# Fastaxx/Penguin.jl

Measured on AMD Instinct MI355X. Metric: time-steps/sec + SpMV GB/s (% HBM roofline), 3D mono diffusion 512^3, higher is better.
Workload: dtype f64

## Files before the change

### include/penguin_hip.h

```cpp
#ifndef PENGUIN_HIP_H
#define PENGUIN_HIP_H

#include <stddef.h>
#include <stdint.h>

#ifdef __cplusplus
extern "C" {
#endif

typedef struct pg_mesh pg_mesh;
typedef struct pg_capacity pg_capacity;
typedef struct pg_diffops pg_diffops;
typedef struct pg_solver pg_solver;
typedef struct pg_streamvort pg_streamvort;

enum { PG_BODY_BALL = 1, PG_BODY_MULTIBALL = 2, PG_BODY_HALFSPACE = 3, PG_BODY_ELLIPSOID = 4, PG_BODY_PLANE = 5 };
enum { PG_BODY_PROGRAM = 6 };
enum { PG_BODY_POLYGON = 7 };
enum { PG_FLAG_COMPLEMENT = 1, PG_FLAG_NO_CENTROIDS = 2 };
enum { PG_CAP_V = 0, PG_CAP_GAMMA = 1, PG_CAP_CELL_TYPES = 2, PG_CAP_A = 3, PG_CAP_B = 4,
       PG_CAP_W = 5, PG_CAP_C_OMEGA = 6, PG_CAP_C_GAMMA = 7,
       PG_CAP_ST_V0 = 8, PG_CAP_ST_V1 = 9, PG_CAP_ST_CT_OMEGA = 10, PG_CAP_ST_CT_GAMMA = 11 };
enum { PG_OP_G = 0, PG_OP_H = 1, PG_OP_WINV = 2,
       PG_OP_C0 = 3 , PG_OP_K0 = 6  };
// ... 194 lines not shown
                                       pg_solver** out);
int32_t pg_solver_create_unsteady_diph(pg_capacity* c1, pg_diffops* o1, pg_capacity* c2, pg_diffops* o2,
                                       const pg_jump_desc* ic, const pg_border_desc* borders, int32_t nborders,
                                       const double* D1, const double* D2, const double* f1, const double* f2,
                                       double dt, const double* T0, int32_t scheme, pg_solver** out);
int32_t pg_solver_create_moving_diph(pg_capacity* c1, pg_diffops* o1, pg_capacity* c2, pg_diffops* o2, const pg_jump_desc* ic,
                                     const pg_border_desc* borders, int32_t nborders, const double* D1, const double* D2,
                                     const double* f1_n, const double* f1_np1, const double* f2_n, const double* f2_np1,
                                     const double* T_prev, pg_solver* previous, int32_t scheme, pg_solver** out);
int32_t pg_solver_create_steady_mono(pg_capacity* c, pg_diffops* o, const pg_bc_desc* bc_interface,
                                     const pg_border_desc* borders, int32_t nborders, const double* Dcoef,
                                     const double* source, pg_solver** out);
int32_t pg_solver_create_steady_diph(pg_capacity* c1, pg_diffops* o1, pg_capacity* c2, pg_diffops* o2,
                                     const pg_jump_desc* ic, const pg_border_desc* borders, int32_t nborders,
                                     const double* D1, const double* D2, const double* f1, const double* f2,
                                     pg_solver** out);
int32_t pg_solver_create_moving_mono(pg_capacity* c, pg_diffops* o, const pg_bc_desc* bc_interface,
                                     const pg_border_desc* borders, int32_t nborders, const double* Dcoef,
                                     const double* source_n, const double* source_np1, const double* T_prev,
                                     pg_solver* previous, int32_t scheme, pg_solver** out);
int32_t pg_solver_create_moving_advdiff_mono(pg_capacity* c, pg_diffops* o, const pg_bc_desc* bc_interface,
                                             const pg_border_desc* borders, int32_t nborders, const double* Dcoef,
                                             const double* source_n, const double* source_np1, const double* T_prev,
                                             pg_solver* previous, int32_t scheme, pg_solver** out);
int32_t pg_solver_create_moving_advdiff_diph(pg_capacity* c1, pg_diffops* o1, pg_capacity* c2, pg_diffops* o2,
                                             const pg_jump_desc* ic, const pg_border_desc* borders, int32_t nborders,
                                             const double* D1, const double* D2, const double* f1_n, const double* f1_np1,
                                             const double* f2_n, const double* f2_np1, const double* T_prev,
                                             pg_solver* previous, int32_t scheme, pg_solver** out);
int32_t pg_solver_create_moving_stefan_diph(pg_capacity* c1, pg_diffops* o1, pg_capacity* c2, pg_diffops* o2,
                                            const pg_jump_desc* ic, const pg_border_desc* borders, int32_t nborders,
                                            const double* D1, const double* D2, const double* f1_n, const double* f1_np1,
                                            const double* f2_n, const double* f2_np1, const double* T_prev,
                                            pg_solver* previous, int32_t scheme, pg_solver** out);
int32_t pg_solver_stefan_terms(const pg_solver* s, double* out);
int32_t pg_solver_destroy(pg_solver* s);

int32_t pg_streamvort_create(pg_capacity* c, pg_diffops* o, const double* nu, double dt, const pg_bc_desc* bc_stream,
                             const pg_bc_desc* bc_vorticity, const pg_border_desc* borders_stream, int32_t nborders_stream,
                             const pg_border_desc* borders_vorticity, int32_t nborders_vorticity, const double* psi0,
                             const double* omega0, pg_streamvort** out);
int32_t pg_streamvort_destroy(pg_streamvort* sv);
int32_t pg_streamvort_set_omega(pg_streamvort* sv, const double* omega);
int32_t pg_streamvort_set_source(pg_streamvort* sv, const double* f_n , const double* f_np1 );
int32_t pg_streamvort_set_interface_values(pg_streamvort* sv, int32_t which, const double* g_n , const double* g_np1 );
int32_t pg_streamvort_set_border_values(pg_streamvort* sv, int32_t which, const double* values );
int32_t pg_streamvort_solve_stream(pg_streamvort* sv, const pg_krylov_opts* opts, pg_step_info* info);
int32_t pg_streamvort_step(pg_streamvort* sv, int32_t scheme, const pg_krylov_opts* opts, pg_step_info* info_psi,
                           pg_step_info* info_omega);
int32_t pg_streamvort_run(pg_streamvort* sv, int64_t steps, int32_t scheme, const pg_krylov_opts* opts, int32_t save_every,
                          pg_streamvort_run_info* info);
int32_t pg_streamvort_get(const pg_streamvort* sv, int32_t field, int64_t state_index, double* out, int64_t len);
int32_t pg_streamvort_num_states(const pg_streamvort* sv, int64_t* out);
int32_t pg_streamvort_time(const pg_streamvort* sv, int64_t state_index, double* out);
int32_t pg_streamvort_solver(pg_streamvort* sv, int32_t which, pg_solver** borrowed);

int32_t pg_solver_set_source(pg_solver* s, int32_t phase, const double* f_n , const double* f_np1 );
int32_t pg_solver_set_interface_value(pg_solver* s, const double* g_n , const double* g_np1 );
int32_t pg_solver_set_border_values(pg_solver* s, const double* values );

enum { PG_TD_SOURCE = 0, PG_TD_INTERFACE = 1, PG_TD_BORDER = 2 };
enum { PG_TD_MAX_TERMS = 8 };
int32_t pg_solver_set_separable(pg_solver* s, int32_t which, int32_t phase, int32_t K, const double* modes, int64_t nrows,
                                const double* coef);
int32_t pg_solver_clear_separable(pg_solver* s, int32_t which, int32_t phase);
int32_t pg_solver_time_data_info(const pg_solver* s, int32_t* terms , int64_t* nrows, int64_t* cursor);
int32_t pg_debug_td_combine_ms(pg_solver* s, int32_t scheme, int32_t repeats, double* ms_per_combine, int32_t* modes,
                               int64_t* bytes);

enum { PG_PROG_MAX_OPS = 96, PG_PROG_MAX_CONST = 32, PG_PROG_MAX_STACK = 16 };
enum {
  PG_OP_CONST = 0, PG_OP_VAR = 1, PG_OP_ADD = 2, PG_OP_SUB = 3, PG_OP_MUL = 4, PG_OP_DIV = 5, PG_OP_NEG = 6, PG_OP_ABS = 7,
  PG_OP_SQRT = 8, PG_OP_EXP = 9, PG_OP_LOG = 10, PG_OP_SIN = 11, PG_OP_COS = 12, PG_OP_TANH = 13, PG_OP_POW = 14,
  PG_OP_ATAN2 = 15, PG_OP_ERF = 16, PG_OP_ERFC = 17, PG_OP_MIN = 18, PG_OP_MAX = 19, PG_OP_LT = 20, PG_OP_LE = 21,
  PG_OP_GT = 22, PG_OP_GE = 23, PG_OP_SELECT = 24, PG_OP_COUNT = 25
};
typedef struct pg_program {
  int32_t n_ops;
  int32_t n_const;
  uint8_t op[PG_PROG_MAX_OPS];
  uint8_t arg[PG_PROG_MAX_OPS];
  double konst[PG_PROG_MAX_CONST];
} pg_program;
int32_t pg_program_validate(const pg_program* prog);
int32_t pg_program_eval_host(const pg_program* prog, int64_t npts, const double* xyz , double t, double* out);
int32_t pg_solver_set_program(pg_solver* s, int32_t which, int32_t phase, const pg_program* prog, int64_t nrows,
                              const double* times );
int32_t pg_solver_set_border_program(pg_solver* s, int32_t key, const pg_program* prog, int64_t nrows,
                                     const double* times );
int32_t pg_solver_program_info(const pg_solver* s, int32_t* programs , int64_t* entries , int64_t* nrows,
                               int64_t* cursor);
int32_t pg_debug_program_eval(const pg_program* prog, int64_t npts, const double* xyz , double t, double* out);
int32_t pg_capacity_create_program(pg_mesh* m, const pg_program* phi, const pg_program* grad , int32_t flags,
                                   pg_capacity** out);
int32_t pg_capacity_create_program3(pg_mesh* m, const pg_program* phi, const pg_program* grad , int32_t flags,
                                    pg_capacity** out);
int32_t pg_capacity_create_polygon(pg_mesh* m, const double* xy , int64_t M, int32_t flags, pg_capacity** out);
int32_t pg_capacity_polygon_ms_parts(const pg_capacity* c, double* ms );
int32_t pg_capacity_create_spacetime_program(pg_mesh* m, const pg_program* phi, const pg_program* grad ,
                                             const pg_program* dphidt, int32_t flags, double t0, double t1, int32_t nq,
                                             const double* tau_w , pg_capacity** out);
int32_t pg_capacity_create_spacetime_polygon(pg_mesh* m, const double* xy0 , const double* xy1 , int64_t M,
                                             int32_t flags, double t0, double t1, int32_t nq, const double* tau_w ,
                                             pg_capacity** out);
int32_t pg_debug_spacetime_kernel_timing(int32_t on);
int32_t pg_debug_capacity_spacetime_ms_parts(const pg_capacity* c, double* ms , int64_t* n_listed);
int32_t pg_debug_td_eval_ms(pg_solver* s, int32_t scheme, int32_t repeats, double* ms_per_eval, int64_t* entries,
                            int64_t* instructions);

enum { PG_MON_SUM = 0, PG_MON_SUMSQ = 1 };
enum { PG_MON_MAX = 8 };
int32_t pg_solver_set_monitors(pg_solver* s, int32_t K, const int32_t* kinds, const double* weights , int64_t len);
int32_t pg_solver_clear_monitors(pg_solver* s);
int32_t pg_solver_monitor_info(const pg_solver* s, int32_t* K, int64_t* rows, int32_t* sparse , int64_t* stored );
int32_t pg_solver_get_monitor_series(const pg_solver* s, int64_t row0, int64_t nrows, double* values ,
                                     double* times );
int32_t pg_solver_drop_states(pg_solver* s);
int32_t pg_debug_monitor_ms(pg_solver* s, int32_t repeats, double* ms_per_eval, int64_t* bytes);
int32_t pg_debug_monitor_eval(pg_solver* s, double* values , int32_t* x_form);

int32_t pg_solver_initial_solve(pg_solver* s, const pg_krylov_opts* opts, pg_step_info* info);
int32_t pg_solver_step(pg_solver* s, int32_t scheme, const pg_krylov_opts* opts, pg_step_info* info);
int32_t pg_solver_run(pg_solver* s, double Tend, int32_t scheme, const pg_krylov_opts* opts, int32_t do_initial,
                      int64_t max_steps, int32_t save_every, pg_run_info* info);
int32_t pg_solver_num_states(const pg_solver* s, int64_t* out);
int32_t pg_solver_get_state(const pg_solver* s, int64_t state_index, double* x, int64_t len);
int32_t pg_solver_system_info(const pg_solver* s, int32_t which, pg_system_info* out);
int32_t pg_solver_get_system_csr(const pg_solver* s, int32_t which, int64_t* rowptr, int64_t* col, double* val,
                                 double* b, int64_t* idx);
int32_t pg_solver_get_row_scaling(const pg_solver* s, int32_t which, double* ds);
int32_t pg_solver_mg_info(const pg_solver* s, pg_mg_info* out);
int32_t pg_solver_mg_info_for(const pg_solver* s, int32_t precond, pg_mg_info* out);
int32_t pg_solver_mg_step_info(const pg_solver* s, int32_t which, pg_mg_info* out);
int32_t pg_solver_spectral_estimate(pg_solver* s, int32_t which, pg_specest_info* out);
int32_t pg_solver_time_spmv(pg_solver* s, int32_t which, int32_t reps, double* avg_ms);

int32_t pg_partition_planes(const int64_t* weight, int64_t nplanes, int32_t nranks, int64_t* bounds);
int32_t pg_slab_numbering_host(int32_t K, int64_t plane, int64_t nplanes, int64_t p0, int64_t p1, const uint8_t* active,
                               int64_t* out);

int32_t pg_debug_spmv_compare(pg_solver* s, int32_t which, int32_t variant_a, int32_t variant_b, double* max_abs_diff,
                              double* max_abs);
int32_t pg_debug_spmv_mode_compare(pg_solver* s, int32_t which, int32_t mode, double* max_abs_diff, double* max_abs,
                                   double* max_dot_rel);
int32_t pg_debug_spmv_sizes(pg_solver* s, int32_t which, int64_t* n, int64_t* n_vec, int64_t* nnz, int32_t* grid);
#define PG_DEBUG_SPMV_SENTINEL 0x7FF8C0DE5EED0BADull
int32_t pg_debug_spmv_apply(pg_solver* s, int32_t which, int32_t variant, int32_t mode, const double* x, const double* aux,
                            const double* dotx, const double* base, double pc0, double pc1, double pc2, int32_t fold,
                            int32_t done, int32_t repeat, double* y, double* partials, double* slot_sums, double* folded,
                            int64_t* ticket);
#define PG_DEBUG_SPMV_SENTINEL_F32 0x7FC5EED0u
int32_t pg_debug_spmv_apply_typed(pg_solver* s, int32_t which, int32_t kind, const void* x, const void* base, double pc0, double pc1,
                                  double pc2, double sigma, int32_t done, double* y64, float* y32, float* p32);
int32_t pg_debug_read_probe(int64_t bytes, int32_t elem_bytes, int32_t nt, int32_t blocks, int32_t reps, double* gbs);
int32_t pg_debug_run_virtual_ranks(int32_t nranks, int32_t N, const int64_t* n, const double* L, int32_t body_kind,
                                   const double* params, int32_t nparams, double interface_value, double border_value,
                                   int32_t nkeys, const int32_t* keys, double dt, int32_t scheme_ctor, int32_t scheme_run,
                                   int64_t steps, double* x_out, int64_t* n_own_out, int64_t* nnz_out,
                                   int64_t* n_ghost_out, int64_t* iters_out);
int32_t pg_debug_set_virtual_rank_method(int32_t method, int32_t restart);
int32_t pg_debug_set_virtual_rank_precond(int32_t precond);
int32_t pg_debug_set_virtual_rank_ramp(double ramp);
int32_t pg_debug_set_virtual_rank_kick(int64_t step, double factor);
int32_t pg_debug_virtual_rank_info(int32_t rank, int64_t* full_rows, int64_t* loop_rows, int64_t* loop_bytes,
                                   int64_t* loop_ghosts);
int32_t pg_debug_scale_diagonal_rows(pg_solver* s, double factor);
int32_t pg_debug_set_poly_give_up(int32_t iterations);

int32_t pg_debug_mg_aggregates(pg_solver* s, int32_t level, int64_t* n, int32_t* agg);
int32_t pg_debug_mg_level_csr(pg_solver* s, int32_t level, int64_t* n, int64_t* nnz, int64_t* rowptr, int64_t* col, double* val);
int32_t pg_debug_mg_apply(pg_solver* s, const double* r, double* z);
int32_t pg_debug_mg_aggregates_for(pg_solver* s, int32_t precond, int32_t level, int64_t* n, int32_t* agg);
int32_t pg_debug_mg_level_csr_for(pg_solver* s, int32_t precond, int32_t level, int64_t* n, int64_t* nnz, int64_t* rowptr, int64_t* col,
                                  double* val);
int32_t pg_debug_mg_apply_for(pg_solver* s, int32_t precond, const double* r, double* z);
int32_t pg_debug_mg_step_aggregates(pg_solver* s, int32_t which, int32_t level, int64_t* n, int32_t* agg);
int32_t pg_debug_mg_step_level_csr(pg_solver* s, int32_t which, int32_t level, int64_t* n, int64_t* nnz, int64_t* rowptr, int64_t* col,
                                   double* val);
int32_t pg_debug_mg_step_apply(pg_solver* s, int32_t which, const double* r, double* z);

int32_t pg_debug_specest_hessenberg(pg_solver* s, int32_t which, int32_t* steps, double* H);

int32_t pg_solver_guess_info(pg_solver* s, int32_t* kept, int32_t* nstates, int32_t* offsets , double* coef ,
                             double* rr_plain, double* rr_taken);

#ifdef __cplusplus
}
#endif
#endif
```

### penguin/jl_amd/_lib.py

```python
from __future__ import annotations

import ctypes as C
import os
import re
from pathlib import Path

import numpy as np

_HERE = Path(__file__).resolve().parent
LIB_PATH = Path(os.environ["PG_LIB_PATH"]) if os.environ.get("PG_LIB_PATH") else _HERE / "lib" / "libpenguin_hip.so"
HEADER_PATH = _HERE.parent.parent / "include" / "penguin_hip.h"


class PenguinHipError(RuntimeError):
    pass


PG_BODY_BALL, PG_BODY_MULTIBALL, PG_BODY_HALFSPACE, PG_BODY_ELLIPSOID, PG_BODY_PLANE = 1, 2, 3, 4, 5
PG_BODY_PROGRAM, PG_BODY_POLYGON = 6, 7
PG_FLAG_COMPLEMENT, PG_FLAG_NO_CENTROIDS = 1, 2
PG_CAP_V, PG_CAP_GAMMA, PG_CAP_CELL_TYPES, PG_CAP_A, PG_CAP_B, PG_CAP_W, PG_CAP_C_OMEGA, PG_CAP_C_GAMMA = range(8)
PG_CAP_ST_V0, PG_CAP_ST_V1, PG_CAP_ST_CT_OMEGA, PG_CAP_ST_CT_GAMMA = 8, 9, 10, 11
PG_OP_G, PG_OP_H, PG_OP_WINV = 0, 1, 2
PG_OP_C0, PG_OP_K0 = 3, 6
# ... 197 lines not shown
def solver_mg_info(handle, precond: int = PG_PRECOND_MG) -> dict:
    info = pg_mg_info()
    check(lib().pg_solver_mg_info_for(handle, C.c_int32(precond), C.byref(info)))
    n = info.levels
    return {"levels": n, "tail_level": info.tail_level, "rows": list(info.rows[:n]), "nnz": list(info.nnz[:n]),
            "setup_ms": info.setup_ms, "bytes": info.bytes}


def debug_mg_aggregates(handle, level: int, precond: int = PG_PRECOND_MG) -> np.ndarray:
    n = C.c_int64(0)
    check(lib().pg_debug_mg_aggregates_for(handle, C.c_int32(precond), C.c_int32(level), C.byref(n), None))
    agg = np.zeros(max(n.value, 1), dtype=np.int32)
    check(lib().pg_debug_mg_aggregates_for(handle, C.c_int32(precond), C.c_int32(level), C.byref(n), agg.ctypes.data_as(c_i32_p)))
    return agg[: n.value]


def debug_mg_level_csr(handle, level: int, precond: int = PG_PRECOND_MG):
    n, nnz = C.c_int64(0), C.c_int64(0)
    pc = C.c_int32(precond)
    check(lib().pg_debug_mg_level_csr_for(handle, pc, C.c_int32(level), C.byref(n), C.byref(nnz), None, None, None))
    rowptr, col, val = np.zeros(n.value + 1, dtype=np.int64), np.zeros(max(nnz.value, 1), dtype=np.int64), np.zeros(max(nnz.value, 1))
    check(lib().pg_debug_mg_level_csr_for(handle, pc, C.c_int32(level), C.byref(n), C.byref(nnz), iptr(rowptr), iptr(col), dptr(val)))
    return rowptr, col[: nnz.value], val[: nnz.value]


def debug_mg_apply(handle, r: np.ndarray, precond: int = PG_PRECOND_MG) -> np.ndarray:
    r = np.ascontiguousarray(r, dtype=np.float64)
    z = np.zeros_like(r)
    check(lib().pg_debug_mg_apply_for(handle, C.c_int32(precond), dptr(r), dptr(z)))
    return z


def _mg_info_dict(info) -> dict:
    n = info.levels
    return {"levels": n, "tail_level": info.tail_level, "rows": list(info.rows[:n]), "nnz": list(info.nnz[:n]),
            "setup_ms": info.setup_ms, "bytes": info.bytes}


def solver_mg_step_info(handle, which: int = 0) -> dict:
    info = pg_mg_info()
    check(lib().pg_solver_mg_step_info(handle, C.c_int32(which), C.byref(info)))
    return _mg_info_dict(info)


def debug_mg_step_aggregates(handle, which: int, level: int) -> np.ndarray:
    n = C.c_int64(0)
    check(lib().pg_debug_mg_step_aggregates(handle, C.c_int32(which), C.c_int32(level), C.byref(n), None))
    agg = np.zeros(max(n.value, 1), dtype=np.int32)
    check(lib().pg_debug_mg_step_aggregates(handle, C.c_int32(which), C.c_int32(level), C.byref(n), agg.ctypes.data_as(c_i32_p)))
    return agg[: n.value]


def debug_mg_step_level_csr(handle, which: int, level: int):
    n, nnz = C.c_int64(0), C.c_int64(0)
    w = C.c_int32(which)
    check(lib().pg_debug_mg_step_level_csr(handle, w, C.c_int32(level), C.byref(n), C.byref(nnz), None, None, None))
    rowptr, col, val = np.zeros(n.value + 1, dtype=np.int64), np.zeros(max(nnz.value, 1), dtype=np.int64), np.zeros(max(nnz.value, 1))
    check(lib().pg_debug_mg_step_level_csr(handle, w, C.c_int32(level), C.byref(n), C.byref(nnz), iptr(rowptr), iptr(col), dptr(val)))
    return rowptr, col[: nnz.value], val[: nnz.value]


def debug_mg_step_apply(handle, which: int, r: np.ndarray) -> np.ndarray:
    r = np.ascontiguousarray(r, dtype=np.float64)
    z = np.zeros_like(r)
    check(lib().pg_debug_mg_step_apply(handle, C.c_int32(which), dptr(r), dptr(z)))
    return z


def solver_spectral_estimate(handle, which: int = 0, run: bool = True) -> dict:
    info = pg_specest_info()
    check(lib().pg_solver_spectral_estimate(handle, C.c_int32(which | (0 if run else 4)), C.byref(info)))
    return {k: getattr(info, k) for k, _ in pg_specest_info._fields_ if k != "reserved"}


def debug_specest_hessenberg(handle, which: int = 0, run: bool = True) -> np.ndarray:
    w = C.c_int32(which | (0 if run else 4))
    k = C.c_int32(0)
    check(lib().pg_debug_specest_hessenberg(handle, w, C.byref(k), None))
    H = np.zeros((k.value + 1) * max(k.value, 1))
    check(lib().pg_debug_specest_hessenberg(handle, w, C.byref(k), dptr(H)))
    return H[: (k.value + 1) * k.value].reshape((k.value + 1, k.value), order="F")


DEBUG_SPMV_SENTINEL = 0x7FF8C0DE5EED0BAD
DEBUG_SPMV_GUARD = 64


def debug_spmv_sizes(handle, which: int) -> tuple[int, int, int, int]:
    n, nv, nnz, grid = C.c_int64(0), C.c_int64(0), C.c_int64(0), C.c_int32(0)
    check(lib().pg_debug_spmv_sizes(handle, C.c_int32(which), C.byref(n), C.byref(nv), C.byref(nnz), C.byref(grid)))
    return n.value, nv.value, nnz.value, grid.value


def loop_system_csr(handle, which: int):
    n, _, nnz, _ = debug_spmv_sizes(handle, which)
    rowptr, col, val = np.zeros(n + 1, dtype=np.int64), np.zeros(max(nnz, 1), dtype=np.int64), np.zeros(max(nnz, 1))
    check(lib().pg_solver_get_system_csr(handle, C.c_int32(which), iptr(rowptr), iptr(col), dptr(val), None, None))
    return rowptr, col[:nnz], val[:nnz]


def debug_spmv_apply(handle, which: int, variant: int, mode: int, x, aux=None, dotx=None, base=None, pc=(0.0, 0.0, 0.0),
                     fold: int = 0, done: int = 0, repeat: int = 1) -> dict:
    n, nv, _, grid = debug_spmv_sizes(handle, which)

    def arr(a, length, name):
        if a is None:
            return None, None
        a = np.ascontiguousarray(a, dtype=np.float64)
        if a.size != length:
            raise ValueError(f"debug_spmv_apply: {name} has {a.size} entries, the matrix needs {length}")
        return a, dptr(a)

    xs, xp = arr(x, nv, "x")
    auxs, auxp = arr(aux, n, "aux")
    dots, dotp = arr(dotx, n, "dotx")
    bases, basep = arr(base, n, "base")
    y = np.zeros(n + DEBUG_SPMV_GUARD)
    partials = np.zeros((5, grid))
    sums, folded = np.zeros(5), np.zeros(5)
    ticket = C.c_int64(-1)
    check(lib().pg_debug_spmv_apply(handle, C.c_int32(which), C.c_int32(variant), C.c_int32(mode), xp, auxp, dotp, basep,
                                    C.c_double(pc[0]), C.c_double(pc[1]), C.c_double(pc[2]), C.c_int32(fold), C.c_int32(done),
                                    C.c_int32(repeat), dptr(y), dptr(partials), dptr(sums), dptr(folded), C.byref(ticket)))
    return {"y": y, "partials": partials, "slot_sums": sums, "folded": folded, "ticket": ticket.value, "grid": grid, "n": n}


DEBUG_SPMV_SENTINEL_F32 = 0x7FC5EED0
TYPED_FIRST, TYPED_MIDDLE, TYPED_HANDOVER = 1, 2, 3


def debug_spmv_apply_typed(handle, which: int, kind: int, x, base=None, pc=(0.0, 0.0, 0.0), sigma: float = 1.0, done: int = 0) -> dict:
    n, nv, _, _ = debug_spmv_sizes(handle, which)
    want_x = np.float64 if kind == TYPED_FIRST else np.float32
    want_b = {TYPED_FIRST: None, TYPED_MIDDLE: np.float32, TYPED_HANDOVER: np.float64}[kind]
    x = np.ascontiguousarray(x)
    if x.dtype != want_x or x.size != nv:
        raise ValueError(f"debug_spmv_apply_typed: x must be {nv} x {np.dtype(want_x).name}")
    if (base is None) != (want_b is None):
        raise ValueError("debug_spmv_apply_typed: base goes with kinds 2 and 3, and only with them")
    bp = None
    if base is not None:
        base = np.ascontiguousarray(base)
        if base.dtype != want_b or base.size != n:
            raise ValueError(f"debug_spmv_apply_typed: base must be {n} x {np.dtype(want_b).name}")
        bp = base.ctypes.data_as(C.c_void_p)
    y64 = np.zeros(n + DEBUG_SPMV_GUARD) if kind == TYPED_HANDOVER else None
    y32 = np.zeros(n + DEBUG_SPMV_GUARD, dtype=np.float32) if kind != TYPED_HANDOVER else None
    p32 = np.zeros(n + DEBUG_SPMV_GUARD, dtype=np.float32) if kind == TYPED_FIRST else None
    ptr = lambda a: None if a is None else a.ctypes.data_as(C.c_void_p)
    check(lib().pg_debug_spmv_apply_typed(handle, C.c_int32(which), C.c_int32(kind), x.ctypes.data_as(C.c_void_p), bp,
                                          C.c_double(pc[0]), C.c_double(pc[1]), C.c_double(pc[2]), C.c_double(sigma), C.c_int32(done),
                                          ptr(y64), ptr(y32), ptr(p32)))
    return {"y": y64 if kind == TYPED_HANDOVER else y32, "p32": p32}
```

### penguin/jl_amd/csrc/pg_common.h

```cpp
#pragma once
#include <hip/hip_runtime.h>
#include "pg_rccl.h"

#include <chrono>
#include <cstdint>
#include <cstdio>
#include <cstring>
#include <stdexcept>
#include <string>
#include <vector>

#include "../../../include/penguin_hip.h"

namespace pg {

using i64 = int64_t;
using i32 = int32_t;

struct Error : std::runtime_error {
  using std::runtime_error::runtime_error;
};

void set_last_error(const std::string& msg);

#define PG_HIP(expr)                                                                              \
  do {                                                                                            \
    hipError_t _e = (expr);                                                                       \
    if (_e != hipSuccess)                                                                         \
      throw pg::Error(std::string("HIP error: ") + hipGetErrorString(_e) + " at " + __FILE__ + ":" + \
                      std::to_string(__LINE__) + " (" #expr ")");                                 \
  } while (0)

#define PG_NCCL(expr)                                                                             \
  do {                                                                                            \
    ncclResult_t _e = (expr);                                                                     \
    if (_e != ncclSuccess)                                                                        \
      throw pg::Error(std::string("RCCL error: ") + pg::rccl::api().GetErrorString(_e) + " at " + __FILE__ + ":" + \
                      std::to_string(__LINE__) + " (" #expr ")");                                 \
  } while (0)

#define PG_REQUIRE(cond, msg)                                   \
  do {                                                          \
    if (!(cond)) throw pg::Error(std::string(msg));             \
  } while (0)

#define PG_API_BEGIN try {
#define PG_API_END                                  \
  return 0;                                         \
  }                                                 \
  catch (const std::exception& e) {                 \
    pg::set_last_error(e.what());                   \
    return 1;                                       \
  }                                                 \
  catch (...) {                                     \
    pg::set_last_error("unknown exception");        \
    return 2;                                       \
  }

struct Config {
  bool debug = false;
  int alloc_poison = 0;
  int async_alloc = 0;
  int alloc_guard = 0;
  long long pool_limit_mb = 0;
  bool poly = true;
  int poly_degree = 6;
  bool poly_adapt = true;
  double poly_margin = 1.0;
  double poly_slack = -1.0;
  int poly_hist = 3;
  bool poly_trend = true;
  int poly_maxdeg = 0;
  int poly_mindeg = 4;
  bool poly_f32 = true;
  int poly_f32_tail = -1;
  int profile_sample = 3;
  bool gamma_elim = true;
  bool diag_elim = true;
  double diag_elim_frac = 0.0005;
  int spmv_variant = 70;
  int spmv_xcd = 1;
  int spmv_strip = 16;
  int spmv_march_k = 0;
  int spmv_minrun = 24;
  bool spmv_march = true;
  bool spmv_edges = true;
  int spmv_tile_units = 0;
  int spmv_blocks_per_cu = 0;
  bool halo_overlap = true;
  int guess_n = 4;
  int guess_depth = 7;
  bool guess_defer = true;
  bool guess_always = false;
  int guess_monitor = 256;
  double guess_pass_cost = 0.34;
  double guess_gain = 0.8;
  bool step_fuse = true;
  bool speculate_product = true;
  int mg_tail_rows = 2048;
  int unit_order = 0;
};
const Config& config();

struct LocalComm;

struct Context {
  bool inited = false;
  LocalComm* local = nullptr;
  int device = 0;
  hipStream_t stream = nullptr;
  hipStream_t comm_stream = nullptr;
  hipEvent_t ev_fork = nullptr, ev_join = nullptr;
  int rank = 0, nranks = 1;
  ncclComm_t comm = nullptr;
  ncclComm_t comm_halo = nullptr;
  bool profiling = false;
  std::string device_name;
};
Context& ctx();
void require_init();
void set_thread_context(Context* c);
Context* thread_context();
LocalComm* local_comm_create(int nranks);
void local_comm_destroy(LocalComm* c);
void comm_allreduce_sum_f64(double* dev, int count, hipStream_t st);
void comm_allreduce_max_f64(double* dev, int count, hipStream_t st);
void comm_allreduce_sum_u64(unsigned long long* dev, i64 count, hipStream_t st);

void* dev_alloc(size_t bytes);
void dev_free(void* p);
void dev_cache_release();
struct AsyncAllocScope {
  AsyncAllocScope();
  ~AsyncAllocScope();
};

template <class T>
struct DevBuf {
  T* p = nullptr;
  i64 n = 0;
  DevBuf() = default;
  explicit DevBuf(i64 n_) { alloc(n_); }
  DevBuf(const DevBuf&) = delete;
  DevBuf& operator=(const DevBuf&) = delete;
  DevBuf(DevBuf&& o) noexcept : p(o.p), n(o.n) { o.p = nullptr; o.n = 0; }
  DevBuf& operator=(DevBuf&& o) noexcept {
    if (this != &o) { release(); p = o.p; n = o.n; o.p = nullptr; o.n = 0; }
    return *this;
  }
  ~DevBuf() { release(); }
  void release() {
    if (p) dev_free(p);
    p = nullptr; n = 0;
  }
  void alloc(i64 n_) {
    release();
    n = n_;
    if (n > 0) p = static_cast<T*>(dev_alloc(sizeof(T) * static_cast<size_t>(n) + 64));
  }
  void zero() {
    if (n > 0) PG_HIP(hipMemsetAsync(p, 0, sizeof(T) * static_cast<size_t>(n), ctx().stream));
  }
  void upload(const T* h, i64 count, i64 offset = 0) {
    if (count > 0) {
      PG_HIP(hipMemcpyAsync(p + offset, h, sizeof(T) * static_cast<size_t>(count), hipMemcpyHostToDevice, ctx().stream));
      PG_HIP(hipStreamSynchronize(ctx().stream));
    }
  }
  void download(T* h, i64 count, i64 offset = 0) const {
    if (count > 0) {
      PG_HIP(hipMemcpyAsync(h, p + offset, sizeof(T) * static_cast<size_t>(count), hipMemcpyDeviceToHost, ctx().stream));
      PG_HIP(hipStreamSynchronize(ctx().stream));
    }
  }
};

inline void* pinned_scratch(int slot, size_t bytes) {
  static thread_local void* buf[2] = {nullptr, nullptr};
  static thread_local size_t cap[2] = {0, 0};
  if (bytes > cap[slot]) {
    if (buf[slot]) (void)hipHostFree(buf[slot]);
    PG_HIP(hipHostMalloc(&buf[slot], bytes + (bytes >> 2)));
    cap[slot] = bytes + (bytes >> 2);
  }
  return buf[slot];
}

struct Laps {
  bool on;
  std::chrono::steady_clock::time_point t0;
  explicit Laps() : on(config().debug), t0(std::chrono::steady_clock::now()) {}
  void lap(const char* what) {
    if (!on) return;
    (void)hipDeviceSynchronize();
    const auto t1 = std::chrono::steady_clock::now();
    fprintf(stderr, "[pg_laps] %-34s %8.2f ms\n", what, std::chrono::duration<double, std::milli>(t1 - t0).count());
    t0 = t1;
  }
};

struct EventPair {
  hipEvent_t e0 = nullptr, e1 = nullptr;
  EventPair() {
    PG_HIP(hipEventCreate(&e0));
    if (hipEventCreate(&e1) != hipSuccess) {
      (void)hipEventDestroy(e0);
      throw Error("hipEventCreate failed");
    }
  }
  ~EventPair() {
    if (e0) (void)hipEventDestroy(e0);
    if (e1) (void)hipEventDestroy(e1);
  }
  EventPair(const EventPair&) = delete;
  EventPair& operator=(const EventPair&) = delete;
};

inline int grid_for(i64 n, int block, int cap = 256 * 8) {
  i64 g = (n + block - 1) / block;
  if (g < 1) g = 1;
  if (g > cap) g = cap;
  return static_cast<int>(g);
}

constexpr int CAP_HALO = 3;

struct Slab {
  int N = 0;
  i64 n[3] = {1, 1, 1};
  i64 ext[3] = {1, 1, 1};
  i64 stride[3] = {1, 1, 1};
  i64 plane = 1;
  i64 nplanes = 1;
  i64 M = 1;
  i64 p0 = 0, p1 = 1;
  i64 s0 = 0, s1 = 1;
  i64 Mloc() const { return (s1 - s0) * plane; }
  i64 first_cell() const { return s0 * plane; }
  void set_own(i64 a, i64 b) {
    p0 = a; p1 = b;
    s0 = p0 - CAP_HALO; if (s0 < 0) s0 = 0;
// ... 38 lines not shown
```

### penguin/jl_amd/csrc/pg_context.hip

```cpp
#include "pg_common.h"

#include <cxxabi.h>
#include <execinfo.h>

#include <atomic>
#include <map>
#include <mutex>
#include <unordered_map>
#include <unordered_set>
#include "pg_host_algos.h"

#include <algorithm>
#include <array>
#include <memory>
#include <set>

namespace pg {

static thread_local std::string g_last_error;
void set_last_error(const std::string& msg) { g_last_error = msg; }

Context& ctx() {
  static Context c;
  Context* t = thread_context();
  return t ? *t : c;
}

const Config& config() {
  static const Config c = [] {
    Config k;
    auto geti = [](const char* name, long long dflt) { const char* v = getenv(name); return v ? atoll(v) : dflt; };
    auto getd = [](const char* name, double dflt) { const char* v = getenv(name); return v ? atof(v) : dflt; };
    k.debug = getenv("PG_DEBUG") != nullptr;
    k.alloc_poison = (int)geti("PG_ALLOC_POISON", 0);
    k.async_alloc = (int)geti("PG_ASYNC_ALLOC", 0);
    k.alloc_guard = (int)geti("PG_ALLOC_GUARD", 0);
    k.pool_limit_mb = geti("PG_POOL_LIMIT_MB", 0);
    k.poly = geti("PG_POLY", 1) != 0;
    k.poly_degree = (int)geti("PG_POLY_DEGREE", 6);
    k.poly_adapt = geti("PG_POLY_ADAPT", getenv("PG_POLY_DEGREE") ? 0 : 1) != 0;
    k.poly_margin = getd("PG_POLY_MARGIN", 1.0);
    k.poly_slack = getd("PG_POLY_SLACK", -1.0);
    k.poly_hist = (int)std::max<long long>(1, std::min<long long>(3, geti("PG_POLY_HIST", 3)));
    k.poly_maxdeg = (int)geti("PG_POLY_MAXDEG", 0);
    k.poly_mindeg = (int)std::max<long long>(2, std::min<long long>(8, geti("PG_POLY_MINDEG", 4)));
    k.poly_trend = geti("PG_POLY_TREND", 1) != 0;
    k.poly_f32 = geti("PG_POLY_F32", 1) != 0;
    k.poly_f32_tail = (int)std::max<long long>(-1, std::min<long long>(64, geti("PG_POLY_F32_TAIL", -1)));
    k.profile_sample = (int)std::max<long long>(1, geti("PG_PROFILE_SAMPLE", 3));
    k.gamma_elim = geti("PG_GAMMA_ELIM", 1) != 0;
    k.diag_elim = geti("PG_DIAG_ELIM", 1) != 0;
    k.diag_elim_frac = getd("PG_DIAG_ELIM_FRAC", 0.0005);
    k.spmv_variant = (int)geti("PG_SPMV_VARIANT", 70);
    k.spmv_xcd = (int)geti("PG_SPMV_XCD", 1);
    k.spmv_strip = (int)geti("PG_SPMV_STRIP", 16);
    k.spmv_march_k = (int)geti("PG_SPMV_MARCH_K", 0);
    k.spmv_minrun = (int)geti("PG_SPMV_MINRUN", 24);
    k.spmv_march = geti("PG_SPMV_MARCH", 1) != 0;
    k.spmv_edges = geti("PG_SPMV_EDGES", 1) != 0;
    k.spmv_tile_units = (int)geti("PG_SPMV_TILE_UNITS", 0);
    k.spmv_blocks_per_cu = (int)geti("PG_SPMV_BLOCKS_PER_CU", 0);
    k.halo_overlap = geti("PG_HALO_OVERLAP", 1) != 0;
    k.speculate_product = geti("PG_SPECULATE", 1) != 0;
    k.guess_n = (int)std::max<long long>(0, std::min<long long>(4, geti("PG_GUESS_STATES", 4)));
    k.guess_depth = (int)std::max<long long>(1, std::min<long long>(7, geti("PG_GUESS_DEPTH", 7)));
    k.mg_tail_rows = (int)std::max<long long>(0, geti("PG_MG_TAIL_ROWS", 2048));
    k.guess_monitor = (int)std::max<long long>(1, geti("PG_GUESS_MONITOR", 256));
    k.guess_pass_cost = getd("PG_GUESS_PASS_COST", 0.34);
    k.guess_always = geti("PG_GUESS_ALWAYS", 0) != 0;
    k.guess_defer = geti("PG_GUESS_DEFER", 1) != 0;
    k.guess_gain = getd("PG_GUESS_GAIN", 0.8);
    k.step_fuse = geti("PG_STEP_FUSE", 1) != 0;
    k.unit_order = (int)geti("PG_SPMV_UNIT_ORDER", 0);
    return k;
  }();
  return c;
}

void require_init() {
  if (!ctx().inited)
    throw Error("penguin_hip: not initialised (call pg_init / pg_init_distributed first)");
}

static void init_device(int device_id) {
  Context& c = ctx();
  int ndev = 0;
  hipError_t e = hipGetDeviceCount(&ndev);
  if (e != hipSuccess || ndev <= 0)
    throw Error("penguin_hip: no HIP device visible -- this library has no CPU fallback");
  PG_REQUIRE(device_id >= 0 && device_id < ndev, "penguin_hip: device id out of range");
  PG_HIP(hipSetDevice(device_id));
  hipDeviceProp_t prop;
  PG_HIP(hipGetDeviceProperties(&prop, device_id));
  c.device = device_id;
  c.device_name = std::string(prop.name) + " (" + prop.gcnArchName + ")";
  if (!c.stream) PG_HIP(hipStreamCreateWithFlags(&c.stream, hipStreamNonBlocking));
  if (!c.comm_stream) PG_HIP(hipStreamCreateWithFlags(&c.comm_stream, hipStreamNonBlocking));
  c.inited = true;
}

}

using namespace pg;

namespace pg {
namespace {
thread_local int t_async_scope = 0;
std::mutex g_alloc_mutex;
struct BlockCache {
  std::multimap<size_t, void*> free_blocks;
  std::unordered_map<void*, size_t> owned;
  size_t free_bytes = 0;
};
BlockCache g_cache;
constexpr size_t CACHE_TRIM_BYTES = (size_t)48 << 30;

size_t round_block(size_t bytes) {
  const size_t q = bytes >= ((size_t)2 << 20) ? ((size_t)2 << 20) : 4096;
  return (bytes + q - 1) / q * q;
}

bool cache_wanted(const Context& c, size_t bytes) {
  const int mode = config().async_alloc;
  if (mode < 0 || !c.inited || !c.stream || c.local) return false;
  if (!(t_async_scope > 0 || mode > 0)) return false;
  const long long lim = config().pool_limit_mb;
  return lim <= 0 || bytes < ((size_t)lim << 20);
}

void poison(void* p, size_t bytes) {
  if (!config().alloc_poison || !p || bytes == 0) return;
  Context& c = ctx();
  if (c.inited && c.stream) PG_HIP(hipMemsetAsync(p, 0xFF, bytes, c.stream));
  else PG_HIP(hipMemset(p, 0xFF, bytes));
}

void cache_trim_locked() {
  if (g_cache.free_blocks.empty()) return;
  (void)hipDeviceSynchronize();
  for (auto& kv : g_cache.free_blocks) {
    g_cache.owned.erase(kv.second);
    (void)hipFree(kv.second);
  }
  g_cache.free_blocks.clear();
  g_cache.free_bytes = 0;
}

void* dev_alloc_raw(size_t bytes) {
  void* p = nullptr;
  Context& c = ctx();
  if (cache_wanted(c, bytes)) {
    const size_t want = round_block(bytes);
    {
      std::lock_guard<std::mutex> lk(g_alloc_mutex);
      auto it = g_cache.free_blocks.lower_bound(want);
      if (it != g_cache.free_blocks.end() && it->first <= want + want / 8) {
        p = it->second;
        g_cache.free_bytes -= it->first;
        g_cache.free_blocks.erase(it);
      }
    }
    if (!p) {
      if (hipMalloc(&p, want) != hipSuccess || !p) {
        (void)hipGetLastError();
        { std::lock_guard<std::mutex> lk(g_alloc_mutex); cache_trim_locked(); }
        PG_HIP(hipMalloc(&p, want));
      }
      std::lock_guard<std::mutex> lk(g_alloc_mutex);
      g_cache.owned[p] = want;
    }
    poison(p, bytes);
    return p;
  }
  PG_HIP(hipMalloc(&p, bytes));
  poison(p, bytes);
  return p;
}

void dev_free_raw(void* p) {
  if (!p) return;
  {
    std::lock_guard<std::mutex> lk(g_alloc_mutex);
    auto it = g_cache.owned.find(p);
    if (it != g_cache.owned.end()) {
      g_cache.free_blocks.emplace(it->second, p);
      g_cache.free_bytes += it->second;
      if (g_cache.free_bytes > CACHE_TRIM_BYTES) cache_trim_locked();
      return;
    }
  }
  (void)hipFree(p);
}

constexpr size_t GUARD = 4096;
struct GuardInfo { char* raw; size_t bytes; unsigned long long seq; std::string where; };
std::unordered_map<void*, GuardInfo> g_guarded;
unsigned long long g_alloc_seq = 0;
std::string call_stack() {
  void* frames[24];
  const int nf = backtrace(frames, 24);
  char** sym = backtrace_symbols(frames, nf);
  std::string s;
  for (int i = 2; sym && i < nf && i < 12; ++i) {
    std::string f = sym[i];
    const size_t a = f.find('('), b = f.find('+', a == std::string::npos ? 0 : a);
    if (a != std::string::npos && b != std::string::npos && b > a + 1) {
      std::string mangled = f.substr(a + 1, b - a - 1);
      int st = 0;
      char* dem = abi::__cxa_demangle(mangled.c_str(), nullptr, nullptr, &st);
      f = st == 0 && dem ? dem : mangled;
      free(dem);
      const size_t par = f.find('(');
      if (par != std::string::npos) f = f.substr(0, par);
    }
// ... 2 lines not shown
  free(sym);
  return s;
}
}

AsyncAllocScope::AsyncAllocScope() { ++t_async_scope; }
AsyncAllocScope::~AsyncAllocScope() { --t_async_scope; }

void dev_cache_release() {
  std::lock_guard<std::mutex> lk(g_alloc_mutex);
  cache_trim_locked();
}

void* dev_alloc(size_t bytes) {
  if (!config().alloc_guard) return dev_alloc_raw(bytes);
  char* raw = static_cast<char*>(dev_alloc_raw(bytes + 2 * GUARD));
  Context& c = ctx();
  hipStream_t st = (c.inited && c.stream) ? c.stream : nullptr;
  PG_HIP(hipMemsetAsync(raw, 0xA5, GUARD, st));
  PG_HIP(hipMemsetAsync(raw + GUARD + bytes, 0xA5, GUARD, st));
  void* user = raw + GUARD;
  std::lock_guard<std::mutex> lk(g_alloc_mutex);
  g_guarded[user] = GuardInfo{raw, bytes, ++g_alloc_seq, call_stack()};
  return user;
}

void dev_free(void* p) {
  if (!config().alloc_guard) { dev_free_raw(p); return; }
  GuardInfo gi;
  {
    std::lock_guard<std::mutex> lk(g_alloc_mutex);
    auto it = g_guarded.find(p);
    if (it == g_guarded.end()) { gi.raw = nullptr; }
    else { gi = it->second; g_guarded.erase(it); }
  }
  if (!gi.raw) { dev_free_raw(p); return; }
  (void)hipDeviceSynchronize();
  std::vector<unsigned char> lo(GUARD), hi(GUARD);
  (void)hipMemcpy(lo.data(), gi.raw, GUARD, hipMemcpyDeviceToHost);
  (void)hipMemcpy(hi.data(), gi.raw + GUARD + gi.bytes, GUARD, hipMemcpyDeviceToHost);
  auto first_bad = [](const std::vector<unsigned char>& g, bool from_end) -> long {
    if (from_end) { for (long i = (long)g.size() - 1; i >= 0; --i) if (g[i] != 0xA5) return i; }
    else { for (size_t i = 0; i < g.size(); ++i) if (g[i] != 0xA5) return (long)i; }
    return -1;
  };
  const long bl = first_bad(lo, true), bh = first_bad(hi, false);
  if (bl >= 0 || bh >= 0) {
    long nl = 0, nh = 0;
    for (unsigned char v : lo) nl += v != 0xA5;
    for (unsigned char v : hi) nh += v != 0xA5;
    fprintf(stderr, "[pg_alloc] GUARD DAMAGED: block #%llu of %zu bytes (incl. 64 of slack): %ld bytes written BELOW it (nearest %ld bytes "
            "before the start), %ld bytes written ABOVE it (first %ld bytes past the end); allocated by: %s\n", gi.seq, gi.bytes, nl,
            bl >= 0 ? (long)GUARD - bl : 0, nh, bh >= 0 ? bh : 0, gi.where.c_str());
  }
  dev_free_raw(gi.raw);
}
}

extern "C" {

int32_t pg_last_error(char* buf, size_t n) {
  if (buf && n > 0) {
    std::strncpy(buf, g_last_error.c_str(), n - 1);
    buf[n - 1] = 0;
  }
  return 0;
}

int32_t pg_init(int32_t device_id) {
  PG_API_BEGIN
  Context& c = ctx();
  init_device(device_id);
  c.rank = 0;
  c.nranks = 1;
  PG_API_END
}

int32_t pg_get_unique_id(void* out128) {
  PG_API_BEGIN
  static_assert(sizeof(ncclUniqueId) == 128, "ncclUniqueId is expected to be 128 bytes");
  ncclUniqueId id;
  PG_NCCL(rccl::api().GetUniqueId(&id));
  std::memcpy(out128, &id, sizeof(id));
  PG_API_END
}

int32_t pg_init_distributed(int32_t device_id, int32_t rank, int32_t nranks, const void* unique_id128) {
  PG_API_BEGIN
  Context& c = ctx();
  PG_REQUIRE(nranks >= 1 && rank >= 0 && rank < nranks, "pg_init_distributed: bad rank / nranks");
  init_device(device_id);
  c.rank = rank;
  c.nranks = nranks;
  if (nranks > 1 || unique_id128 != nullptr) {
    PG_REQUIRE(unique_id128 != nullptr, "pg_init_distributed: unique id required when nranks > 1");
    ncclUniqueId id;
    std::memcpy(&id, unique_id128, sizeof(id));
    const rccl::Api& R = rccl::api();
    PG_NCCL(R.CommInitRank(&c.comm, nranks, id, rank));
    bool split_ok = false;
    if (R.CommSplit) {
      split_ok = R.CommSplit(c.comm, 0, rank, &c.comm_halo, nullptr) == ncclSuccess && c.comm_halo != nullptr;
      if (!split_ok) c.comm_halo = nullptr;
    }
    if (!split_ok) {
      ncclUniqueId id2;
      if (rank == 0) PG_NCCL(R.GetUniqueId(&id2));
      DevBuf<char> buf((i64)sizeof(id2));
      if (rank == 0) buf.upload(reinterpret_cast<const char*>(&id2), (i64)sizeof(id2));
      PG_NCCL(R.Broadcast(buf.p, buf.p, sizeof(id2), ncclChar, 0, c.comm, c.stream));
      buf.download(reinterpret_cast<char*>(&id2), (i64)sizeof(id2));
      PG_NCCL(R.CommInitRank(&c.comm_halo, nranks, id2, rank));
    }
  }
  PG_API_END
}

int32_t pg_finalize(void) {
  PG_API_BEGIN
  Context& c = ctx();
  if (c.inited) {
    (void)hipDeviceSynchronize();
    if (c.comm_halo) { (void)rccl::api().CommDestroy(c.comm_halo); c.comm_halo = nullptr; }
    if (c.comm) { (void)rccl::api().CommDestroy(c.comm); c.comm = nullptr; }
    dev_cache_release();
    if (c.stream) { (void)hipStreamDestroy(c.stream); c.stream = nullptr; }
    if (c.comm_stream) { (void)hipStreamDestroy(c.comm_stream); c.comm_stream = nullptr; }
    if (c.ev_fork) { (void)hipEventDestroy(c.ev_fork); c.ev_fork = nullptr; }
    if (c.ev_join) { (void)hipEventDestroy(c.ev_join); c.ev_join = nullptr; }
    c.inited = false;
  }
  PG_API_END
}

int32_t pg_device_synchronize(void) {
  PG_API_BEGIN
  require_init();
  PG_HIP(hipDeviceSynchronize());
  PG_API_END
}

int32_t pg_set_profiling(int32_t on) {
  PG_API_BEGIN
  ctx().profiling = on != 0;
  PG_API_END
}

int32_t pg_config_string(char* buf, size_t n) {
  PG_API_BEGIN
  const Config& k = config();
  char tmp[1024];
  snprintf(tmp, sizeof(tmp),
           "spmv_variant=%d spmv_xcd=%d spmv_strip=%d spmv_unit_order=%d spmv_march=%d spmv_edges=%d spmv_march_k=%d spmv_minrun=%d spmv_tile_units=%d "
           "spmv_blocks_per_cu=%d halo_overlap=%d speculate=%d poly=%d poly_degree=%d poly_adapt=%d "
           "poly_margin=%g poly_slack=%g poly_hist=%d poly_trend=%d poly_maxdeg=%d poly_f32=%d poly_f32_tail=%d gamma_elim=%d diag_elim=%d "
           "guess_states=%d guess_depth=%d guess_defer=%d step_fuse=%d async_alloc=%d cache_limit_mb=%lld alloc_poison=%d alloc_guard=%d profile_sample=%d debug=%d",
           k.spmv_variant, k.spmv_xcd, k.spmv_strip, k.unit_order, (int)k.spmv_march, (int)k.spmv_edges, k.spmv_march_k, k.spmv_minrun, k.spmv_tile_units,
           k.spmv_blocks_per_cu, (int)k.halo_overlap, (int)k.speculate_product, (int)k.poly, k.poly_degree, (int)k.poly_adapt,
           k.poly_margin, k.poly_slack, k.poly_hist, (int)k.poly_trend, k.poly_maxdeg, (int)k.poly_f32, k.poly_f32_tail,
           (int)k.gamma_elim, (int)k.diag_elim, k.guess_n, k.guess_depth, (int)k.guess_defer, (int)k.step_fuse, k.async_alloc, k.pool_limit_mb, k.alloc_poison, k.alloc_guard, k.profile_sample, (int)k.debug);
  if (buf && n > 0) {
    std::strncpy(buf, tmp, n - 1);
    buf[n - 1] = 0;
  }
  PG_API_END
}

int32_t pg_device_name(char* buf, size_t n) {
  PG_API_BEGIN
  require_init();
  if (buf && n > 0) {
    std::strncpy(buf, ctx().device_name.c_str(), n - 1);
    buf[n - 1] = 0;
  }
  PG_API_END
}

int32_t pg_mesh_create(int32_t N, const int64_t* n, const double* L, const double* x0, pg_mesh** out) {
  PG_API_BEGIN
  PG_REQUIRE(N >= 1 && N <= 3, "pg_mesh_create: N must be 1, 2 or 3");
  PG_REQUIRE(out != nullptr, "pg_mesh_create: out is NULL");
  PG_REQUIRE(n != nullptr && L != nullptr, "pg_mesh_create: n / L is NULL");
  std::unique_ptr<pg_mesh> guard(new pg_mesh());
  pg_mesh* m = guard.get();
  m->N = N;
  for (int d = 0; d < N; ++d) {
    PG_REQUIRE(n[d] >= 1, "pg_mesh_create: n_d must be >= 1");
    m->n[d] = n[d];
    m->L[d] = L[d];
    m->x0[d] = x0 ? x0[d] : 0.0;
    const double h = L[d] / static_cast<double>(n[d]);
    m->centers[d].resize(n[d]);
    m->nodes[d].resize(n[d] + 1);
    for (i64 j = 0; j < n[d]; ++j) m->centers[d][j] = m->x0[d] + static_cast<double>(j) * h;
    for (i64 j = 0; j <= n[d]; ++j) m->nodes[d][j] = m->x0[d] + (static_cast<double>(j) + 0.5) * h;
  }
  if (ctx().inited) {
    for (int d = 0; d < N; ++d) {
      m->d_nodes[d].alloc(n[d] + 1);
      m->d_nodes[d].upload(m->nodes[d].data(), n[d] + 1);
    }
  }
  *out = guard.release();
  PG_API_END
}

int32_t pg_mesh_destroy(pg_mesh* m) {
  PG_API_BEGIN
  delete m;
  PG_API_END
}

int32_t pg_mesh_get_centers(const pg_mesh* m, int32_t d, double* out, int64_t len) {
  PG_API_BEGIN
  PG_REQUIRE(m && d >= 0 && d < m->N && len == m->n[d], "pg_mesh_get_centers: bad arguments");
  std::memcpy(out, m->centers[d].data(), sizeof(double) * len);
  PG_API_END
}

int32_t pg_mesh_get_nodes(const pg_mesh* m, int32_t d, double* out, int64_t len) {
  PG_API_BEGIN
  PG_REQUIRE(m && d >= 0 && d < m->N && len == m->n[d] + 1, "pg_mesh_get_nodes: bad arguments");
  std::memcpy(out, m->nodes[d].data(), sizeof(double) * len);
  PG_API_END
}

int32_t pg_mesh_num_border_cells(const pg_mesh* m, int64_t* out) {
  PG_API_BEGIN
  PG_REQUIRE(m && out, "pg_mesh_num_border_cells: bad arguments");
  i64 all = 1, inner = 1;
  for (int d = 0; d < m->N; ++d) {
    all *= m->n[d];
    inner *= std::max<i64>(m->n[d] - 2, 0);
  }
  *out = all - inner;
  PG_API_END
}

int32_t pg_mesh_get_border_cells(const pg_mesh* mc, int64_t* idx, double* pos, int32_t* key) {
  PG_API_BEGIN
  PG_REQUIRE(mc, "pg_mesh_get_border_cells: mesh is NULL");
  pg_mesh* m = const_cast<pg_mesh*>(mc);
  mesh_build_border(m);
  const size_t nb = m->border_key.size();
  if (idx) std::memcpy(idx, m->border_idx.data(), sizeof(i64) * nb * m->N);
  if (pos) std::memcpy(pos, m->border_pos.data(), sizeof(double) * nb * m->N);
  if (key) std::memcpy(key, m->border_key.data(), sizeof(i32) * nb);
  PG_API_END
}

int32_t pg_partition_planes(const int64_t* weight, int64_t nplanes, int32_t nranks, int64_t* bounds) {
  PG_API_BEGIN
  PG_REQUIRE(weight && bounds && nplanes >= 1 && nranks >= 1, "pg_partition_planes: bad arguments");
  PG_REQUIRE(nplanes >= nranks, "pg_partition_planes: fewer planes than ranks");
  pghost::partition_planes(weight, nplanes, nranks, bounds);
  PG_API_END
}

int32_t pg_slab_numbering_host(int32_t K, int64_t plane, int64_t nplanes, int64_t p0, int64_t p1, const uint8_t* active,
                               int64_t* out) {
  PG_API_BEGIN
  PG_REQUIRE(K >= 1 && K <= pghost::SLAB_MAX_KINDS && plane >= 1 && nplanes >= 1 && p0 >= 0 && p1 > p0 && p1 <= nplanes && active && out,
             "pg_slab_numbering_host: bad arguments");
  const pghost::SlabPlanes g = pghost::slab_planes(p0, p1, nplanes, CAP_HALO);
  const i64 Mloc = (g.s1 - g.s0) * plane;
  const i64 lcA0 = (g.a0 - g.s0) * plane, lcA1 = (g.a1 - g.s0) * plane;
  const i64 lcO = (p0 - g.s0) * plane, lcU = (p1 - g.s0) * plane, lcFE = (p0 + 1 - g.s0) * plane, lcLB = (p1 - 1 - g.s0) * plane;
  i64 posO[pghost::SLAB_MAX_KINDS], posU[pghost::SLAB_MAX_KINDS], posFE[pghost::SLAB_MAX_KINDS], posLB[pghost::SLAB_MAX_KINDS],
      tot[pghost::SLAB_MAX_KINDS];
  for (int k = 0; k < K; ++k) {
    i64 c = 0;
    posO[k] = posU[k] = posFE[k] = posLB[k] = -1;
    for (i64 lc = 0; lc <= Mloc; ++lc) {
      if (lc == lcO) posO[k] = c;
      if (lc == lcU) posU[k] = c;
      if (lc == lcFE) posFE[k] = c;
      if (lc == lcLB) posLB[k] = c;
      if (lc < Mloc && lc >= lcA0 && lc < lcA1 && active[(i64)k * Mloc + lc]) ++c;
    }
    tot[k] = c;
  }
  pghost::SlabNumbering sn;
  pghost::slab_numbering(K, posO, posU, posFE, posLB, tot, p0 > 0, p1 < nplanes, sn);
  i64 q = 0;
  out[q++] = sn.n_own;
  out[q++] = sn.n_ghost;
  const i64* arrays[10] = {sn.cnt_own, sn.off_own, sn.cntL, sn.offL, sn.cntU, sn.offU, sn.sendL_off, sn.sendL_cnt, sn.sendU_off, sn.sendU_cnt};
  for (const i64* a : arrays)
    for (int k = 0; k < K; ++k) out[q++] = a[k];
  PG_API_END
}

}

namespace pg {

void mesh_build_border(pg_mesh* m) {
  if (m->border_built) return;
  const int N = m->N;
  std::vector<i64>& bi = m->border_idx;
  std::set<std::array<i64, 3>> seen;
  auto emit = [&](i64 i0, i64 i1, i64 i2) {
    std::array<i64, 3> key{i0, i1, i2};
    if (!seen.insert(key).second) return;
    const i64 id[3] = {i0, i1, i2};
    for (int d = 0; d < N; ++d) {
      bi.push_back(id[d] + 1);
      m->border_pos.push_back(m->centers[d][id[d]]);
    }
    m->border_key.push_back(border_key_of(N, m->n, i0, i1, i2));
  };
// ... 34 lines not shown
```

### penguin/jl_amd/csrc/pg_solver.hip

```cpp
#include <algorithm>
#include <cmath>
#include <memory>

#include "pg_krylov.h"
#include "pg_reduce.h"
#include "pg_multigrid.h"
#include "pg_program.h"
#include "pg_scan.h"
#include "pg_solver_internal.h"
#include "pg_spmv.h"
#include "pg_specest.h"

using namespace pg;

namespace pg { extern double g_host_wait_us; }

struct pg_solver {
  int nphase = 1;
  pg_capacity* cap[2] = {nullptr, nullptr};
  pg_diffops* ops[2] = {nullptr, nullptr};
  Slab slab;
  int K = 2;
  i64 Mloc = 0, M = 0;
  double dt = 0.0, t = 0.0;
// ... 3485 lines not shown
  spmv_mode_compare(A, std::max(nv, A.n), mode, max_abs_diff, max_abs, max_dot_rel);
  PG_API_END
}

int32_t pg_debug_spmv_sizes(pg_solver* s, int32_t which, int64_t* n, int64_t* n_vec, int64_t* nnz, int32_t* grid) {
  PG_API_BEGIN
  require_init();
  PG_REQUIRE(s, "pg_debug_spmv_sizes: NULL argument");
  i64 nv = 0;
  const CsrMatrix& A = debug_matrix(s, which, &nv);
  if (n) *n = A.n;
  if (n_vec) *n_vec = std::max(nv, A.n);
  if (nnz) *nnz = A.nnz;
  if (grid) *grid = spmv_default_grid(A.n);
  PG_API_END
}

int32_t pg_debug_spmv_apply(pg_solver* s, int32_t which, int32_t variant, int32_t mode, const double* x, const double* aux,
                            const double* dotx, const double* base, double pc0, double pc1, double pc2, int32_t fold,
                            int32_t done, int32_t repeat, double* y, double* partials, double* slot_sums, double* folded,
                            int64_t* ticket) {
  PG_API_BEGIN
  require_init();
  PG_REQUIRE(s && x && y && slot_sums && folded && ticket, "pg_debug_spmv_apply: NULL argument");
  PG_REQUIRE(ctx().nranks == 1 && !ctx().comm, "pg_debug_spmv_apply: one rank (the split launch of a slab is not covered)");
  PG_REQUIRE(variant == 70 || variant == 38 || variant == 2 || variant == 1, "pg_debug_spmv_apply: variants 70, 38, 2 and 1");
  PG_REQUIRE(mode == 0 || mode == 1 || mode == 2 || mode == 3 || mode == 8, "pg_debug_spmv_apply: launch modes 0, 1, 2, 3 and 8");
  PG_REQUIRE(repeat == 1 || repeat == 2, "pg_debug_spmv_apply: repeat is 1 or 2");
  PG_REQUIRE(fold == 0 || fold == 1, "pg_debug_spmv_apply: fold is 0 or 1");
  const bool slices = (variant & 64) != 0;
  PG_REQUIRE(slices || (mode != 8 && !dotx && !fold),
             "pg_debug_spmv_apply: mode 8, a separate dot operand and the folded scalar phase exist in the slice kernel (variant 70) only");
  PG_REQUIRE(!fold || (mode >= 1 && mode <= 3), "pg_debug_spmv_apply: only the modes with dots (1, 2, 3) fold a scalar phase");
  PG_REQUIRE((mode == 1 || mode == 3) == (aux != nullptr), "pg_debug_spmv_apply: aux goes with modes 1 and 3, and only with them");
  PG_REQUIRE(!dotx || mode == 2 || mode == 3, "pg_debug_spmv_apply: dotx goes with modes 2 and 3");
  PG_REQUIRE(!base || mode == 8, "pg_debug_spmv_apply: base goes with mode 8");
  i64 nv = 0;
  const CsrMatrix& A = debug_matrix(s, which, &nv);
  const i64 n = A.n;
  PG_REQUIRE(n > 0, "pg_debug_spmv_apply: the matrix has no rows");
  PG_REQUIRE(!slices || A.srec.p, "pg_debug_spmv_apply: the matrix has no slice image");
  nv = std::max(nv, n);
  hipStream_t st = ctx().stream;
  const int grid = spmv_default_grid(n);
  constexpr i64 GUARD = 64;
  double sentinel;
  const unsigned long long sbits = PG_DEBUG_SPMV_SENTINEL;
  std::memcpy(&sentinel, &sbits, sizeof(double));
  DevBuf<double> dx(nv), daux(nv), ddot(nv), dbase(nv), dy(n + GUARD), dpart(5 * (i64)grid), dsc(S_COUNT);
  DevBuf<unsigned> dticket(1);
  daux.zero(); ddot.zero(); dbase.zero(); dsc.zero(); dticket.zero();
  dx.upload(x, nv);
  if (aux) daux.upload(aux, n);
  if (dotx) ddot.upload(dotx, n);
  if (base) dbase.upload(base, n);
  {
    std::vector<double> fill((size_t)std::max<i64>(n + GUARD, 5 * (i64)grid), sentinel);
    dy.upload(fill.data(), n + GUARD);
    if (fold && mode == 3) std::fill(fill.begin() + 2 * (size_t)grid, fill.begin() + 4 * (size_t)grid, 0.0);
    dpart.upload(fill.data(), 5 * (i64)grid);
    std::vector<double> hsc(S_COUNT, 0.0);
    for (int k = 0; k < 5; ++k) hsc[S_RED0 + k] = sentinel;
    hsc[S_DONE] = (double)done;
    dsc.upload(hsc.data(), S_COUNT);
  }
  FinArgs f{fold ? dticket.p : nullptr, fold ? dsc.p : nullptr, PH_NONE, fold ? (mode == 1 ? 1 : (mode == 2 ? 2 : 5)) : 0, 0,
            dotx ? ddot.p : nullptr};
  if (mode == 8) { f.pc0 = pc0; f.pc1 = pc1; f.pc2 = pc2; f.base = base ? dbase.p : dx.p; }
  const bool with_fin = mode == 8 || fold || dotx;
  for (int r = 0; r < repeat; ++r) {
    const bool folded_here = launch_spmv_as(variant, mode, A, dx.p, dy.p, aux ? daux.p : nullptr, mode >= 1 && mode <= 3 ? dpart.p : nullptr,
                                            dsc.p, grid, st, with_fin ? &f : nullptr);
    PG_REQUIRE(folded_here == (fold != 0), "pg_debug_spmv_apply: the launch did not report the scalar phase as asked");
  }
  PG_HIP(hipGetLastError());
  dy.download(y, n + GUARD);
  std::vector<double> hp(5 * (size_t)grid), hsc(S_COUNT);
  dpart.download(hp.data(), 5 * (i64)grid);
  dsc.download(hsc.data(), S_COUNT);
  if (partials) std::memcpy(partials, hp.data(), sizeof(double) * hp.size());
  for (int k = 0; k < 5; ++k) {
    double a = 0.0;
    for (int i = 0; i < grid; ++i) a += hp[(size_t)k * grid + i];
    slot_sums[k] = a;
    folded[k] = hsc[S_RED0 + k];
  }
  unsigned ht = 0;
  dticket.download(&ht, 1);
  *ticket = (int64_t)ht;
  PG_API_END
}

int32_t pg_debug_spmv_apply_typed(pg_solver* s, int32_t which, int32_t kind, const void* x, const void* base, double pc0, double pc1,
                                  double pc2, double sigma, int32_t done, double* y64, float* y32, float* p32) {
  PG_API_BEGIN
  require_init();
  PG_REQUIRE(s && x, "pg_debug_spmv_apply_typed: NULL argument");
  PG_REQUIRE(ctx().nranks == 1 && !ctx().comm, "pg_debug_spmv_apply_typed: one rank");
  PG_REQUIRE(kind == TYPED_FIRST || kind == TYPED_MIDDLE || kind == TYPED_HANDOVER, "pg_debug_spmv_apply_typed: kinds 1 (first), 2 (middle), 3 (hand-over)");
  PG_REQUIRE((kind == TYPED_FIRST) == (base == nullptr), "pg_debug_spmv_apply_typed: the first launch's base is its x; the others take one");
  PG_REQUIRE((kind == TYPED_FIRST) == (p32 != nullptr), "pg_debug_spmv_apply_typed: p32 is the first launch's output, and only its");
  PG_REQUIRE(kind == TYPED_HANDOVER ? (y64 && !y32) : (y32 && !y64), "pg_debug_spmv_apply_typed: y32 for kinds 1 and 2, y64 for kind 3");
  PG_REQUIRE(spmv_supports_typed_chain(), "pg_debug_spmv_apply_typed: the typed launches exist in the slice kernel with the stream hint only");
  i64 nv = 0;
  const CsrMatrix& A = debug_matrix(s, which, &nv);
  const i64 n = A.n;
  PG_REQUIRE(n > 0 && A.srec.p, "pg_debug_spmv_apply_typed: the matrix has no rows or no slice image");
  nv = std::max(nv, n);
  hipStream_t st = ctx().stream;
  const int grid = spmv_default_grid(n);
  constexpr i64 GUARD = 64;
  double sentinel;
  const unsigned long long sbits = PG_DEBUG_SPMV_SENTINEL;
  std::memcpy(&sentinel, &sbits, sizeof(double));
  float sentinel32;
  const unsigned sbits32 = PG_DEBUG_SPMV_SENTINEL_F32;
  std::memcpy(&sentinel32, &sbits32, sizeof(float));
  DevBuf<double> dx64(nv), db64(nv), dy64(n + GUARD), dsc(S_COUNT);
  DevBuf<float> dx32(nv), db32(nv), dy32(n + GUARD), dp32(n + GUARD);
  db64.zero(); db32.zero();
  if (kind == TYPED_FIRST) dx64.upload(static_cast<const double*>(x), nv);
  else dx32.upload(static_cast<const float*>(x), nv);
  if (kind == TYPED_MIDDLE) db32.upload(static_cast<const float*>(base), n);
  if (kind == TYPED_HANDOVER) db64.upload(static_cast<const double*>(base), n);
  {
    std::vector<double> f64((size_t)(n + GUARD), sentinel);
    std::vector<float> f32((size_t)(n + GUARD), sentinel32);
    dy64.upload(f64.data(), n + GUARD);
    dy32.upload(f32.data(), n + GUARD);
    dp32.upload(f32.data(), n + GUARD);
    std::vector<double> hsc(S_COUNT, 0.0);
    hsc[S_DONE] = (double)done;
    dsc.upload(hsc.data(), S_COUNT);
  }
  FinArgs f{nullptr, nullptr, PH_NONE, 0, 0, nullptr};
  f.pc0 = pc0; f.pc1 = pc1; f.pc2 = pc2;
  if (kind == TYPED_FIRST) {
    f.base = dx64.p; f.p32 = dp32.p; f.psig = sigma;
    launch_spmv_typed(kind, A, dx64.p, dy32.p, dsc.p, grid, st, f);
  } else if (kind == TYPED_MIDDLE) {
    f.base = reinterpret_cast<const double*>(db32.p);
    launch_spmv_typed(kind, A, dx32.p, dy32.p, dsc.p, grid, st, f);
  } else {
    f.base = db64.p;
    launch_spmv_typed(kind, A, dx32.p, dy64.p, dsc.p, grid, st, f);
  }
  PG_HIP(hipGetLastError());
  if (y64) dy64.download(y64, n + GUARD);
  if (y32) dy32.download(y32, n + GUARD);
  if (p32) dp32.download(p32, n + GUARD);
  PG_API_END
}

__global__ void k_scale_rows(i64 n_e, const int* __restrict__ elist, double factor, double* __restrict__ z) {
  for (i64 q = blockIdx.x * (i64)blockDim.x + threadIdx.x; q < n_e; q += (i64)gridDim.x * blockDim.x) z[elist[q]] *= factor;
}

int32_t pg_debug_scale_diagonal_rows(pg_solver* s, double factor) {
  PG_API_BEGIN
  require_init();
  PG_REQUIRE(s && s->have_run, "pg_debug_scale_diagonal_rows: no run matrix yet");
  const CsrMatrix& A = run_matrix(s);
  DiagElim& DE = (&A == &s->A_ctor) ? s->diag_ctor : s->diag_run;
  PG_REQUIRE(DE.active && DE.n_e > 0, "pg_debug_scale_diagonal_rows: the loop of this solver is not the compact one");
  hipLaunchKernelGGL(k_scale_rows, dim3(grid_for(DE.n_e, BLOCK)), dim3(BLOCK), 0, ctx().stream, DE.n_e, (const int*)DE.elist.p, factor,
                     s->z.p);
  PG_HIP(hipGetLastError());
  PG_HIP(hipStreamSynchronize(ctx().stream));
  s->x_valid = false;
  s->spec_y_valid = false;
  PG_API_END
}

int32_t pg_solver_guess_info(pg_solver* s, int32_t* kept, int32_t* nstates, int32_t* offsets, double* coef, double* rr_plain,
                             double* rr_taken) {
  PG_API_BEGIN
  require_init();
  PG_REQUIRE(s && kept && nstates && offsets && coef && rr_plain && rr_taken, "pg_solver_guess_info: NULL argument");
  *kept = s->hist_cnt;
  *nstates = 0;
  *rr_plain = *rr_taken = 0.0;
  for (int j = 0; j < 4; ++j) { offsets[j] = 0; coef[j] = 0.0; }
  if (s->guess_coef.n >= 16 && s->hist_cnt > 0) {
    double hc[16];
    s->guess_coef.download(hc, 16, s->guess_buf ? GUESS_USED : 0);
    *nstates = (int32_t)hc[4];
    for (int j = 0; j < *nstates && j < 4; ++j) { offsets[j] = (int32_t)hc[5 + j] + 1; coef[j] = hc[j]; }
    *rr_plain = hc[9];
    *rr_taken = hc[10];
  }
  PG_API_END
}

int32_t pg_solver_time_spmv(pg_solver* s, int32_t which, int32_t reps, double* avg_ms) {
  PG_API_BEGIN
  require_init();
  PG_REQUIRE(s && avg_ms && reps > 0, "pg_solver_time_spmv: bad arguments");
  const int sel = which & 1, mode = (which & 2048) ? 8 : ((which >> 4) & 7);
  PG_REQUIRE(mode <= 3 || mode == 8, "pg_solver_time_spmv: unknown launch mode");
  if (sel == 1) PG_REQUIRE(s->have_run, "run matrix not assembled yet");
  const CsrMatrix& Afull = sel == 0 ? s->A_ctor : run_matrix(s);
  GammaElim& E = (&Afull == &s->A_ctor) ? s->elim_ctor : s->elim_run;
  if ((which & 512) && !E.tried) build_gamma_elim(Afull, s->nb, E);
  DiagElim& DE = (&Afull == &s->A_ctor) ? s->diag_ctor : s->diag_run;
  if ((which & 4096) && !DE.tried) build_diag_elim(Afull, s->nb, s->slab, DE);
  const CsrMatrix& A = ((which & 4096) && DE.active) ? DE.A : (((which & 512) && E.active) ? E.A : Afull);
  const bool chained = (which & 1024) != 0;
  hipStream_t st = ctx().stream;
  EventPair ev;
  KrylovWork& w = s->work;
  const bool cold = (which & 256) != 0;
  constexpr int RING = 7;
  std::vector<DevBuf<double>> ring;
  const i64 nv = s->nb.n_vec();
  if (cold) {
    ring.resize(RING);
    for (auto& b : ring) {
      b.alloc(nv > 0 ? nv : 1);
      if (nv > 0) PG_HIP(hipMemcpyAsync(b.p, s->z.p, sizeof(double) * (size_t)nv, hipMemcpyDeviceToDevice, st));
    }
  }
  int it = 0;
  auto one = [&]() {
    const double* xin = cold ? ring[it % RING].p : (chained && (it & 1) ? s->y.p : s->z.p);
    double* yout = cold ? ring[(it + 3) % RING].p : (chained && (it & 1) ? s->z.p : s->y.p);
    const double* ax = cold ? ring[(it + 5) % RING].p : w.rhat.p;
    ++it;
    if (mode == 0) spmv(A, xin, yout, st);
    else if (mode == 8) {
      FinArgs f{nullptr, nullptr, PH_NONE, 0, 0, nullptr};
      f.pc0 = 1.0; f.pc1 = -0.5; f.pc2 = 0.5; f.base = s->b.p;
      launch_spmv(8, A, xin, yout, nullptr, nullptr, nullptr, w.grid, st, &f);
    }
    else launch_spmv(mode, A, xin, yout, ax, w.partials.p, nullptr, w.grid, st);
  };
  for (int i = 0; i < 3; ++i) one();
  PG_HIP(hipEventRecord(ev.e0, st));
  for (int i = 0; i < reps; ++i) one();
  PG_HIP(hipEventRecord(ev.e1, st));
  PG_HIP(hipEventSynchronize(ev.e1));
  PG_HIP(hipGetLastError());
  float ms = 0.f;
  PG_HIP(hipEventElapsedTime(&ms, ev.e0, ev.e1));
  *avg_ms = ms / reps;
  PG_API_END
}

}

namespace pg {

int32_t solver_create_unsteady_mono_dev(pg_capacity* c, pg_diffops* o, const pg_bc_desc* bc_interface, const pg_border_desc* borders,
                                        int32_t nborders, const SolverDeviceData& dev, double dt, const double* T0,
                                        pg_solver* previous, int32_t scheme, pg_solver** out) {
  SolverSpec d = spec_mono("pg_streamvort_step", c, o, bc_interface, borders, nborders, nullptr, nullptr, nullptr, out);
  d.dt = dt; d.T0 = T0; d.previous = previous; d.scheme = scheme;
  d.dev = &dev;
  d.solved_once = true;
  return create_solver(d);
}

i64 solver_mloc(const pg_solver* s) { return s->Mloc; }

double* solver_source_dev(pg_solver* s) {
  if (s->f_np1[0].n != s->Mloc) { s->f_np1[0].alloc(s->Mloc); s->f_np1[0].zero(); }
  return s->f_np1[0].p;
}

void solver_data_changed(pg_solver* s) { s->bconst_dirty = true; }

void solver_solve_again(pg_solver* s, const pg_krylov_opts* opts, SolveStats& st) {
  PG_REQUIRE(s->scheme_ctor == PG_SCHEME_STEADY && !s->moving, "solve again: a steady solver is expected");
  if (!s->initial_done) {
    build_first_rhs(s);
    do_initial(s, opts, st);
    return;
  }
  const pg_krylov_opts o = opts ? *opts : default_opts();
  MgHierarchy* const mg = mg_prepare(s, o);
  if (mg_is_step(o.precond)) mg_step_conditions(s, o.method);
  specest_prepare(s, s->A_ctor, o);
  const i64 n = s->nb.n_own;
  ensure_bconst(s, PG_SCHEME_STEADY);
  if (n > 0) apply_left(s->A_ctor, s->bconst.p, s->b.p, ctx().stream);
  const bool from_state = o.warm_start != 0 && (o.method == PG_METHOD_BICGSTAB || o.method == PG_METHOD_IDRS) && n > 0;
  solve_ctor_system(s, o, st, from_state, false, mg);
}

constexpr double REFINE_RELTOL = 1e-6;

__global__ void k_refine_residual(i64 n, i64 nvec, const double* __restrict__ b, const double* __restrict__ y, double* __restrict__ r) {
  for (i64 i = blockIdx.x * (i64)blockDim.x + threadIdx.x; i < nvec; i += (i64)gridDim.x * blockDim.x) r[i] = i < n ? b[i] - y[i] : 0.0;
}

__global__ void k_refine_add(i64 n, const double* __restrict__ d, double* __restrict__ z) {
  for (i64 i = blockIdx.x * (i64)blockDim.x + threadIdx.x; i < n; i += (i64)gridDim.x * blockDim.x) z[i] += d[i];
}

static void refine_once(pg_solver* s, const pg_krylov_opts& o, SolveStats& st) {
  const i64 n = s->nb.n_own, nv = s->nb.n_vec();
  if (n <= 0) return;
  hipStream_t stream = ctx().stream;
  const CsrMatrix& A = s->A_ctor;
  spmv_halo(A, s->nb, s->slab, s->z.p, s->y.p, stream);
  DevBuf<double> r(nv);
  hipLaunchKernelGGL(k_refine_residual, dim3(grid_for(nv, BLOCK)), dim3(BLOCK), 0, stream, n, nv, (const double*)s->b.p,
// ... 48 lines not shown
```

### penguin/jl_amd/csrc/pg_spmv.h

```cpp
#pragma once
#include "pg_system.h"

namespace pg {

enum { S_RHO = 0, S_RHO_OLD, S_ALPHA, S_OMEGA, S_BETA, S_RR, S_BB, S_TOL2, S_DONE, S_ITERS, S_RELTOL2, S_ABSTOL2,
       S_RESTART, S_RHAT2, S_FORCE, S_PENDING3, S_RRW, S_HALF, S_RR0 ,
       S_MOVED ,
       S_HELD ,
       S_RED0, S_RED1, S_RED2, S_RED3, S_RED4, S_COUNT };

constexpr int BLOCK = 256;

__device__ inline double wave_sum(double v) {
#pragma unroll
  for (int off = 32; off > 0; off >>= 1) v += __shfl_down(v, off, 64);
  return v;
}

__device__ inline double block_sum(double v, double* sh ) {
  v = wave_sum(v);
  const int lane = threadIdx.x & 63, wave = threadIdx.x >> 6;
  __syncthreads();
  if (lane == 0) sh[wave] = v;
  __syncthreads();
// ... 2 lines not shown
#pragma unroll
    for (int w = 0; w < BLOCK / 64; ++w) s += sh[w];
  }
  return s;
}

enum { PH_NONE = -1, PH_INIT = 0, PH_BICG_1, PH_BICG_2, PH_BICG_3, PH_CG_INIT, PH_CG_1, PH_CG_2, PH_BICG_S };

__device__ inline void end_of_iteration(double* sc) {
  const double rrw = sc[S_RED1], rr = sc[S_RED2];
  sc[S_PENDING3] = 0.0;
  sc[S_RR] = rrw;
  sc[S_ITERS] += 1.0;
  if (rrw <= sc[S_TOL2]) sc[S_DONE] = 1.0;
  else if (sc[S_RESTART] != 0.0) { sc[S_RHO] = rr; sc[S_RHAT2] = rr; }
}

__device__ inline void derive(int phase, double* sc) {
  const double r0 = sc[S_RED0], r1 = sc[S_RED1];
  switch (phase) {
    case PH_INIT: {
      const double bbw = r1, rrw = sc[S_RED2];
      sc[S_BB] = bbw; sc[S_RR] = rrw; sc[S_RHO] = r0; sc[S_RHO_OLD] = 1.0;
      sc[S_ALPHA] = 1.0; sc[S_OMEGA] = 1.0; sc[S_BETA] = 0.0; sc[S_ITERS] = 0.0;
      sc[S_RESTART] = 0.0; sc[S_RHAT2] = r0; sc[S_FORCE] = 0.0; sc[S_PENDING3] = 0.0;
      const double t2 = sc[S_RELTOL2] * bbw;
      sc[S_TOL2] = t2 > sc[S_ABSTOL2] ? t2 : sc[S_ABSTOL2];
      sc[S_DONE] = (rrw <= sc[S_TOL2]) ? 1.0 : 0.0;
      sc[S_RR0] = rrw;
      break;
    }
    case PH_CG_INIT: {
      sc[S_BB] = r1; sc[S_RR] = r0; sc[S_RHO] = r0; sc[S_RHO_OLD] = 1.0;
      sc[S_ALPHA] = 1.0; sc[S_OMEGA] = 1.0; sc[S_BETA] = 0.0; sc[S_ITERS] = 0.0;
      sc[S_RESTART] = 0.0; sc[S_RHAT2] = r0; sc[S_FORCE] = 0.0; sc[S_PENDING3] = 0.0;
      const double t2 = sc[S_RELTOL2] * r1;
      sc[S_TOL2] = t2 > sc[S_ABSTOL2] ? t2 : sc[S_ABSTOL2];
      sc[S_DONE] = (r1 <= sc[S_TOL2]) ? 1.0 : 0.0;
      sc[S_RRW] = r1;
      break;
    }
    case PH_BICG_1:
      if (sc[S_PENDING3] != 0.0) end_of_iteration(sc);
      if (sc[S_DONE] != 0.0) break;
      if (r0 == 0.0) { sc[S_ALPHA] = 0.0; sc[S_FORCE] = 1.0; } else sc[S_ALPHA] = sc[S_RHO] / r0;
      break;
    case PH_BICG_2: {
      const double ts = r0, tt = r1, rs = sc[S_RED2], ss = sc[S_RED3], rt = sc[S_RED4];
      const double omega = tt != 0.0 ? ts / tt : 0.0;
      const double rho_old = sc[S_RHO], rho_new = rs - omega * rt;
      double rr_pred = ss - 2.0 * omega * ts + omega * omega * tt;
      rr_pred = rr_pred > 0.0 ? rr_pred : 0.0;
      sc[S_OMEGA] = omega;
      sc[S_RHO_OLD] = rho_old;
      sc[S_RHO] = rho_new;
      if (omega == 0.0 || sc[S_FORCE] != 0.0 || rho_new * rho_new < 1e-20 * sc[S_RHAT2] * rr_pred) {
        sc[S_FORCE] = 0.0;
        sc[S_RESTART] = 1.0;
        sc[S_BETA] = 0.0;
      } else {
        sc[S_RESTART] = 0.0;
        sc[S_BETA] = (rho_new / rho_old) * (sc[S_ALPHA] / omega);
      }
      break;
    }
    case PH_BICG_3:
      if (sc[S_PENDING3] != 0.0) end_of_iteration(sc);
      break;
    case PH_BICG_S:
      if (sc[S_DONE] == 0.0 && sc[S_RED4] <= sc[S_TOL2]) {
        sc[S_RR] = sc[S_RED4];
        sc[S_ITERS] += 1.0;
        sc[S_PENDING3] = 0.0;
        sc[S_DONE] = 1.0;
        sc[S_HALF] = sc[S_ITERS];
      }
      break;
    case PH_CG_1:
      if (r0 == 0.0) sc[S_DONE] = 2.0; else sc[S_ALPHA] = sc[S_RR] / r0;
      break;
    case PH_CG_2: {
      const double rr_old = sc[S_RR];
      sc[S_RR] = r0;
      sc[S_RRW] = r1;
      sc[S_ITERS] += 1.0;
      if (r1 <= sc[S_TOL2]) sc[S_DONE] = 1.0;
      else sc[S_BETA] = r0 / rr_old;
      break;
    }
  }
}


__device__ inline void store_partial(double* p, double v) {
  __hip_atomic_store(reinterpret_cast<unsigned long long*>(p), (unsigned long long)__double_as_longlong(v), __ATOMIC_RELAXED,
                     __HIP_MEMORY_SCOPE_AGENT);
}
__device__ inline double load_partial(const double* p) {
  return __longlong_as_double((long long)__hip_atomic_load(reinterpret_cast<const unsigned long long*>(p), __ATOMIC_RELAXED,
                                                            __HIP_MEMORY_SCOPE_AGENT));
}

__device__ inline void put_partial(double* p, double v, int accum) { store_partial(p, accum ? v + load_partial(p) : v); }

__device__ inline bool last_block_arrives(unsigned* ticket, unsigned nblocks, double* sh ) {
  asm volatile("s_waitcnt vmcnt(0)" ::: "memory");
  __syncthreads();
  if (threadIdx.x == 0) {
    const unsigned t = __hip_atomic_fetch_add(ticket, 1u, __ATOMIC_RELAXED, __HIP_MEMORY_SCOPE_AGENT);
    const bool last = t == nblocks - 1;
    if (last) __hip_atomic_store(ticket, 0u, __ATOMIC_RELAXED, __HIP_MEMORY_SCOPE_AGENT);
    sh[0] = last ? 1.0 : 0.0;
  }
  __syncthreads();
  const bool last = sh[0] != 0.0;
  __syncthreads();
  return last;
}

struct FinArgs {
  unsigned* ticket;
  double* sc;
  int phase;
  int nslots;
  int do_derive;
  const double* dotx;
  double pc0 = 0.0, pc1 = 0.0;
  const double* base = nullptr;
  double pc2 = 0.0;
  float* p32 = nullptr;
  double psig = 0.0;
};

__device__ inline void fold_scalar_phase(const FinArgs& fin, const double* __restrict__ partials, double* s_red, int nparts) {
  if (!fin.ticket) return;
  if (!last_block_arrives(fin.ticket, gridDim.x, s_red)) return;
  for (int sl = 0; sl < fin.nslots; ++sl) {
    double a = 0.0;
    for (int i = threadIdx.x; i < nparts; i += BLOCK) a += load_partial(partials + (size_t)sl * nparts + i);
    const double t = block_sum(a, s_red);
    if (threadIdx.x == 0) fin.sc[S_RED0 + sl] = t;
  }
  if (threadIdx.x == 0 && fin.do_derive) derive(fin.phase, fin.sc);
}

bool launch_spmv(int mode, const CsrMatrix& A, const double* x, double* y, const double* aux, double* partials,
                 const double* sc, int grid, hipStream_t st, const FinArgs* fin = nullptr);
bool launch_spmv_as(int variant, int mode, const CsrMatrix& A, const double* x, double* y, const double* aux, double* partials,
                    const double* sc, int grid, hipStream_t st, const FinArgs* fin = nullptr);
enum { TYPED_FIRST = 1, TYPED_MIDDLE = 2, TYPED_HANDOVER = 3 };
void launch_spmv_typed(int kind, const CsrMatrix& A, const void* x, void* y, const double* sc, int grid, hipStream_t st,
                       const FinArgs& fin);
bool spmv_supports_typed_chain();
bool spmv_with_halo(int mode, const CsrMatrix& A, const Numbering& nb, const Slab& slab, double* x, double* y, const double* aux,
                    double* partials, const double* sc, int grid, hipStream_t st, const FinArgs* fin = nullptr);
void launch_spmv_variant(int variant, const CsrMatrix& A, const double* x, double* y, hipStream_t st);
void spmv_mode_compare(const CsrMatrix& A, i64 nv, int mode, double* max_abs_diff, double* max_abs, double* max_dot_rel);
int spmv_default_grid(i64 n);
bool spmv_supports_preconditioner_product();

}
```

### penguin/jl_amd/csrc/pg_spmv.hip

```cpp
#include <algorithm>
#include <cstdlib>
#include <thread>
#include <type_traits>
#include <vector>

#include "pg_host_algos.h"
#include "pg_krylov.h"
#include "pg_spmv.h"

namespace pg {
namespace {

constexpr int SPMV_ROWS = 256;
constexpr int SPMV_LDS_ENTRIES = 3584;

template <int MODE>
__global__ __launch_bounds__(BLOCK) void k_spmv(i64 n, const int* __restrict__ rowptr, const int* __restrict__ col,
                                                const double* __restrict__ val, const double* __restrict__ x,
                                                double* __restrict__ y, const double* __restrict__ aux,
                                                double* __restrict__ partials, const double* __restrict__ sc) {
  __shared__ double s_val[SPMV_LDS_ENTRIES];
  __shared__ int s_col[SPMV_LDS_ENTRIES];
  __shared__ double s_red[BLOCK / 64];
  if (sc && sc[S_DONE] != 0.0) return;
// ... 432 lines not shown
    a1[j] = xp.y;  a2[j] = xp_n;  ++j;
    a1[j] = xm.y;  a2[j] = xm_n;  ++j;
    a1[j] = xc.y;  a2[j] = xc_nx;
  }
  double s1 = 0.0, s2 = 0.0;
  int lo = rng & 255, hi = rng >> 8;
  if (EDGE) {
    const int nlo = einfo & 255, nhi = (einfo >> 8) & 255, e0 = (einfo >> 16) - e_first;
    const int elo = lo - nlo, ehi = hi + nhi, p1 = l2 + 1, p2 = l2 + 2;
    const bool g1 = p1 >= elo && p1 < ehi && !(p1 >= lo && p1 < hi), g2 = p2 >= elo && p2 < ehi && !(p2 >= lo && p2 < hi);
    const d2_t* q1 = g1 ? el + (e0 + (p1 - elo) - (p1 >= hi ? hi - lo : 0)) : cl;
    const d2_t* q2 = g2 ? el + (e0 + (p2 - elo) - (p2 >= hi ? hi - lo : 0)) : cl;
#pragma unroll
    for (int jp = 0; jp < (CNT + 1) / 2; ++jp) {
      const d2_t w1 = q1[64 * jp], w2 = q2[64 * jp];
      s1 += w1.x * a1[2 * jp];
      s2 += w2.x * a2[2 * jp];
      if (2 * jp + 1 < CNT) {
        s1 += w1.y * a1[2 * jp + 1];
        s2 += w2.y * a2[2 * jp + 1];
      }
    }
    lo = elo;
    hi = ehi;
  } else {
#pragma unroll
    for (int j = 0; j < CNT; ++j) { s1 += c[j] * a1[j]; s2 += c[j] * a2[j]; }
  }
  const double b1 = VT::P32 ? xc.y : sd.ax2.x, b2 = VT::P32 ? xc_nx : sd.ax2.y;
  s1 = mode_out<MODE>(s1, xc.y, b1, pc0, pc1, pc2);
  s2 = mode_out<MODE>(s2, xc_nx, b2, pc0, pc1, pc2);
  const bool nost = (dbg & 32) && s1 != 1.2345e-300;
  const bool allst = (dbg & 512) != 0;
  const bool v1 = ((l2 + 1 >= lo && l2 + 1 < hi) || allst) && !nost, v2 = ((l2 + 2 >= lo && l2 + 2 < hi) || allst) && !nost;
  if (VT::P32) {
    if (v1 && v2) store_pair_t(prow, psig * b1, psig * b2, false);
    else if (v1) store_one_t(prow, psig * b1);
    else if (v2) store_one_t(prow + 1, psig * b2);
  }
  if (v1 && v2) {
    store_pair_t(yrow, s1, s2, (dbg & 2048) != 0);
  } else if (v1) {
    store_one_t(yrow, s1);
  } else if (v2) {
    store_one_t(yrow + 1, s2);
  }
  if (MI::DOT0) {
    const double w1 = v1 ? s1 : 0.0, w2 = v2 ? s2 : 0.0;
    acc0 += (v1 ? sd.ax.x : 0.0) * w1 + (v2 ? sd.ax.y : 0.0) * w2;
    if (MI::DOT1) acc1 += w1 * w1 + w2 * w2;
    if (MI::DOT2) acc2 += (v1 ? sd.ax2.x : 0.0) * w1 + (v2 ? sd.ax2.y : 0.0) * w2;
  }
  return xc_nx;
}

template <int CNT, int MODE, bool EDGE, class VT, int KK, int Q0 = 0, int KTOT = KK>
__device__ __forceinline__ void march_unit(int rec, int lane, const typename VT::TX* __restrict__ x, typename VT::TY* __restrict__ y,
                                  const double* __restrict__ pa, const typename VT::TB* __restrict__ pb, double pc0, double pc1,
                                  double pc2, double& acc0, double& acc1, double& acc2, int dbg,
                                  const double* __restrict__ e_val, double* sv, double* sx, float* __restrict__ p32, double psig) {
  using MI = ModeInfo<MODE>;
  constexpr bool Y = CNT == 7;
  const int amask = (dbg & 128) ? ~1 : ~0;
  const int one = (dbg & 128) ? 0 : 1;
  const bool nolat = (dbg & 64) != 0;
  double c[CNT];
#pragma unroll
  for (int j = 0; j < CNT; ++j) c[j] = __hiloint2double(rlane(rec, 3 + 2 * j), rlane(rec, 2 + 2 * j));
  const int l2 = 2 * lane;
  int rb[KK];
  typedef typename PairOf<typename VT::TX>::type xpair_t;
  typedef typename PairOf<typename VT::TB>::type bpair_t;
  xpair_t ln[KK + 2];
  MarchSide<typename VT::TX, typename VT::TB> sd[KK];
  const bool act = lane < (rlane(rec, 0) >> 16);
  d2_t zero;
  zero.x = zero.y = 0.0;
  xpair_t xzero;
  xzero.x = xzero.y = 0;
  bpair_t bzero;
  bzero.x = bzero.y = 0;
#pragma unroll
  for (int q = 0; q < KK + 2; ++q) ln[q] = xzero;
#pragma unroll
  for (int q = 0; q < KK; ++q) {
    rb[q] = rlane(rec, 18 + 4 * (Q0 + q)) & amask;
    sd[q].ym = sd[q].yp = xzero;
    sd[q].ax = zero;
    sd[q].ax2 = bzero;
  }
  if (act) {
    ln[0] = load_raw<false>(x + (rlane(rec, Q0 == 0 ? 16 : 18 + 4 * (Q0 - 1)) & amask) + l2);
#pragma unroll
    for (int q = 0; q < KK; ++q) ln[q + 1] = load_raw<false>(x + rb[q] + l2);
    ln[KK + 1] = load_raw<false>(x + (rlane(rec, Q0 + KK == KTOT ? 17 : 18 + 4 * (Q0 + KK)) & amask) + l2);
#pragma unroll
    for (int q = 0; q < KK; ++q) {
      if (Y && !nolat) {
        sd[q].ym = load_raw<false>(x + rb[q] + (rlane(rec, 19 + 4 * (Q0 + q)) & amask) + l2 + one);
        sd[q].yp = load_raw<false>(x + rb[q] + (rlane(rec, 20 + 4 * (Q0 + q)) & amask) + l2 + one);
      }
      if (MI::HAS_A) sd[q].ax = load_pair<false>(pa + rb[q] + l2 + one);
      if (MI::HAS_B && !VT::P32) sd[q].ax2 = load_raw<false>(pb + rb[q] + l2 + one);
    }
  }
  const int e_first = rlane(rec, MARCH_EDGE + 2 + Q0) >> 16;
  const int e_cnt = (Q0 + KK == KTOT ? rlane(rec, MARCH_EDGE + 1) : rlane(rec, MARCH_EDGE + 2 + Q0 + KK) >> 16) - e_first;
  int elane = lane;
  if (EDGE) asm volatile("" : "+v"(elane));
  if (EDGE && e_cnt > 0) {
    const int e_all = rlane(rec, MARCH_EDGE + 1);
    const double* ep = e_val + (i64)MARCH_ESLOTS * rlane(rec, MARCH_EDGE) + 2 * (e_first + elane);
    asm volatile("s_waitcnt lgkmcnt(0)" ::: "memory");
    if (elane < e_cnt) {
#pragma unroll
      for (int jp = 0; jp < (CNT + 1) / 2; ++jp)
        __builtin_amdgcn_global_load_lds((const __attribute__((address_space(1))) void*)(ep + 2 * jp * e_all),
                                         (__attribute__((address_space(3))) void*)(sv + 128 * jp), 16, 0, 0);
    }
    asm volatile("s_waitcnt vmcnt(0)" ::: "memory");
  }
  if (EDGE) {
    const int k = elane - 2;
    if (k >= 0 && k < 2 * CNT) reinterpret_cast<int*>(sx)[256 * (k >> 2) + (k & 3)] = rec;
  }
  const d2_t* el = reinterpret_cast<const d2_t*>(sv);
  const d2_t* cl = reinterpret_cast<const d2_t*>(sx);
  double xm_n = lane_up((double)ln[0].x);
#pragma unroll
  for (int q = 0; q < KK; ++q)
    xm_n = march_plane<CNT, MODE, EDGE, VT>(c, rlane(rec, 21 + 4 * (Q0 + q)), l2, y + rb[q] + l2 + one, ln[q], xm_n, ln[q + 1], ln[q + 2], sd[q], pc0,
                                  pc1, pc2, acc0, acc1, acc2, dbg, rlane(rec, MARCH_EDGE + 2 + Q0 + q), e_first, el, cl,
                                  VT::P32 ? p32 + rb[q] + l2 + one : nullptr, psig);
}

template <int CNT, int MODE, bool EDGE, class VT>
__device__ __forceinline__ void march_dispatch(int rec, int lane, const typename VT::TX* __restrict__ x, typename VT::TY* __restrict__ y,
                                      const double* __restrict__ pa, const typename VT::TB* __restrict__ pb, double pc0, double pc1,
                                      double pc2, double& acc0, double& acc1, double& acc2, int dbg,
                                      const double* __restrict__ e_val, double* sv, double* sx, float* __restrict__ p32, double psig) {
  constexpr bool SPLIT = MODE == 3 && MARCH_K == 2 * MARCH_KS && PG_MARCH_SPLIT;
  if ((rlane(rec, 0) & 255) == MARCH_K) {
    if (SPLIT) {
      march_unit<CNT, MODE, EDGE, VT, MARCH_KS, 0, MARCH_K>(rec, lane, x, y, pa, pb, pc0, pc1, pc2, acc0, acc1, acc2, dbg, e_val, sv, sx, p32, psig);
      march_unit<CNT, MODE, EDGE, VT, MARCH_KS, MARCH_KS, MARCH_K>(rec, lane, x, y, pa, pb, pc0, pc1, pc2, acc0, acc1, acc2, dbg, e_val, sv, sx, p32, psig);
    } else {
      march_unit<CNT, MODE, EDGE, VT, MARCH_K>(rec, lane, x, y, pa, pb, pc0, pc1, pc2, acc0, acc1, acc2, dbg, e_val, sv, sx, p32, psig);
    }
  } else {
    march_unit<CNT, MODE, EDGE, VT, MARCH_KS>(rec, lane, x, y, pa, pb, pc0, pc1, pc2, acc0, acc1, acc2, dbg, e_val, sv, sx, p32, psig);
  }
}

template <int MODE, bool NT, bool DIAG, class VT = VecF64>
__global__ __launch_bounds__(BLOCK, 4) void k_spmv_s(i64 nslices, const int* __restrict__ srec,
                                                  const double* __restrict__ pval, const int* __restrict__ g_rowid,
                                                  const int* __restrict__ g_rowptr, const int* __restrict__ g_col,
                                                  const double* __restrict__ g_val, const typename VT::TX* __restrict__ x,
                                                  typename VT::TY* __restrict__ y, const double* __restrict__ aux,
                                                  double* __restrict__ partials, const double* __restrict__ sc, int xcd,
                                                  FinArgs fin, int pstride, int accum, const int* __restrict__ mrec,
                                                  i64 nunits, const int* __restrict__ tiles, int tpx,
                                                  const double* __restrict__ e_val) {
  __shared__ __attribute__((aligned(16))) double s_val[BLOCK / 64][512];
  __shared__ __attribute__((aligned(16))) double s_x[BLOCK / 64][512];
  __shared__ double s_red[BLOCK / 64];
  if (sc && sc[S_DONE] != 0.0) return;
  using MI = ModeInfo<MODE>;
  constexpr bool DOTS = MI::DOT0;
  static_assert(MODE == 8 || std::is_same<VT, VecF64>::value, "element types per stream exist for mode 8 only");
  const double* __restrict__ dx = fin.dotx ? fin.dotx : reinterpret_cast<const double*>(x);
  const double* __restrict__ pa = MODE == 1 ? aux : ((MODE == 2 || MODE == 3) ? dx : nullptr);
  const typename VT::TB* __restrict__ pb = reinterpret_cast<const typename VT::TB*>(MODE == 3 ? aux : (MODE == 8 ? fin.base : nullptr));
  float* __restrict__ p32 = VT::P32 ? fin.p32 : nullptr;
  const double psig = fin.psig;
  const int lane = threadIdx.x & 63;
  const int wave = __builtin_amdgcn_readfirstlane(threadIdx.x >> 6);
  double* __restrict__ sv = s_val[wave];
  double* __restrict__ sx = s_x[wave];
  d2_t* sv2 = reinterpret_cast<d2_t*>(sv);
  d2_t* sx2 = reinterpret_cast<d2_t*>(sx);
  double acc0 = 0.0, acc1 = 0.0, acc2 = 0.0;
  const int dbg = DIAG ? (xcd >> 8) : 0;
  xcd &= 255;
  xcd &= 1;
  const bool xsplit = xcd && gridDim.x >= 8;
  const int xid = xsplit ? (blockIdx.x & 7) : 0;
  const int woff = xsplit ? (int)(blockIdx.x >> 3) * (BLOCK / 64) + wave : (int)blockIdx.x * (BLOCK / 64) + wave;
  const int wstr = xsplit ? (int)(((i64)gridDim.x + 7 - xid) >> 3) * (BLOCK / 64) : (int)gridDim.x * (BLOCK / 64);
  const int* __restrict__ tb = tiles ? tiles + 2 * (tpx + 1) * xid : nullptr;
  const int ntile = tiles ? tpx : 1;
  const int l31 = lane & 31;
  for (int tile = 0; tile < ntile; ++tile) {
  i64 ulo, uhi, slo, shi, ubase, sbase;
  if (tiles) {
    ubase = tb[0]; sbase = tb[1];
    ulo = tb[2 * tile]; slo = tb[2 * tile + 1]; uhi = tb[2 * tile + 2]; shi = tb[2 * tile + 3];
  } else if (xsplit) {
    ubase = ulo = nunits * xid / 8; uhi = nunits * (xid + 1) / 8;
    sbase = slo = nslices * xid / 8; shi = nslices * (xid + 1) / 8;
  } else {
    ubase = ulo = 0; uhi = nunits;
    sbase = slo = 0; shi = nslices;
  }
  auto run_units = [&]() __attribute__((always_inline)) {
  if (nunits > 0) {
    int d = (woff - (int)(ulo - ubase)) % wstr;
    d = d < 0 ? d + wstr : d;
    i64 ucur = ulo + d;
    const i64 ustride = wstr;
    int urec = ucur < uhi ? mrec[(unsigned)(MARCH_REC * (int)ucur + lane)] : 0;
    for (; ucur < uhi; ucur += ustride) {
      const i64 un = ucur + ustride;
      const int urec_n = mrec[(unsigned)(MARCH_REC * (int)(un < uhi ? un : ucur) + lane)];
      if (!(dbg & 16)) {
        const bool edge = rlane(urec, MARCH_EDGE + 1) > 0;
        if (((rlane(urec, 0) >> 8) & 255) == 7) {
          if (edge) march_dispatch<7, MODE, true, VT>(urec, lane, x, y, pa, pb, fin.pc0, fin.pc1, fin.pc2, acc0, acc1, acc2, dbg, e_val, sv, sx, p32, psig);
          else march_dispatch<7, MODE, false, VT>(urec, lane, x, y, pa, pb, fin.pc0, fin.pc1, fin.pc2, acc0, acc1, acc2, dbg, e_val, sv, sx, p32, psig);
        } else {
          if (edge) march_dispatch<5, MODE, true, VT>(urec, lane, x, y, pa, pb, fin.pc0, fin.pc1, fin.pc2, acc0, acc1, acc2, dbg, e_val, sv, sx, p32, psig);
          else march_dispatch<5, MODE, false, VT>(urec, lane, x, y, pa, pb, fin.pc0, fin.pc1, fin.pc2, acc0, acc1, acc2, dbg, e_val, sv, sx, p32, psig);
        }
      }
      urec = urec_n;
    }
  }
  };
  auto run_slices = [&]() __attribute__((always_inline)) {
  int ds_ = (woff - (int)(slo - sbase)) % wstr;
  ds_ = ds_ < 0 ? ds_ + wstr : ds_;
  const i64 first = slo + ds_, wstride = wstr, hi = shi;
  const i64 lastc = hi - 1;
  int rec = first < hi ? srec[(unsigned)(SL_REC * (int)first + l31)] : 0;
  int rec_n = srec[(unsigned)(SL_REC * (int)(first + wstride < hi ? first + wstride : (first < hi ? lastc : 0)) + l31)];
  for (i64 chunk = first; chunk < hi; chunk += wstride) {
    const i64 cnn = chunk + 2 * wstride;
    const int rec_nn = srec[(unsigned)(SL_REC * (int)(cnn < hi ? cnn : lastc) + l31)];
    SDesc d;
    d.r0 = rlane(rec, 0); d.meta = rlane(rec, 1); d.base = rlane(rec, 2); d.aux = rlane(rec, 3);
    const int nrows = d.meta & 255, type = (d.meta >> 8) & 3, cnt = d.meta >> 16;
    const bool skip = ((dbg & 1) && type == SL_G) || ((dbg & 2) && type != SL_G);
    if (skip) {
    } else if (type == SL_U) {
      slice_dispatch<false, MODE, NT, VT>(cnt, d, nrows, rec, pval, x, y, pa, pb, lane, acc0, acc1, acc2, dbg, fin.pc0, fin.pc1, fin.pc2, p32, psig);
    } else if (type == SL_P) {
      slice_dispatch<true, MODE, NT, VT>(cnt, d, nrows, rec, pval, x, y, pa, pb, lane, acc0, acc1, acc2, dbg, fin.pc0, fin.pc1, fin.pc2, p32, psig);
    } else {
      Desc dd;
      dd.r0 = d.r0; dd.base = d.base; dd.r1 = d.r0 + nrows; dd.end = d.aux;
      StreamW q;
      stream_issue_w<NT>(q, dd, g_rowptr, g_col, g_val, lane);
      const bool live = lane < nrows;
      const int rid = g_rowid[d.r0 + (live ? lane : 0)];
      const int basev = dd.base & ~1, basec = dd.base & ~3;
      const int av = q.ra - basev, ac = q.ra - basec, len = q.rb - q.ra;
#pragma unroll
      for (int j = 0; j < XV_IT; ++j) sv2[lane + 64 * j] = q.v[j];
      const double opa = MI::HAS_A ? pa[rid] : 0.0, opb_ = (MI::HAS_B && !VT::P32) ? (double)pb[rid] : 0.0;
      const double xown = MI::OWN ? (double)x[rid] : 0.0;
      const double opb = VT::P32 ? xown : opb_;
      double xg[XC_IT][4];
#pragma unroll
      for (int j = 0; j < XC_IT; ++j) {
        xg[j][0] = (double)x[q.c[j].x]; xg[j][1] = (double)x[q.c[j].y]; xg[j][2] = (double)x[q.c[j].z]; xg[j][3] = (double)x[q.c[j].w];
      }
#pragma unroll
      for (int j = 0; j < XC_IT; ++j) {
        d2_t lo2, hi2;
        lo2.x = xg[j][0]; lo2.y = xg[j][1]; hi2.x = xg[j][2]; hi2.y = xg[j][3];
        sx2[2 * (lane + 64 * j)] = lo2;
        sx2[2 * (lane + 64 * j) + 1] = hi2;
      }
      __builtin_amdgcn_wave_barrier();
      double sum = 0.0;
      int maxlen = len;
#pragma unroll
      for (int off = 32; off > 0; off >>= 1) {
        const int other = __shfl_xor(maxlen, off, 64);
        maxlen = other > maxlen ? other : maxlen;
      }
      maxlen = __builtin_amdgcn_readfirstlane(maxlen);
      for (int j0 = 0; j0 < maxlen; j0 += GUNR) {
        double vv[GUNR], xv[GUNR];
#pragma unroll
        for (int j = 0; j < GUNR; ++j) {
          const int k = j0 + j < len ? j0 + j : 0;
          vv[j] = sv[av + k];
          xv[j] = sx[ac + k];
        }
#pragma unroll
        for (int j = 0; j < GUNR; ++j)
          if (j0 + j < len) sum += vv[j] * xv[j];
      }
      __builtin_amdgcn_wave_barrier();
      if (live) {
        sum = mode_out<MODE>(sum, xown, opb, fin.pc0, fin.pc1, fin.pc2);
        store_one_t(y + rid, sum);
        if (VT::P32) store_one_t(p32 + rid, psig * opb);
        if (MI::DOT0) acc0 += opa * sum;
        if (MI::DOT1) acc1 += sum * sum;
        if (MI::DOT2) acc2 += opb * sum;
      }
    }
    rec = rec_n;
    rec_n = rec_nn;
  }
  };
  if (DIAG && (dbg & 4096)) { run_slices(); run_units(); }
  else { run_units(); run_slices(); }
  }
  if (DOTS) {
    const double t0 = block_sum(acc0, s_red);
    if (threadIdx.x == 0) put_partial(partials + blockIdx.x, t0, accum);
  }
  if (MI::DOT1) {
    const double t1 = block_sum(acc1, s_red);
    if (threadIdx.x == 0) put_partial(partials + pstride + blockIdx.x, t1, accum);
  }
  if (MI::DOT2) {
    const double t2 = block_sum(acc2, s_red);
    if (threadIdx.x == 0) put_partial(partials + 4 * (size_t)pstride + blockIdx.x, t2, accum);
  }
  if (DOTS) fold_scalar_phase(fin, partials, s_red, pstride);
}

__global__ void k_row_same(i64 n, const int* __restrict__ rowptr, const int* __restrict__ col,
                           const double* __restrict__ val, unsigned char* __restrict__ flags) {
  for (i64 r = blockIdx.x * (i64)blockDim.x + threadIdx.x; r < n; r += (i64)gridDim.x * blockDim.x) {
    unsigned char f = 0;
    bool ghost = false;
    for (int k = rowptr[r]; k < rowptr[r + 1]; ++k) ghost = ghost || col[k] >= n;
    if (r > 0) {
      const int a = rowptr[r], b = rowptr[r + 1], pa = rowptr[r - 1];
      if (b - a == a - pa) {
        bool same = true, vsame = true;
        for (int k = 0; k < b - a; ++k) {
          same = same && (col[a + k] - 1 == col[pa + k]);
          vsame = vsame && (__double_as_longlong(val[a + k]) == __double_as_longlong(val[pa + k]));
        }
        f = same ? (vsame ? 3 : 1) : 0;
      }
    }
    flags[r] = f | (ghost ? 4 : 0);
  }
}

__global__ void k_pval_fill(i64 nslices, const int* __restrict__ srec, const int* __restrict__ rowptr,
                            const double* __restrict__ val, double* __restrict__ pval) {
  for (i64 sidx = blockIdx.x; sidx < nslices; sidx += gridDim.x) {
    const int r0 = srec[SL_REC * sidx], meta = srec[SL_REC * sidx + 1], base = srec[SL_REC * sidx + 2];
    if (((meta >> 8) & 3) != SL_P) continue;
    const int nrows = meta & 255, cnt = meta >> 16;
    for (int q = threadIdx.x; q < nrows * cnt; q += blockDim.x) {
      const int l = q / cnt, j = q % cnt;
      pval[(i64)base + (i64)j * nrows + l] = val[rowptr[r0 + l] + j];
    }
  }
}

__global__ void k_gpack(i64 ng, const int* __restrict__ g_rowid, const int* __restrict__ g_rowptr,
                        const int* __restrict__ rowptr, const int* __restrict__ col, const double* __restrict__ val,
                        int* __restrict__ g_col, double* __restrict__ g_val) {
  for (i64 q = blockIdx.x * (i64)blockDim.x + threadIdx.x; q < ng; q += (i64)gridDim.x * blockDim.x) {
    const int r = g_rowid[q], a = rowptr[r], len = rowptr[r + 1] - a, ga = g_rowptr[q];
    for (int k = 0; k < len; ++k) {
      g_col[ga + k] = col[a + k];
      if (g_val) g_val[ga + k] = val[a + k];
    }
  }
}

__global__ void k_fill_records(i64 nslices, int* __restrict__ srec, const int* __restrict__ rowptr,
                               const int* __restrict__ col, const double* __restrict__ val) {
  for (i64 q = blockIdx.x * (i64)blockDim.x + threadIdx.x; q < nslices; q += (i64)gridDim.x * blockDim.x) {
    int* rec = srec + SL_REC * q;
    const int type = (rec[1] >> 8) & 3;
    if (type == SL_G) continue;
    const int r = rec[0], a = rowptr[r], len = rowptr[r + 1] - a;
    for (int k = 0; k < SL_MAXCNT; ++k) {
      rec[4 + k] = col[a + (k < len ? k : 0)] - r;
      const double v = (k < len && type == SL_U) ? val[a + k] : 0.0;
      rec[12 + 2 * k] = __double2loint(v);
      rec[13 + 2 * k] = __double2hiint(v);
    }
  }
}

int variant() {
  return config().spmv_variant;
}

int xcd_map() {
  return config().spmv_xcd;
}

}
void ensure_csr_chunks(const CsrMatrix& A);
namespace {

#define PG_LAUNCH_C_ARGS(KERNEL, X, Y, AUX, PART)                                                               \
  hipLaunchKernelGGL(HIP_KERNEL_NAME(KERNEL), dim3(grid), dim3(BLOCK), 0, st, A.n, A.nchunks, A.chunk_desc.p, \
                     A.rowptr.p, A.col.p, A.val.p, X, Y, AUX, PART, (const double*)nullptr)
#define PG_LAUNCH_C(KERNEL)                                                                                    \
  hipLaunchKernelGGL(HIP_KERNEL_NAME(KERNEL), dim3(grid), dim3(BLOCK), 0, st, A.n, A.nchunks, A.chunk_desc.p, \
                     A.rowptr.p, A.col.p, A.val.p, x, y, aux, partials, sc)

template <int MODE>
bool launch_slices(int v, const CsrMatrix& A, i64 s0, i64 ns, const double* x, double* y, const double* aux, double* partials,
                   const double* sc, int grid, int pstride, int accum, hipStream_t st, const FinArgs* fin, bool units = true) {
  FinArgs fa{nullptr, nullptr, PH_NONE, 0, 0, nullptr};
  if (fin && MODE >= 1) fa = *fin;
  const int* rec = A.srec.p + SL_REC * s0;
  const i64 nu = units ? A.nunits : 0;
  const bool tiled = units && A.tiles_per_xcd > 0 && s0 == 0 && ns == A.tile_ns && (xcd_map() & 1) && grid >= 8;
  const int* tiles = tiled ? (const int*)A.tiles.p : nullptr;
  const int tpx = tiled ? A.tiles_per_xcd : 0;
  if (xcd_map() >= 256)
    hipLaunchKernelGGL(HIP_KERNEL_NAME(k_spmv_s<MODE, true, true>), dim3(grid), dim3(BLOCK), 0, st, ns, rec, A.pval.p,
                       A.g_rowid.p, A.g_rowptr.p, A.g_col.p, A.g_val.p, x, y, aux, partials, sc, xcd_map(), fa, pstride, accum,
                       (const int*)A.mrec.p, nu, tiles, tpx, (const double*)A.e_val.p);
  else if (v & 4)
    hipLaunchKernelGGL(HIP_KERNEL_NAME(k_spmv_s<MODE, true, false>), dim3(grid), dim3(BLOCK), 0, st, ns, rec, A.pval.p,
                       A.g_rowid.p, A.g_rowptr.p, A.g_col.p, A.g_val.p, x, y, aux, partials, sc, xcd_map(), fa, pstride, accum,
                       (const int*)A.mrec.p, nu, tiles, tpx, (const double*)A.e_val.p);
  else
    hipLaunchKernelGGL(HIP_KERNEL_NAME(k_spmv_s<MODE, false, false>), dim3(grid), dim3(BLOCK), 0, st, ns, rec, A.pval.p,
                       A.g_rowid.p, A.g_rowptr.p, A.g_col.p, A.g_val.p, x, y, aux, partials, sc, xcd_map(), fa, pstride, accum,
                       (const int*)A.mrec.p, nu, tiles, tpx, (const double*)A.e_val.p);
  return fa.ticket != nullptr;
}

template <int MODE>
bool launch_mode(int v, const CsrMatrix& A, const double* x, double* y, const double* aux, double* partials,
                 const double* sc, int grid, hipStream_t st, const FinArgs* fin) {
  if (v & 64) return launch_slices<MODE>(v, A, 0, A.nslices, x, y, aux, partials, sc, grid, grid, 0, st, fin);
  PG_REQUIRE(MODE != 8 && !(fin && fin->dotx), "the preconditioner products and separate dot operands need the slice kernel");
  if (v != 1) ensure_csr_chunks(A);
  if (v == 1) {
    hipLaunchKernelGGL(HIP_KERNEL_NAME(k_spmv<MODE>), dim3(grid), dim3(BLOCK), 0, st, A.n, A.rowptr.p, A.col.p, A.val.p, x, y,
                       aux, partials, sc);
    return false;
  }
  if (v & 4) PG_LAUNCH_C((k_spmv_cw<MODE, true>));
  else PG_LAUNCH_C((k_spmv_cw<MODE, false>));
  return false;
}

template <class VT>
void launch_typed(const CsrMatrix& A, const void* x, void* y, const double* sc, int grid, hipStream_t st, const FinArgs& fin) {
  const bool tiled = A.tiles_per_xcd > 0 && A.nslices == A.tile_ns && (xcd_map() & 1) && grid >= 8;
  hipLaunchKernelGGL(HIP_KERNEL_NAME(k_spmv_s<8, true, false, VT>), dim3(grid), dim3(BLOCK), 0, st, A.nslices, (const int*)A.srec.p,
                     (const double*)A.pval.p, (const int*)A.g_rowid.p, (const int*)A.g_rowptr.p, (const int*)A.g_col.p,
                     (const double*)A.g_val.p, static_cast<const typename VT::TX*>(x), static_cast<typename VT::TY*>(y),
                     (const double*)nullptr, (double*)nullptr, sc, xcd_map(), fin, grid, 0, (const int*)A.mrec.p, A.nunits,
                     tiled ? (const int*)A.tiles.p : (const int*)nullptr, tiled ? A.tiles_per_xcd : 0, (const double*)A.e_val.p);
}

}

bool spmv_supports_typed_chain() { return (variant() & 64) != 0 && (variant() & 4) != 0 && xcd_map() < 256; }

void launch_spmv_typed(int kind, const CsrMatrix& A, const void* x, void* y, const double* sc, int grid, hipStream_t st,
                       const FinArgs& fin) {
  if (A.n == 0) return;
  PG_REQUIRE(spmv_supports_typed_chain() && A.srec.p, "typed Horner launches need the slice kernel with the stream hint (PG_SPMV_VARIANT 70)");
  PG_REQUIRE(!fin.ticket && fin.base, "typed Horner launch: a base operand and no scalar phase");
  if (kind == TYPED_FIRST) {
    PG_REQUIRE(fin.p32 && x == (const void*)fin.base, "typed Horner launch (first): x = base and a p32 output");
    launch_typed<VecTypes<double, double, float, true>>(A, x, y, sc, grid, st, fin);
  } else if (kind == TYPED_MIDDLE) {
    launch_typed<VecTypes<float, float, float, false>>(A, x, y, sc, grid, st, fin);
  } else {
    PG_REQUIRE(kind == TYPED_HANDOVER, "unknown typed Horner launch");
    launch_typed<VecTypes<float, double, double, false>>(A, x, y, sc, grid, st, fin);
  }
}


namespace {

struct Slice {
  int r0, meta, base, aux;
  int key;
  int bnd;
  i64 okey = 0;
};

using pghost::MRun;

constexpr int RUN_INFO = 25;

__global__ void k_run_info(i64 nruns, const int* __restrict__ run_r0, const int* __restrict__ rowptr,
                           const int* __restrict__ col, const double* __restrict__ val, const int* __restrict__ cell,
                           const int* __restrict__ map, int* __restrict__ out) {
  for (i64 q = blockIdx.x * (i64)blockDim.x + threadIdx.x; q < nruns; q += (i64)gridDim.x * blockDim.x) {
    const int r = run_r0[q], a = rowptr[r], len = rowptr[r + 1] - a;
    out[RUN_INFO * q + 24] = cell ? cell[map ? map[r] : r] : -1;
    for (int k = 0; k < 8; ++k) {
      out[RUN_INFO * q + k] = k < len ? col[a + k] - r : 0;
      const double v = k < len ? val[a + k] : 0.0;
      out[RUN_INFO * q + 8 + 2 * k] = __double2loint(v);
      out[RUN_INFO * q + 9 + 2 * k] = __double2hiint(v);
    }
  }
}

__global__ void k_fill_units(i64 nunits, int* __restrict__ mrec, const int* __restrict__ rowptr,
                             const double* __restrict__ val) {
  for (i64 q = blockIdx.x * (i64)blockDim.x + threadIdx.x; q < nunits; q += (i64)gridDim.x * blockDim.x) {
    int* rec = mrec + MARCH_REC * q;
    const int cnt = (rec[0] >> 8) & 255, a = rowptr[rec[1]];
    for (int k = 0; k < cnt; ++k) {
      rec[2 + 2 * k] = __double2loint(val[a + k]);
      rec[3 + 2 * k] = __double2hiint(val[a + k]);
    }
  }
}

__global__ void k_fill_edges(i64 ne, const int* __restrict__ meta, const int* __restrict__ rowptr, const double* __restrict__ val,
                             double* __restrict__ e_val) {
  for (i64 q = blockIdx.x * (i64)blockDim.x + threadIdx.x; q < ne; q += (i64)gridDim.x * blockDim.x) {
    const int r = meta[4 * q], dst = meta[4 * q + 1], dist = meta[4 * q + 2], sm = meta[4 * q + 3];
    const int a = rowptr[r], len = sm >> 24;
    for (int j = 0; j < MARCH_ESLOTS; ++j) e_val[dst + (i64)(j >> 1) * dist + (j & 1)] = 0.0;
    for (int k = 0; k < len; ++k) {
      const int j = (sm >> (3 * k)) & 7;
      e_val[dst + (i64)(j >> 1) * dist + (j & 1)] = val[a + k];
    }
  }
}

__global__ void k_edges_invalid(i64 ne, const int* __restrict__ meta, const int* __restrict__ rowptr_t, const int* __restrict__ col_t,
                                const int* __restrict__ rowptr, const int* __restrict__ col, unsigned long long* __restrict__ out) {
  unsigned long long c = 0;
  for (i64 q = blockIdx.x * (i64)blockDim.x + threadIdx.x; q < ne; q += (i64)gridDim.x * blockDim.x) {
    const int r = meta[4 * q], a = rowptr[r], at = rowptr_t[r], len = rowptr[r + 1] - a;
    bool same = len == rowptr_t[r + 1] - at && len == (meta[4 * q + 3] >> 24);
    for (int k = 0; same && k < len; ++k) same = col[a + k] == col_t[at + k];
    c += same ? 0 : 1;
  }
  if (c) atomicAdd(out, c);
}

__global__ void k_units_invalid(i64 nunits, const int* __restrict__ mrec, const int* __restrict__ rowptr,
                                const double* __restrict__ val, const unsigned char* __restrict__ flags,
                                unsigned long long* __restrict__ out) {
  unsigned long long c = 0;
  for (i64 q = blockIdx.x; q < nunits; q += gridDim.x) {
    const int* rec = mrec + MARCH_REC * q;
    const int K = rec[0] & 255, cnt = (rec[0] >> 8) & 255, a0 = rowptr[rec[1]];
    for (int i = 0; i < K; ++i) {
      const int rb = rec[18 + 4 * i], lo = rec[21 + 4 * i] & 255, hi = rec[21 + 4 * i] >> 8;
      for (int l = lo + threadIdx.x; l < hi; l += blockDim.x) {
        const int r = rb + l;
        if (l > lo) {
          c += (flags[r] & 3) != 3 ? 1 : 0;
        } else {
          const int a = rowptr[r];
          bool same = rowptr[r + 1] - a == cnt;
          for (int k = 0; same && k < cnt; ++k)
            same = __double_as_longlong(val[a + k]) == __double_as_longlong(val[a0 + k]);
          c += same ? 0 : 1;
        }
      }
    }
  }
  if (c) atomicAdd(out, c);
}

__global__ void k_row_cells(i64 nrows, const int* __restrict__ rows, const int* __restrict__ cell, const int* __restrict__ map,
                            int* __restrict__ out) {
  for (i64 q = blockIdx.x * (i64)blockDim.x + threadIdx.x; q < nrows; q += (i64)gridDim.x * blockDim.x) {
    const int r = rows[q];
    out[q] = cell[map ? map[r] : r];
  }
}

int march_strip() {
  return config().spmv_strip;
}
bool has_geo(const CsrMatrix& A) { return A.geo_cell && A.geo_ext0 > 0 && A.geo_lines > 0 && march_strip() > 0; }

std::vector<i64> row_orders(const CsrMatrix& A, const std::vector<int>& rows) {
  std::vector<i64> ord(rows.size(), 0);
  if (!has_geo(A) || rows.empty()) return ord;
  const i64 nr = (i64)rows.size();
  DevBuf<int> d_rows(nr), d_cells(nr);
  d_rows.upload(rows.data(), nr);
  hipLaunchKernelGGL(k_row_cells, dim3(grid_for(nr, 256)), dim3(256), 0, ctx().stream, nr, d_rows.p, A.geo_cell, A.geo_map, d_cells.p);
  PG_HIP(hipGetLastError());
  std::vector<int> cells(rows.size());
  d_cells.download(cells.data(), nr);
  for (i64 q = 0; q < nr; ++q) ord[q] = pghost::march_order(cells[q], A.geo_ext0, A.geo_lines, march_strip());
  return ord;
}

void emit_u_rows(std::vector<Slice>& up, i64 a, i64 b, int cnt) {
  for (i64 r = a; r < b; r += SL_MAXROWS_U) {
    const int rows = (int)std::min<i64>(SL_MAXROWS_U, b - r);
    up.push_back(Slice{(int)r, rows | (SL_U << 8) | (cnt << 16), 0, 0, (int)r, 0});
  }
}

void build_march_units(CsrMatrix& A, const std::vector<MRun>& runs, std::vector<int>& mrec, std::vector<Slice>& up,
                       std::vector<i64>& ukeys, pghost::EdgePlan* edges) {
  A.rows_m = 0;
  const i64 nr = (i64)runs.size();
  if (nr == 0) return;
  hipStream_t st = ctx().stream;
  std::vector<int> info((size_t)RUN_INFO * nr);
// ... 118 lines not shown
    for (auto& pt : parts) {
      up.insert(up.end(), pt.up.begin(), pt.up.end());
      grows.insert(grows.end(), pt.grows.begin(), pt.grows.end());
      runs.insert(runs.end(), pt.runs.begin(), pt.runs.end());
      A.rows_u += pt.rows_u; A.rows_p += pt.rows_p; A.nnz_p += pt.nnz_p;
    }
  }
  laps.lap("    slices: host classification");
  std::vector<int> mrec;
  std::vector<i64> ukeys;
  pghost::EdgePlan edges;
  std::vector<int> c_ptr, c_col;
  if (!runs.empty() && !grows.empty() && config().spmv_edges) {
    const i64 nc = (i64)grows.size();
    c_ptr.assign(nc + 1, 0);
    for (i64 q = 0; q < nc; ++q) c_ptr[q + 1] = c_ptr[q] + (rp[grows[q] + 1] - rp[grows[q]]);
    c_col.resize((size_t)c_ptr[nc] + 1);
    DevBuf<int> d_rows(nc), d_ptr(nc + 1), d_col(c_ptr[nc] + 8);
    d_rows.upload(grows.data(), nc);
    d_ptr.upload(c_ptr.data(), nc + 1);
    hipLaunchKernelGGL(k_gpack, dim3(grid_for(nc, 256)), dim3(256), 0, st, nc, d_rows.p, d_ptr.p, A.rowptr.p, A.col.p, A.val.p,
                       d_col.p, (double*)nullptr);
    PG_HIP(hipGetLastError());
    if (c_ptr[nc] > 0) d_col.download(c_col.data(), c_ptr[nc]);
    edges.cand = pghost::EdgeCands{grows.data(), nc, c_ptr.data(), c_col.data()};
  }
  build_march_units(A, runs, mrec, up, ukeys, &edges);
  A.rows_e = edges.rows_e;
  A.e_slots = edges.slots_read;
  A.e_meta.alloc(std::max<i64>((i64)edges.meta.size(), 1));
  A.e_val.alloc((i64)MARCH_ESLOTS * A.rows_e + 8);
  A.e_val.zero();
  if (A.rows_e > 0) {
    A.e_meta.upload(edges.meta.data(), (i64)edges.meta.size());
    hipLaunchKernelGGL(k_fill_edges, dim3(grid_for(A.rows_e, 256)), dim3(256), 0, st, A.rows_e, (const int*)A.e_meta.p, A.rowptr.p,
                       A.val.p, A.e_val.p);
    PG_HIP(hipGetLastError());
    std::vector<int> er((size_t)A.rows_e);
    for (i64 q = 0; q < A.rows_e; ++q) er[q] = edges.meta[4 * q];
    std::sort(er.begin(), er.end());
    size_t w = 0;
    for (size_t q = 0; q < grows.size(); ++q)
      if (!std::binary_search(er.begin(), er.end(), grows[q])) grows[w++] = grows[q];
    grows.resize(w);
  }
  A.nunits = (i64)mrec.size() / MARCH_REC;
  A.mrec.alloc(std::max<i64>((i64)mrec.size(), 1));
  if (!mrec.empty()) A.mrec.upload(mrec.data(), (i64)mrec.size());
  laps.lap("    slices: marching units");
  {
    i64 pbase = 0;
    for (auto& sl : up) {
      if (((sl.meta >> 8) & 3) != SL_P) continue;
      const int rows = sl.meta & 255, cnt = sl.meta >> 16;
      PG_REQUIRE(pbase + (i64)rows * cnt < (i64)2147483647, "P-slice value array exceeds int32 indexing");
      sl.base = (int)pbase;
      pbase += (i64)rows * cnt;
    }
  }
  A.pval.alloc(A.nnz_p + 8);
  std::vector<i64> g_ord = row_orders(A, grows);
  if (has_geo(A) && !grows.empty()) {
    std::vector<i64> uniq(g_ord);
    std::sort(uniq.begin(), uniq.end());
    uniq.erase(std::unique(uniq.begin(), uniq.end()), uniq.end());
    std::vector<i64> start(uniq.size() + 1, 0);
    std::vector<int> bucket(grows.size());
    for (size_t q = 0; q < grows.size(); ++q) {
      bucket[q] = (int)(std::lower_bound(uniq.begin(), uniq.end(), g_ord[q]) - uniq.begin());
      ++start[bucket[q] + 1];
    }
    for (size_t b = 0; b < uniq.size(); ++b) start[b + 1] += start[b];
    std::vector<int> sorted(grows.size());
    std::vector<i64> sorted_ord(grows.size());
    for (size_t q = 0; q < grows.size(); ++q) {
      const i64 pos = start[bucket[q]]++;
      sorted[pos] = grows[q];
      sorted_ord[pos] = g_ord[q];
    }
    grows.swap(sorted);
    g_ord.swap(sorted_ord);
  }
  {
    std::vector<std::pair<int, i64>> both(grows.size());
    for (size_t q = 0; q < grows.size(); ++q) both[q] = {grows[q], g_ord[q]};
    std::stable_partition(both.begin(), both.end(), [&](const std::pair<int, i64>& e) { return (fl[e.first] & 4) == 0; });
    for (size_t q = 0; q < grows.size(); ++q) { grows[q] = both[q].first; g_ord[q] = both[q].second; }
  }
  const i64 ng = (i64)grows.size();
  i64 ng_int = 0;
  while (ng_int < ng && (fl[grows[ng_int]] & 4) == 0) ++ng_int;
  A.rows_g = ng;
  std::vector<int> grp(ng + 1, 0);
  for (i64 q = 0; q < ng; ++q) grp[q + 1] = grp[q] + (rp[grows[q] + 1] - rp[grows[q]]);
  A.nnz_g = grp[ng];
  A.g_rowid.alloc(ng > 0 ? ng : 1);
  A.g_rowptr.alloc(ng + 1);
  A.g_col.alloc(A.nnz_g + 8);
  A.g_val.alloc(A.nnz_g + 8);
  A.g_col.zero();
  A.g_val.zero();
  A.g_rowptr.upload(grp.data(), ng + 1);
  {
    std::vector<int> firsts(up.size());
    for (size_t q = 0; q < up.size(); ++q) firsts[q] = up[q].key;
    const std::vector<i64> ord = row_orders(A, firsts);
    for (size_t q = 0; q < up.size(); ++q) up[q].okey = ord[q] * ((i64)1 << 32) + up[q].key;
  }
  std::vector<Slice> all(up);
  if (ng > 0) {
    A.g_rowid.upload(grows.data(), ng);
    hipLaunchKernelGGL(k_gpack, dim3(grid_for(ng, 256)), dim3(256), 0, st, ng, A.g_rowid.p, A.g_rowptr.p, A.rowptr.p, A.col.p,
                       A.val.p, A.g_col.p, A.g_val.p);
    PG_HIP(hipGetLastError());
    i64 q = 0;
    while (q < ng) {
      i64 e = q + 1;
      PG_REQUIRE(grp[e] - grp[q] <= SPMV_CHUNK_ENTRIES, "CSR row longer than an SpMV chunk");
      const i64 stop = q < ng_int ? ng_int : ng;
      while (e < stop && e - q < 64 && grp[e + 1] - grp[q] <= SPMV_CHUNK_ENTRIES) ++e;
      all.push_back(Slice{(int)q, (int)(e - q) | (SL_G << 8), grp[q], grp[e], grows[q], q >= ng_int ? 1 : 0,
                          g_ord[q] * ((i64)1 << 32) + grows[q]});
      q = e;
    }
  }
  std::stable_sort(all.begin(), all.end(), [](const Slice& a, const Slice& b) { return a.bnd != b.bnd ? a.bnd < b.bnd : a.okey < b.okey; });
  A.nslices = (i64)all.size();
  A.nslices_int = 0;
  while (A.nslices_int < A.nslices && !all[A.nslices_int].bnd) ++A.nslices_int;
  {
    const int tile_units = config().spmv_tile_units;
    const i64 T = tile_units > 0 ? std::min<i64>(256, (A.nunits / 8 + tile_units / 2) / tile_units) : 0;
    A.tiles_per_xcd = 0;
    A.tile_ns = 0;
    A.tiles.release();
    if (T >= 2 && A.nslices_int > 0 && (i64)ukeys.size() == A.nunits) {
      std::vector<i64> skeys((size_t)A.nslices_int);
      for (i64 q = 0; q < A.nslices_int; ++q) skeys[q] = all[q].okey;
      std::vector<int> tab;
      pghost::plan_tiles(ukeys, skeys, (int)T, tab);
      A.tiles.alloc((i64)tab.size());
      A.tiles.upload(tab.data(), (i64)tab.size());
      A.tiles_per_xcd = (int)T;
      A.tile_ns = A.nslices_int;
    }
  }
  std::vector<int> sd(SL_REC * (A.nslices + 1), 0);
  for (i64 q = 0; q < A.nslices; ++q) {
    int* rec = sd.data() + SL_REC * q;
    rec[0] = all[q].r0; rec[1] = all[q].meta; rec[2] = all[q].base; rec[3] = all[q].aux;
  }
  A.srec.alloc((i64)sd.size());
  A.srec.upload(sd.data(), (i64)sd.size());
  if (A.nslices > 0) {
    hipLaunchKernelGGL(k_fill_records, dim3(grid_for(A.nslices, 256)), dim3(256), 0, st, A.nslices, A.srec.p, A.rowptr.p, A.col.p,
                       A.val.p);
    PG_HIP(hipGetLastError());
  }
  if (A.nnz_p > 0) {
    hipLaunchKernelGGL(k_pval_fill, dim3((unsigned)std::min<i64>(A.nslices, 65535)), dim3(256), 0, st, A.nslices, A.srec.p,
                       A.rowptr.p, A.val.p, A.pval.p);
    PG_HIP(hipGetLastError());
  }
  PG_HIP(hipStreamSynchronize(st));
  laps.lap("    slices: packing + records");
  A.spmv_bytes = 4 * SL_REC * A.nslices + 4 * MARCH_REC * A.nunits + 8 * A.nnz_p + 12 * A.nnz_g + 8 * ng + 8 * A.e_slots + 16 * n;
  if (config().debug)
    fprintf(stderr, "[pg_spmv] slices %lld (%lld wait for the halo), marching units %lld (%lld rows, %lld edge rows): rows U %lld P %lld G %lld of %lld; nnz P %lld G %lld of %lld; bytes/launch %lld (CSR %lld)\n",
            (long long)A.nslices, (long long)(A.nslices - A.nslices_int), (long long)A.nunits, (long long)A.rows_m, (long long)A.rows_e, (long long)A.rows_u, (long long)A.rows_p, (long long)A.rows_g,
            (long long)n, (long long)A.nnz_p, (long long)A.nnz_g, (long long)A.nnz, (long long)A.spmv_bytes,
            (long long)(12 * A.nnz + 20 * n));
}

}

void ensure_csr_chunks(const CsrMatrix& Ac) {
  CsrMatrix& A = const_cast<CsrMatrix&>(Ac);
  if (A.chunk_desc.p || A.n == 0) return;
  std::vector<int> rp(A.n + 1);
  A.rowptr.download(rp.data(), A.n + 1);
  std::vector<int> cd;
  cd.reserve(2 * (A.n / 60 + 16));
  i64 r = 0;
  while (r < A.n) {
    i64 e = r + 1;
    PG_REQUIRE(rp[e] - rp[r] <= SPMV_CHUNK_ENTRIES, "CSR row longer than an SpMV chunk");
    while (e < A.n && e - r < 64 && rp[e + 1] - rp[r] <= SPMV_CHUNK_ENTRIES) ++e;
    cd.push_back((int)r);
    cd.push_back(rp[r]);
    r = e;
  }
  A.nchunks = (i64)cd.size() / 2;
  cd.push_back((int)A.n);
  cd.push_back(rp[A.n]);
  cd.push_back((int)A.n);
  cd.push_back(rp[A.n]);
  A.chunk_desc.alloc((i64)cd.size());
  A.chunk_desc.upload(cd.data(), (i64)cd.size());
}

void build_spmv_chunks(CsrMatrix& A) {
  Laps laps;
  int* rp = static_cast<int*>(pinned_scratch(0, sizeof(int) * (size_t)(A.n + 1)));
  A.rowptr.download(rp, A.n + 1);
  laps.lap("    chunks: rowptr download");
  A.chunk_desc.release();
  A.nchunks = 0;
  build_slices(A, rp);
}

__global__ void k_slices_invalid(i64 nslices, const int* __restrict__ srec, const unsigned char* __restrict__ flags,
                                 unsigned long long* __restrict__ out) {
  unsigned long long c = 0;
  for (i64 q = blockIdx.x; q < nslices; q += gridDim.x) {
    const int r0 = srec[SL_REC * q], meta = srec[SL_REC * q + 1];
    const int nrows = meta & 255, type = (meta >> 8) & 3;
    const unsigned char need = type == SL_U ? 3 : 1;
    for (int l = 1 + threadIdx.x; l < nrows; l += blockDim.x) c += (flags[r0 + l] & need) != need ? 1 : 0;
  }
  if (c) atomicAdd(out, c);
}

template <class T>
static void clone_buf(DevBuf<T>& dst, const DevBuf<T>& src, hipStream_t st) {
  dst.alloc(src.n > 0 ? src.n : 1);
  if (src.n > 0) PG_HIP(hipMemcpyAsync(dst.p, src.p, sizeof(T) * (size_t)src.n, hipMemcpyDeviceToDevice, st));
}

bool build_slices_like(const CsrMatrix& T, CsrMatrix& A) {
  hipStream_t st = ctx().stream;
  const i64 n = A.n;
  if (!T.rowflags.p || T.n != n || !T.srec.p) return false;
  A.rowflags.alloc(n);
  DevBuf<unsigned long long> diff(1);
  diff.zero();
  hipLaunchKernelGGL(k_row_same, dim3(grid_for(n, 256, 256 * 16)), dim3(256), 0, st, n, A.rowptr.p, A.col.p, A.val.p,
                     A.rowflags.p);
  if (T.nslices > 0)
    hipLaunchKernelGGL(k_slices_invalid, dim3((unsigned)std::min<i64>(T.nslices, 16384)), dim3(64), 0, st, T.nslices, T.srec.p,
                       A.rowflags.p, diff.p);
  if (T.nunits > 0)
    hipLaunchKernelGGL(k_units_invalid, dim3((unsigned)std::min<i64>(T.nunits, 16384)), dim3(64), 0, st, T.nunits, T.mrec.p,
                       A.rowptr.p, A.val.p, A.rowflags.p, diff.p);
  if (T.rows_e > 0)
    hipLaunchKernelGGL(k_edges_invalid, dim3(grid_for(T.rows_e, 256)), dim3(256), 0, st, T.rows_e, (const int*)T.e_meta.p,
                       (const int*)T.rowptr.p, (const int*)T.col.p, (const int*)A.rowptr.p, (const int*)A.col.p, diff.p);
  PG_HIP(hipGetLastError());
  unsigned long long h = 0;
  diff.download(&h, 1);
  if (h != 0) return false;
  A.chunk_desc.release();
  A.nchunks = 0;
  A.nslices = T.nslices;
  A.nslices_int = T.nslices_int;
  A.rows_u = T.rows_u; A.rows_p = T.rows_p; A.rows_g = T.rows_g; A.nnz_p = T.nnz_p; A.nnz_g = T.nnz_g;
  A.spmv_bytes = T.spmv_bytes;
  A.nunits = T.nunits; A.rows_m = T.rows_m;
  A.tiles_per_xcd = T.tiles_per_xcd; A.tile_ns = T.tile_ns;
  if (T.tiles_per_xcd > 0) clone_buf(A.tiles, T.tiles, st);
  else A.tiles.release();
  clone_buf(A.mrec, T.mrec, st);
  if (A.nunits > 0)
    hipLaunchKernelGGL(k_fill_units, dim3(grid_for(A.nunits, 256)), dim3(256), 0, st, A.nunits, A.mrec.p, A.rowptr.p, A.val.p);
  A.rows_e = T.rows_e; A.e_slots = T.e_slots;
  clone_buf(A.e_meta, T.e_meta, st);
  A.e_val.alloc((i64)MARCH_ESLOTS * A.rows_e + 8);
  A.e_val.zero();
  if (A.rows_e > 0)
    hipLaunchKernelGGL(k_fill_edges, dim3(grid_for(A.rows_e, 256)), dim3(256), 0, st, A.rows_e, (const int*)A.e_meta.p, A.rowptr.p,
                       A.val.p, A.e_val.p);
  clone_buf(A.srec, T.srec, st);
  clone_buf(A.g_rowid, T.g_rowid, st);
  clone_buf(A.g_rowptr, T.g_rowptr, st);
  A.pval.alloc(A.nnz_p + 8);
  A.g_col.alloc(A.nnz_g + 8);
  A.g_val.alloc(A.nnz_g + 8);
  A.g_col.zero();
  A.g_val.zero();
  if (A.nslices > 0)
    hipLaunchKernelGGL(k_fill_records, dim3(grid_for(A.nslices, 256)), dim3(256), 0, st, A.nslices, A.srec.p, A.rowptr.p, A.col.p,
                       A.val.p);
  if (A.nnz_p > 0)
    hipLaunchKernelGGL(k_pval_fill, dim3((unsigned)std::min<i64>(A.nslices, 65535)), dim3(256), 0, st, A.nslices, A.srec.p,
                       A.rowptr.p, A.val.p, A.pval.p);
  if (A.rows_g > 0)
    hipLaunchKernelGGL(k_gpack, dim3(grid_for(A.rows_g, 256)), dim3(256), 0, st, A.rows_g, A.g_rowid.p, A.g_rowptr.p, A.rowptr.p,
                       A.col.p, A.val.p, A.g_col.p, A.g_val.p);
  PG_HIP(hipGetLastError());
  PG_HIP(hipStreamSynchronize(st));
  return true;
}

bool spmv_supports_preconditioner_product() { return (variant() & 64) != 0; }

int spmv_default_grid(i64 n) {
  const int per_cu = config().spmv_blocks_per_cu > 0 ? config().spmv_blocks_per_cu : ((variant() & 64) ? 4 : 6);
  static int cus = 0;
  if (cus == 0) {
    hipDeviceProp_t prop;
    cus = 256;
    if (hipGetDeviceProperties(&prop, ctx().device) == hipSuccess && prop.multiProcessorCount > 0) cus = prop.multiProcessorCount;
  }
  return grid_for(n, BLOCK, cus * per_cu);
}

static inline __attribute__((always_inline)) bool launch_by_mode(int v, int mode, const CsrMatrix& A, const double* x, double* y,
                                                                 const double* aux, double* partials, const double* sc, int grid,
                                                                 hipStream_t st, const FinArgs* fin) {
  if (mode == 0) return launch_mode<0>(v, A, x, y, aux, partials, sc, grid, st, fin);
  if (mode == 1) return launch_mode<1>(v, A, x, y, aux, partials, sc, grid, st, fin);
  if (mode == 2) return launch_mode<2>(v, A, x, y, aux, partials, sc, grid, st, fin);
  if (mode == 8) return launch_mode<8>(v, A, x, y, aux, partials, sc, grid, st, fin);
  PG_REQUIRE(mode == 3, "unknown SpMV launch mode");
  return launch_mode<3>(v, A, x, y, aux, partials, sc, grid, st, fin);
}

bool launch_spmv(int mode, const CsrMatrix& A, const double* x, double* y, const double* aux, double* partials,
                 const double* sc, int grid, hipStream_t st, const FinArgs* fin) {
  if (A.n == 0) return false;
  return launch_by_mode(variant(), mode, A, x, y, aux, partials, sc, grid, st, fin);
}

bool launch_spmv_as(int v, int mode, const CsrMatrix& A, const double* x, double* y, const double* aux, double* partials,
                    const double* sc, int grid, hipStream_t st, const FinArgs* fin) {
  if (A.n == 0) return false;
  return launch_by_mode(v, mode, A, x, y, aux, partials, sc, grid, st, fin);
}

bool spmv_with_halo(int mode, const CsrMatrix& A, const Numbering& nb, const Slab& slab, double* x, double* y, const double* aux,
                    double* partials, const double* sc, int grid, hipStream_t st, const FinArgs* fin) {
  if (A.n == 0 || !A.halo_needed) {
    if (A.halo_needed) halo_exchange(nb, slab, x, st);
    return launch_spmv(mode, A, x, y, aux, partials, sc, grid, st, fin);
  }
  const int v = variant();
  const bool overlap = config().halo_overlap;
  const i64 ni = A.nslices_int, nbnd = A.nslices - A.nslices_int;
  if (!(v & 64) || !overlap || (ni == 0 && A.nunits == 0) || nbnd == 0) {
    halo_exchange(nb, slab, x, st);
    return launch_spmv(mode, A, x, y, aux, partials, sc, grid, st, fin);
  }
  const int grid2 = (int)std::max<i64>(1, std::min<i64>(grid, (nbnd + BLOCK / 64 - 1) / (BLOCK / 64)));
  halo_begin(nb, slab, x, st);
  bool folded;
  FinArgs fin_nofold{nullptr, nullptr, PH_NONE, 0, 0, fin ? fin->dotx : nullptr};
  if (fin) { fin_nofold.pc0 = fin->pc0; fin_nofold.pc1 = fin->pc1; fin_nofold.pc2 = fin->pc2; fin_nofold.base = fin->base; }
#define PG_SPLIT(MODE_)                                                                                              \
  launch_slices<MODE_>(v, A, 0, ni, x, y, aux, partials, sc, grid, grid, 0, st, fin ? &fin_nofold : nullptr);      \
  halo_end(st);                                                                                                      \
  folded = launch_slices<MODE_>(v, A, ni, nbnd, x, y, aux, partials, sc, grid2, grid, 1, st, fin, false)
  if (mode == 0) { PG_SPLIT(0); }
  else if (mode == 1) { PG_SPLIT(1); }
  else if (mode == 2) { PG_SPLIT(2); }
  else if (mode == 8) { PG_SPLIT(8); }
  else { PG_REQUIRE(mode == 3, "unknown SpMV launch mode"); PG_SPLIT(3); }
#undef PG_SPLIT
  return folded;
}

namespace {

__global__ void k_hash_vector(i64 n, unsigned long long seed, double* x) {
  for (i64 i = blockIdx.x * (i64)blockDim.x + threadIdx.x; i < n; i += (i64)gridDim.x * blockDim.x) {
    unsigned long long h = ((unsigned long long)i + seed) * 0x9E3779B97F4A7C15ull + 0x632BE59BD9B4E019ull;
    h ^= h >> 29; h *= 0xBF58476D1CE4E5B9ull; h ^= h >> 32;
    x[i] = (double)(h >> 11) * (1.0 / 9007199254740992.0) - 0.5;
  }
}

template <int MODE>
__global__ void k_mode_epilogue(i64 n, double* __restrict__ y, const double* __restrict__ x, const double* __restrict__ b, double pc0,
                                double pc1, double pc2) {
  for (i64 i = blockIdx.x * (i64)blockDim.x + threadIdx.x; i < n; i += (i64)gridDim.x * blockDim.x)
    y[i] = mode_out<MODE>(y[i], x[i], b[i], pc0, pc1, pc2);
}

template <int MODE>
void mode_compare(const CsrMatrix& A, i64 nv, double* max_abs_diff, double* max_abs, double* max_dot_rel) {
  hipStream_t st = ctx().stream;
  const i64 n = A.n;
  const int grid = spmv_default_grid(n);
  DevBuf<double> x(nv), aux(nv), base(nv), ya(n), yb(n), pa(5 * (i64)grid), pb(5 * (i64)grid);
  hipLaunchKernelGGL(k_hash_vector, dim3(grid_for(nv, BLOCK)), dim3(BLOCK), 0, st, nv, 0ull, x.p);
  hipLaunchKernelGGL(k_hash_vector, dim3(grid_for(nv, BLOCK)), dim3(BLOCK), 0, st, nv, 0x5851F42D4C957F2Dull, aux.p);
  hipLaunchKernelGGL(k_hash_vector, dim3(grid_for(nv, BLOCK)), dim3(BLOCK), 0, st, nv, 0x14057B7EF767814Full, base.p);
  pa.zero();
  pb.zero();
  FinArgs fin{nullptr, nullptr, PH_NONE, 0, 0, nullptr};
  fin.pc0 = 0.75; fin.pc1 = -0.4375; fin.pc2 = 1.25;
  fin.base = base.p;
  launch_slices<MODE>(70, A, 0, A.nslices, x.p, ya.p, aux.p, pa.p, nullptr, grid, grid, 0, st, MODE == 8 ? &fin : nullptr);
  ensure_csr_chunks(A);
  if (MODE == 8) {
    PG_LAUNCH_C_ARGS((k_spmv_cw<0, true>), x.p, yb.p, aux.p, pb.p);
    hipLaunchKernelGGL(HIP_KERNEL_NAME(k_mode_epilogue<MODE>), dim3(grid_for(n, BLOCK)), dim3(BLOCK), 0, st, n, yb.p,
                       (const double*)x.p, (const double*)base.p, fin.pc0, fin.pc1, fin.pc2);
  } else {
    PG_LAUNCH_C_ARGS((k_spmv_cw<(MODE == 8 ? 0 : MODE), true>), x.p, yb.p, aux.p, pb.p);
  }
  PG_HIP(hipGetLastError());
  std::vector<double> ha(n), hb(n), qa(5 * (size_t)grid), qb(5 * (size_t)grid);
  ya.download(ha.data(), n);
  yb.download(hb.data(), n);
  pa.download(qa.data(), 5 * (i64)grid);
  pb.download(qb.data(), 5 * (i64)grid);
  *max_abs_diff = *max_abs = *max_dot_rel = 0.0;
  for (i64 i = 0; i < n; ++i) {
    *max_abs_diff = std::max(*max_abs_diff, std::fabs(ha[i] - hb[i]));
    *max_abs = std::max(*max_abs, std::fabs(ha[i]));
  }
  const int slots[3] = {0, 1, 4};
  const int nslot = MODE == 1 ? 1 : (MODE == 3 ? 3 : 0);
  for (int k = 0; k < nslot; ++k) {
    double a = 0.0, b = 0.0;
    for (int i = 0; i < grid; ++i) { a += qa[(size_t)slots[k] * grid + i]; b += qb[(size_t)slots[k] * grid + i]; }
    *max_dot_rel = std::max(*max_dot_rel, std::fabs(a - b) / std::max(std::fabs(b), 1e-300));
  }
}

}

void spmv_mode_compare(const CsrMatrix& A, i64 nv, int mode, double* max_abs_diff, double* max_abs, double* max_dot_rel) {
  *max_abs_diff = *max_abs = *max_dot_rel = 0.0;
  if (A.n == 0) return;
// ... 14 lines not shown
```

### penguin/jl_amd/csrc/pg_system.h

```cpp
#pragma once
#include <vector>

#include "pg_stencil.h"

namespace pg {

struct SpecEst {
  bool tried = false;
  bool admitted = false;
  int steps = 0;
  double g_ritz = 0.0, g_used = 0.0;
  double re_min = 0.0, re_max = 0.0, im_max = 0.0;
  double ms = 0.0;
  std::vector<double> H;
};

struct Numbering {
  int K = 2;
  i64 Mloc = 0;
  i64 n_own = 0, n_ghost = 0;
  i64 cnt_own[MAX_KINDS] = {0, 0, 0, 0}, off_own[MAX_KINDS] = {0, 0, 0, 0};
  i64 cntL[MAX_KINDS] = {0, 0, 0, 0}, offL[MAX_KINDS] = {0, 0, 0, 0};
  i64 cntU[MAX_KINDS] = {0, 0, 0, 0}, offU[MAX_KINDS] = {0, 0, 0, 0};
  i64 sendL_off[MAX_KINDS] = {0, 0, 0, 0}, sendL_cnt[MAX_KINDS] = {0, 0, 0, 0};
  i64 sendU_off[MAX_KINDS] = {0, 0, 0, 0}, sendU_cnt[MAX_KINDS] = {0, 0, 0, 0};
  DevBuf<int> red;
  DevBuf<int> row_cell;
  i64 n_vec() const { return n_own + n_ghost; }
  int kind_of_row(i64 r) const {
    int k = 0;
    while (k + 1 < K && r >= off_own[k + 1]) ++k;
    return k;
  }
};

struct CsrMatrix {
  i64 n = 0, nnz = 0;
  int scheme = -1;
  DevBuf<int> rowptr, col;
  DevBuf<double> val;
  DevBuf<double> ds;
  DevBuf<int> chunk_desc;
  i64 nchunks = 0;
  DevBuf<int> srec;
  DevBuf<double> pval;
  DevBuf<int> g_rowid, g_rowptr, g_col;
  DevBuf<double> g_val;
  DevBuf<int> mrec;
  i64 nunits = 0, rows_m = 0;
  DevBuf<int> e_meta;
  DevBuf<double> e_val;
  i64 rows_e = 0, e_slots = 0;
  DevBuf<int> tiles;
  int tiles_per_xcd = 0;
  i64 tile_ns = 0;
  const int* geo_cell = nullptr;
  const int* geo_map = nullptr;
  i64 geo_ext0 = 0, geo_lines = 0;
  bool want_units = true;
  i64 nslices = 0;
  i64 nslices_int = 0;
  DevBuf<unsigned char> rowflags;
  i64 rows_u = 0, rows_p = 0, rows_g = 0, nnz_p = 0, nnz_g = 0;
  i64 spmv_bytes = 0;
  bool halo_needed = true;
  bool poly_ok = false;
  double gersh = 0.0;
  SpecEst est;
  bool poly_gave_up = false;
  i64 n_blk = 0;
  i64 nnz_raw = 0;
  DevBuf<int> blk_rows, blk_idx;
  DevBuf<double> blk_coef, blk_cn, blk_fw;
  DevBuf<unsigned char> isblk;
  DevBuf<int> blk_pos;
};
inline void poly_record_stagnation(const CsrMatrix& A) {
  CsrMatrix& M = const_cast<CsrMatrix&>(A);
  M.poly_ok = false;
  M.est.admitted = false;
  M.poly_gave_up = true;
}
constexpr int SPMV_CHUNK_ENTRIES = 508;
void build_spmv_chunks(CsrMatrix& A);

void build_numbering(const SysParams& P, const Slab& slab, Numbering& nb);
void assemble_csr(const SysParams& P, const Slab& slab, const Numbering& nb, CsrMatrix& A, bool scale = true);
void assemble_csr_preconditioned(const SysParams& P, const Slab& slab, const Numbering& nb, CsrMatrix& A,
                                 const bool* inherit_halo = nullptr);
void assemble_csr_like(const SysParams& P, const Slab& slab, const Numbering& nb, const CsrMatrix& T, CsrMatrix& A);
bool build_slices_like(const CsrMatrix& T, CsrMatrix& A);
void decide_poly(CsrMatrix& A);
void apply_left(const CsrMatrix& A, const double* in, double* out, hipStream_t st);
void apply_rows_padded(const SysParams& P, const Slab& slab, const double* x, double* y);

}
```

Before: 1376.

## Add dynamic per-XCD work hand-out for slice SpMV kernel

Adds a dynamic hand-out path to the slice SpMV kernel for modes 0 and 8. Workgroups draw unit and slice tickets from per-XCD atomic counters, held in double-buffered head sets that each launch resets for the next one. A second mode (the default, 2) passes a 'rung' flag to the non-dynamic kernel instead, which changes how work is handed out statically. The aim is to even out load imbalance and tail effects across workgroups. In exchange it adds atomic traffic, an extra kernel argument and a per-matrix state buffer, plus debug entry points that timestamp waves.

```diff
diff --git a/include/penguin_hip.h b/include/penguin_hip.h
--- a/include/penguin_hip.h
+++ b/include/penguin_hip.h
@@ -370,6 +370,10 @@
 #define PG_DEBUG_SPMV_SENTINEL_F32 0x7FC5EED0u
 int32_t pg_debug_spmv_apply_typed(pg_solver* s, int32_t which, int32_t kind, const void* x, const void* base, double pc0, double pc1,
                                   double pc2, double sigma, int32_t done, double* y64, float* y32, float* p32);
+int32_t pg_debug_spmv_handout(pg_solver* s, int32_t which, int32_t kind, int32_t handout, int32_t grid, int32_t repeat, const void* x,
+                              const void* base, double pc0, double pc1, double pc2, double sigma, double* y64, float* y32, float* p32);
+int32_t pg_debug_spmv_wave_stamps(pg_solver* s, int32_t which, int32_t handout, int32_t grid, int32_t reps, uint64_t* stamps,
+                                  double* avg_us);
 int32_t pg_debug_read_probe(int64_t bytes, int32_t elem_bytes, int32_t nt, int32_t blocks, int32_t reps, double* gbs);
 int32_t pg_debug_run_virtual_ranks(int32_t nranks, int32_t N, const int64_t* n, const double* L, int32_t body_kind,
                                    const double* params, int32_t nparams, double interface_value, double border_value,
diff --git a/penguin/jl_amd/_lib.py b/penguin/jl_amd/_lib.py
--- a/penguin/jl_amd/_lib.py
+++ b/penguin/jl_amd/_lib.py
@@ -373,3 +373,40 @@
                                           C.c_double(pc[0]), C.c_double(pc[1]), C.c_double(pc[2]), C.c_double(sigma), C.c_int32(done),
                                           ptr(y64), ptr(y32), ptr(p32)))
     return {"y": y64 if kind == TYPED_HANDOVER else y32, "p32": p32}
+
+
+def debug_spmv_handout(handle, which: int, kind: int, handout: int, x, base=None, pc=(0.0, 0.0, 0.0), sigma: float = 1.0,
+                       grid: int = 0, repeat: int = 1) -> dict:
+    n, nv, _, _ = debug_spmv_sizes(handle, which)
+    want_x = np.float64 if kind in (0, 8, TYPED_FIRST) else np.float32
+    want_b = {0: None, 8: np.float64, TYPED_FIRST: None, TYPED_MIDDLE: np.float32, TYPED_HANDOVER: np.float64}[kind]
+    x = np.ascontiguousarray(x)
+    if x.dtype != want_x or x.size != nv:
+        raise ValueError(f"debug_spmv_handout: x must be {nv} x {np.dtype(want_x).name}")
+    if (base is None) != (want_b is None):
+        raise ValueError("debug_spmv_handout: base goes with kinds 8, 2 and 3, and only with them")
+    bp = None
+    if base is not None:
+        base = np.ascontiguousarray(base)
+        if base.dtype != want_b or base.size != n:
+            raise ValueError(f"debug_spmv_handout: base must be {n} x {np.dtype(want_b).name}")
+        bp = base.ctypes.data_as(C.c_void_p)
+    f64out = kind in (0, 8, TYPED_HANDOVER)
+    y64 = np.zeros(n + DEBUG_SPMV_GUARD) if f64out else None
+    y32 = np.zeros(n + DEBUG_SPMV_GUARD, dtype=np.float32) if not f64out else None
+    p32 = np.zeros(n + DEBUG_SPMV_GUARD, dtype=np.float32) if kind == TYPED_FIRST else None
+    ptr = lambda a: None if a is None else a.ctypes.data_as(C.c_void_p)
+    check(lib().pg_debug_spmv_handout(handle, C.c_int32(which), C.c_int32(kind), C.c_int32(handout), C.c_int32(grid),
+                                      C.c_int32(repeat), x.ctypes.data_as(C.c_void_p), bp, C.c_double(pc[0]), C.c_double(pc[1]),
+                                      C.c_double(pc[2]), C.c_double(sigma), ptr(y64), ptr(y32), ptr(p32)))
+    return {"y": y64 if f64out else y32, "p32": p32}
+
+
+def debug_spmv_wave_stamps(handle, which: int, handout: int, grid: int = 0, reps: int = 50):
+    n, _, _, g = debug_spmv_sizes(handle, which)
+    g = grid if grid > 0 else g
+    st = np.zeros((4 * g, 4), dtype=np.uint64)
+    us = C.c_double()
+    check(lib().pg_debug_spmv_wave_stamps(handle, C.c_int32(which), C.c_int32(handout), C.c_int32(grid), C.c_int32(reps),
+                                          st.ctypes.data_as(C.c_void_p), C.byref(us)))
+    return st, us.value
diff --git a/penguin/jl_amd/csrc/pg_common.h b/penguin/jl_amd/csrc/pg_common.h
--- a/penguin/jl_amd/csrc/pg_common.h
+++ b/penguin/jl_amd/csrc/pg_common.h
@@ -87,6 +87,7 @@
   bool spmv_edges = true;
   int spmv_tile_units = 0;
   int spmv_blocks_per_cu = 0;
+  int spmv_handout = 2;
   bool halo_overlap = true;
   int guess_n = 4;
   int guess_depth = 7;
diff --git a/penguin/jl_amd/csrc/pg_context.hip b/penguin/jl_amd/csrc/pg_context.hip
--- a/penguin/jl_amd/csrc/pg_context.hip
+++ b/penguin/jl_amd/csrc/pg_context.hip
@@ -60,6 +60,7 @@
     k.spmv_edges = geti("PG_SPMV_EDGES", 1) != 0;
     k.spmv_tile_units = (int)geti("PG_SPMV_TILE_UNITS", 0);
     k.spmv_blocks_per_cu = (int)geti("PG_SPMV_BLOCKS_PER_CU", 0);
+    k.spmv_handout = (int)std::max<long long>(0, std::min<long long>(2, geti("PG_SPMV_HANDOUT", 2)));
     k.halo_overlap = geti("PG_HALO_OVERLAP", 1) != 0;
     k.speculate_product = geti("PG_SPECULATE", 1) != 0;
     k.guess_n = (int)std::max<long long>(0, std::min<long long>(4, geti("PG_GUESS_STATES", 4)));
@@ -368,11 +369,11 @@
   char tmp[1024];
   snprintf(tmp, sizeof(tmp),
            "spmv_variant=%d spmv_xcd=%d spmv_strip=%d spmv_unit_order=%d spmv_march=%d spmv_edges=%d spmv_march_k=%d spmv_minrun=%d spmv_tile_units=%d "
-           "spmv_blocks_per_cu=%d halo_overlap=%d speculate=%d poly=%d poly_degree=%d poly_adapt=%d "
+           "spmv_blocks_per_cu=%d spmv_handout=%d halo_overlap=%d speculate=%d poly=%d poly_degree=%d poly_adapt=%d "
            "poly_margin=%g poly_slack=%g poly_hist=%d poly_trend=%d poly_maxdeg=%d poly_f32=%d poly_f32_tail=%d gamma_elim=%d diag_elim=%d "
            "guess_states=%d guess_depth=%d guess_defer=%d step_fuse=%d async_alloc=%d cache_limit_mb=%lld alloc_poison=%d alloc_guard=%d profile_sample=%d debug=%d",
            k.spmv_variant, k.spmv_xcd, k.spmv_strip, k.unit_order, (int)k.spmv_march, (int)k.spmv_edges, k.spmv_march_k, k.spmv_minrun, k.spmv_tile_units,
-           k.spmv_blocks_per_cu, (int)k.halo_overlap, (int)k.speculate_product, (int)k.poly, k.poly_degree, (int)k.poly_adapt,
+           k.spmv_blocks_per_cu, k.spmv_handout, (int)k.halo_overlap, (int)k.speculate_product, (int)k.poly, k.poly_degree, (int)k.poly_adapt,
            k.poly_margin, k.poly_slack, k.poly_hist, (int)k.poly_trend, k.poly_maxdeg, (int)k.poly_f32, k.poly_f32_tail,
            (int)k.gamma_elim, (int)k.diag_elim, k.guess_n, k.guess_depth, (int)k.guess_defer, (int)k.step_fuse, k.async_alloc, k.pool_limit_mb, k.alloc_poison, k.alloc_guard, k.profile_sample, (int)k.debug);
   if (buf && n > 0) {
diff --git a/penguin/jl_amd/csrc/pg_solver.hip b/penguin/jl_amd/csrc/pg_solver.hip
--- a/penguin/jl_amd/csrc/pg_solver.hip
+++ b/penguin/jl_amd/csrc/pg_solver.hip
@@ -3661,6 +3661,117 @@
   PG_API_END
 }
 
+int32_t pg_debug_spmv_handout(pg_solver* s, int32_t which, int32_t kind, int32_t handout, int32_t grid, int32_t repeat, const void* x,
+                              const void* base, double pc0, double pc1, double pc2, double sigma, double* y64, float* y32, float* p32) {
+  PG_API_BEGIN
+  require_init();
+  PG_REQUIRE(s && x, "pg_debug_spmv_handout: NULL argument");
+  PG_REQUIRE(ctx().nranks == 1 && !ctx().comm, "pg_debug_spmv_handout: one rank");
+  PG_REQUIRE(kind == 0 || kind == 8 || kind == TYPED_FIRST || kind == TYPED_MIDDLE || kind == TYPED_HANDOVER,
+             "pg_debug_spmv_handout: kinds 0 (mode 0), 8 (mode 8, fp64), 1 / 2 / 3 (typed mode 8: first, middle, hand-over)");
+  PG_REQUIRE(handout >= 0 && handout <= 2, "pg_debug_spmv_handout: hand-out 0, 1 or 2");
+  PG_REQUIRE(repeat >= 1 && repeat <= 64, "pg_debug_spmv_handout: 1 .. 64 launches");
+  const bool f64out = kind == 0 || kind == 8 || kind == TYPED_HANDOVER;
+  PG_REQUIRE(f64out ? (y64 && !y32) : (y32 && !y64), "pg_debug_spmv_handout: y64 for kinds 0, 8 and 3, y32 for kinds 1 and 2");
+  PG_REQUIRE((kind == TYPED_FIRST) == (p32 != nullptr), "pg_debug_spmv_handout: p32 is the first typed launch's output, and only its");
+  PG_REQUIRE((kind == 8 || kind == TYPED_MIDDLE || kind == TYPED_HANDOVER) == (base != nullptr),
+             "pg_debug_spmv_handout: kinds 8, 2 and 3 take a base (the first typed launch's base is its x)");
+  PG_REQUIRE(spmv_supports_typed_chain(), "pg_debug_spmv_handout: the slice kernel with the stream hint only");
+  i64 nv = 0;
+  const CsrMatrix& A = debug_matrix(s, which, &nv);
+  const i64 n = A.n;
+  PG_REQUIRE(n > 0 && A.srec.p, "pg_debug_spmv_handout: the matrix has no rows or no slice image");
+  nv = std::max(nv, n);
+  PG_REQUIRE(grid <= 65536, "pg_debug_spmv_handout: grid too large");
+  const int g = grid > 0 ? grid : spmv_default_grid(n);
+  hipStream_t st = ctx().stream;
+  constexpr i64 GUARD = 64;
+  double sentinel;
+  const unsigned long long sbits = PG_DEBUG_SPMV_SENTINEL;
+  std::memcpy(&sentinel, &sbits, sizeof(double));
+  float sentinel32;
+  const unsigned sbits32 = PG_DEBUG_SPMV_SENTINEL_F32;
+  std::memcpy(&sentinel32, &sbits32, sizeof(float));
+  const bool x64 = kind == 0 || kind == 8 || kind == TYPED_FIRST;
+  DevBuf<double> dx64(nv), db64(nv), dy64(n + GUARD);
+  DevBuf<float> dx32(nv), db32(nv), dy32(n + GUARD), dp32(n + GUARD);
+  db64.zero(); db32.zero();
+  if (x64) dx64.upload(static_cast<const double*>(x), nv);
+  else dx32.upload(static_cast<const float*>(x), nv);
+  if (kind == TYPED_MIDDLE) db32.upload(static_cast<const float*>(base), n);
+  if (kind == 8 || kind == TYPED_HANDOVER) db64.upload(static_cast<const double*>(base), n);
+  {
+    std::vector<double> f64((size_t)(n + GUARD), sentinel);
+    std::vector<float> f32((size_t)(n + GUARD), sentinel32);
+    dy64.upload(f64.data(), n + GUARD);
+    dy32.upload(f32.data(), n + GUARD);
+    dp32.upload(f32.data(), n + GUARD);
+  }
+  FinArgs f{nullptr, nullptr, PH_NONE, 0, 0, nullptr};
+  f.pc0 = pc0; f.pc1 = pc1; f.pc2 = pc2;
+  struct Unforce { ~Unforce() { spmv_force_handout(-1); } } unforce;
+  spmv_force_handout(handout);
+  for (int r = 0; r < repeat; ++r) {
+    if (kind == 0) {
+      launch_spmv_as(70, 0, A, dx64.p, dy64.p, nullptr, nullptr, nullptr, g, st, nullptr);
+    } else if (kind == 8) {
+      f.base = db64.p;
+      launch_spmv_as(70, 8, A, dx64.p, dy64.p, nullptr, nullptr, nullptr, g, st, &f);
+    } else if (kind == TYPED_FIRST) {
+      f.base = dx64.p; f.p32 = dp32.p; f.psig = sigma;
+      launch_spmv_typed(kind, A, dx64.p, dy32.p, nullptr, g, st, f);
+    } else if (kind == TYPED_MIDDLE) {
+      f.base = reinterpret_cast<const double*>(db32.p);
+      launch_spmv_typed(kind, A, dx32.p, dy32.p, nullptr, g, st, f);
+    } else {
+      f.base = db64.p;
+      launch_spmv_typed(kind, A, dx32.p, dy64.p, nullptr, g, st, f);
+    }
+  }
+  PG_HIP(hipGetLastError());
+  if (y64) dy64.download(y64, n + GUARD);
+  if (y32) dy32.download(y32, n + GUARD);
+  if (p32) dp32.download(p32, n + GUARD);
+  PG_API_END
+}
+
+int32_t pg_debug_spmv_wave_stamps(pg_solver* s, int32_t which, int32_t handout, int32_t grid, int32_t reps, uint64_t* stamps,
+                                  double* avg_us) {
+  PG_API_BEGIN
+  require_init();
+  PG_REQUIRE(s && stamps && reps >= 1, "pg_debug_spmv_wave_stamps: bad arguments");
+  PG_REQUIRE(ctx().nranks == 1 && !ctx().comm, "pg_debug_spmv_wave_stamps: one rank");
+  PG_REQUIRE(handout >= 0 && handout <= 2, "pg_debug_spmv_wave_stamps: hand-out 0, 1 or 2");
+  i64 nv = 0;
+  const CsrMatrix& A = debug_matrix(s, which, &nv);
+  const i64 n = A.n;
+  PG_REQUIRE(n > 0 && A.srec.p, "pg_debug_spmv_wave_stamps: the matrix has no rows or no slice image");
+  nv = std::max(nv, n);
+  PG_REQUIRE(grid <= 65536, "pg_debug_spmv_wave_stamps: grid too large");
+  const int g = grid > 0 ? grid : spmv_default_grid(n);
+  hipStream_t st = ctx().stream;
+  std::vector<float> hx((size_t)nv), hb((size_t)nv);
+  for (i64 i = 0; i < nv; ++i) { hx[i] = 0.5f + 0.25f * (float)((i * 37) % 101) / 101.0f; hb[i] = 1.0f - 0.5f * (float)((i * 13) % 89) / 89.0f; }
+  DevBuf<float> dx(nv), dy(nv), db(nv);
+  DevBuf<unsigned long long> dst(4 * (i64)(BLOCK / 64) * g);
+  dx.upload(hx.data(), nv);
+  dy.upload(hx.data(), nv);
+  db.upload(hb.data(), nv);
+  dst.zero();
+  EventPair ev;
+  spmv_stamped_launches(A, handout, dx.p, dy.p, db.p, 1.0, -0.5, 0.5, g, 3, st, dst.p);
+  PG_HIP(hipEventRecord(ev.e0, st));
+  spmv_stamped_launches(A, handout, dx.p, dy.p, db.p, 1.0, -0.5, 0.5, g, reps, st, dst.p);
+  PG_HIP(hipEventRecord(ev.e1, st));
+  PG_HIP(hipEventSynchronize(ev.e1));
+  float ms = 0.f;
+  PG_HIP(hipEventElapsedTime(&ms, ev.e0, ev.e1));
+  if (avg_us) *avg_us = 1e3 * ms / reps;
+  static_assert(sizeof(unsigned long long) == sizeof(uint64_t), "stamp words");
+  dst.download(reinterpret_cast<unsigned long long*>(stamps), 4 * (i64)(BLOCK / 64) * g);
+  PG_API_END
+}
+
 __global__ void k_scale_rows(i64 n_e, const int* __restrict__ elist, double factor, double* __restrict__ z) {
   for (i64 q = blockIdx.x * (i64)blockDim.x + threadIdx.x; q < n_e; q += (i64)gridDim.x * blockDim.x) z[elist[q]] *= factor;
 }
diff --git a/penguin/jl_amd/csrc/pg_spmv.h b/penguin/jl_amd/csrc/pg_spmv.h
--- a/penguin/jl_amd/csrc/pg_spmv.h
+++ b/penguin/jl_amd/csrc/pg_spmv.h
@@ -178,6 +178,9 @@
 void launch_spmv_typed(int kind, const CsrMatrix& A, const void* x, void* y, const double* sc, int grid, hipStream_t st,
                        const FinArgs& fin);
 bool spmv_supports_typed_chain();
+void spmv_force_handout(int handout);
+void spmv_stamped_launches(const CsrMatrix& A, int handout, const float* x, float* y, const float* base, double pc0, double pc1,
+                           double pc2, int grid, int reps, hipStream_t st, unsigned long long* stamps);
 bool spmv_with_halo(int mode, const CsrMatrix& A, const Numbering& nb, const Slab& slab, double* x, double* y, const double* aux,
                     double* partials, const double* sc, int grid, hipStream_t st, const FinArgs* fin = nullptr);
 void launch_spmv_variant(int variant, const CsrMatrix& A, const double* x, double* y, hipStream_t st);
diff --git a/penguin/jl_amd/csrc/pg_spmv.hip b/penguin/jl_amd/csrc/pg_spmv.hip
--- a/penguin/jl_amd/csrc/pg_spmv.hip
+++ b/penguin/jl_amd/csrc/pg_spmv.hip
@@ -608,7 +608,21 @@
   }
 }
 
-template <int MODE, bool NT, bool DIAG, class VT = VecF64>
+struct HandArgs {
+  unsigned* heads;
+  int set;
+  int rung;
+  unsigned long long* stamps;
+};
+constexpr int HANDOUT_LINE = 32;
+constexpr int HANDOUT_SET = 16 * HANDOUT_LINE;
+constexpr int HANDOUT_WORDS = 2 * HANDOUT_SET;
+
+__device__ inline unsigned draw_ticket(unsigned* head) {
+  return __builtin_amdgcn_atomic_inc32(head, 0xFFFFFFFFu, __ATOMIC_RELAXED, "agent");
+}
+
+template <int MODE, bool NT, bool DIAG, class VT = VecF64, bool DYN = false>
 __global__ __launch_bounds__(BLOCK, 4) void k_spmv_s(i64 nslices, const int* __restrict__ srec,
                                                   const double* __restrict__ pval, const int* __restrict__ g_rowid,
                                                   const int* __restrict__ g_rowptr, const int* __restrict__ g_col,
@@ -617,11 +631,18 @@
                                                   double* __restrict__ partials, const double* __restrict__ sc, int xcd,
                                                   FinArgs fin, int pstride, int accum, const int* __restrict__ mrec,
                                                   i64 nunits, const int* __restrict__ tiles, int tpx,
-                                                  const double* __restrict__ e_val) {
+                                                  const double* __restrict__ e_val, HandArgs hand) {
   __shared__ __attribute__((aligned(16))) double s_val[BLOCK / 64][512];
   __shared__ __attribute__((aligned(16))) double s_x[BLOCK / 64][512];
   __shared__ double s_red[BLOCK / 64];
+  static_assert(!DYN || MODE == 0 || MODE == 8, "the dynamic hand-out is for the launches without dots");
+  if (DYN && blockIdx.x == 0 && threadIdx.x < 16)
+    __hip_atomic_store(hand.heads + HANDOUT_SET * (hand.set ^ 1) + HANDOUT_LINE * (int)threadIdx.x, 0u, __ATOMIC_RELAXED,
+                       __HIP_MEMORY_SCOPE_AGENT);
   if (sc && sc[S_DONE] != 0.0) return;
+  const unsigned long long stamp0 = DIAG ? __builtin_amdgcn_s_memtime() : 0ull;
+  unsigned long long stamp1 = 0, stamp2 = 0;
+  unsigned cnt_u5 = 0, cnt_u7 = 0, cnt_sg = 0, cnt_sup = 0;
   using MI = ModeInfo<MODE>;
   constexpr bool DOTS = MI::DOT0;
   static_assert(MODE == 8 || std::is_same<VT, VecF64>::value, "element types per stream exist for mode 8 only");
@@ -659,8 +680,42 @@
     ubase = ulo = 0; uhi = nunits;
     sbase = slo = 0; shi = nslices;
   }
+  unsigned* const uhead = DYN ? hand.heads + HANDOUT_SET * hand.set + HANDOUT_LINE * xid : nullptr;
+  unsigned* const shead = DYN ? uhead + 8 * HANDOUT_LINE : nullptr;
+  int stick0 = -1;
+  auto unit_body = [&](const int urec) __attribute__((always_inline)) {
+    if (!(dbg & 16)) {
+      const bool edge = rlane(urec, MARCH_EDGE + 1) > 0;
+      if (((rlane(urec, 0) >> 8) & 255) == 7) {
+        if (DIAG) ++cnt_u7;
+        if (edge) march_dispatch<7, MODE, true, VT>(urec, lane, x, y, pa, pb, fin.pc0, fin.pc1, fin.pc2, acc0, acc1, acc2, dbg, e_val, sv, sx, p32, psig);
+        else march_dispatch<7, MODE, false, VT>(urec, lane, x, y, pa, pb, fin.pc0, fin.pc1, fin.pc2, acc0, acc1, acc2, dbg, e_val, sv, sx, p32, psig);
+      } else {
+        if (DIAG) ++cnt_u5;
+        if (edge) march_dispatch<5, MODE, true, VT>(urec, lane, x, y, pa, pb, fin.pc0, fin.pc1, fin.pc2, acc0, acc1, acc2, dbg, e_val, sv, sx, p32, psig);
+        else march_dispatch<5, MODE, false, VT>(urec, lane, x, y, pa, pb, fin.pc0, fin.pc1, fin.pc2, acc0, acc1, acc2, dbg, e_val, sv, sx, p32, psig);
+      }
+    }
+  };
   auto run_units = [&]() __attribute__((always_inline)) {
-  if (nunits > 0) {
+  if (DYN) {
+    const int ucount = (int)(uhi - ulo);
+    int t0 = woff, t1 = woff + wstr;
+    int urec = t0 < ucount ? mrec[(unsigned)(MARCH_REC * ((int)ulo + t0) + lane)] : 0;
+    asm volatile("" : "+v"(urec));
+    while (t0 < ucount) {
+      const bool more = t1 < ucount;
+      const int urec_n = mrec[(unsigned)(MARCH_REC * ((int)ulo + (more ? t1 : t0)) + lane)];
+      unsigned tv = 0;
+      if (lane == 0) tv = draw_ticket(more ? uhead : shead);
+      unit_body(urec);
+      urec = urec_n;
+      const int tn = (int)rlane((int)tv, 0);
+      t0 = t1;
+      t1 = more ? 2 * wstr + tn : ucount;
+      if (!more) stick0 = tn;
+    }
+  } else if (nunits > 0) {
     int d = (woff - (int)(ulo - ubase)) % wstr;
     d = d < 0 ? d + wstr : d;
     i64 ucur = ulo + d;
@@ -669,34 +724,17 @@
     for (; ucur < uhi; ucur += ustride) {
       const i64 un = ucur + ustride;
       const int urec_n = mrec[(unsigned)(MARCH_REC * (int)(un < uhi ? un : ucur) + lane)];
-      if (!(dbg & 16)) {
-        const bool edge = rlane(urec, MARCH_EDGE + 1) > 0;
-        if (((rlane(urec, 0) >> 8) & 255) == 7) {
-          if (edge) march_dispatch<7, MODE, true, VT>(urec, lane, x, y, pa, pb, fin.pc0, fin.pc1, fin.pc2, acc0, acc1, acc2, dbg, e_val, sv, sx, p32, psig);
-          else march_dispatch<7, MODE, false, VT>(urec, lane, x, y, pa, pb, fin.pc0, fin.pc1, fin.pc2, acc0, acc1, acc2, dbg, e_val, sv, sx, p32, psig);
-        } else {
-          if (edge) march_dispatch<5, MODE, true, VT>(urec, lane, x, y, pa, pb, fin.pc0, fin.pc1, fin.pc2, acc0, acc1, acc2, dbg, e_val, sv, sx, p32, psig);
-          else march_dispatch<5, MODE, false, VT>(urec, lane, x, y, pa, pb, fin.pc0, fin.pc1, fin.pc2, acc0, acc1, acc2, dbg, e_val, sv, sx, p32, psig);
-        }
-      }
+      unit_body(urec);
       urec = urec_n;
     }
   }
   };
-  auto run_slices = [&]() __attribute__((always_inline)) {
-  int ds_ = (woff - (int)(slo - sbase)) % wstr;
-  ds_ = ds_ < 0 ? ds_ + wstr : ds_;
-  const i64 first = slo + ds_, wstride = wstr, hi = shi;
-  const i64 lastc = hi - 1;
-  int rec = first < hi ? srec[(unsigned)(SL_REC * (int)first + l31)] : 0;
-  int rec_n = srec[(unsigned)(SL_REC * (int)(first + wstride < hi ? first + wstride : (first < hi ? lastc : 0)) + l31)];
-  for (i64 chunk = first; chunk < hi; chunk += wstride) {
-    const i64 cnn = chunk + 2 * wstride;
-    const int rec_nn = srec[(unsigned)(SL_REC * (int)(cnn < hi ? cnn : lastc) + l31)];
+  auto slice_body = [&](const int rec) __attribute__((always_inline)) {
     SDesc d;
     d.r0 = rlane(rec, 0); d.meta = rlane(rec, 1); d.base = rlane(rec, 2); d.aux = rlane(rec, 3);
     const int nrows = d.meta & 255, type = (d.meta >> 8) & 3, cnt = d.meta >> 16;
     const bool skip = ((dbg & 1) && type == SL_G) || ((dbg & 2) && type != SL_G);
+    if (DIAG) { if (type == SL_G) ++cnt_sg; else ++cnt_sup; }
     if (skip) {
     } else if (type == SL_U) {
       slice_dispatch<false, MODE, NT, VT>(cnt, d, nrows, rec, pval, x, y, pa, pb, lane, acc0, acc1, acc2, dbg, fin.pc0, fin.pc1, fin.pc2, p32, psig);
@@ -759,12 +797,60 @@
         if (MI::DOT2) acc2 += opb * sum;
       }
     }
+  };
+  auto run_slices = [&]() __attribute__((always_inline)) {
+  if (DYN) {
+    const int scount = (int)(shi - slo);
+    const int lastc = scount > 0 ? (int)slo + scount - 1 : 0;
+    const int have = stick0 >= 0 ? 1 : 0;
+    unsigned tv = 0;
+    if (lane < 3 - have) tv = draw_ticket(shead);
+    int c = have ? stick0 : rlane((int)tv, 2), n1 = rlane((int)tv, 0), n2 = rlane((int)tv, 1);
+    if (!have && c > n1) { const int t = c; c = n1; n1 = t; }
+    if (n1 > n2) { const int t = n1; n1 = n2; n2 = t; }
+    if (!have && c > n1) { const int t = c; c = n1; n1 = t; }
+    int rec = c < scount ? srec[(unsigned)(SL_REC * ((int)slo + c) + l31)] : 0;
+    int rec_n = srec[(unsigned)(SL_REC * (n1 < scount ? (int)slo + n1 : lastc) + l31)];
+    while (c < scount) {
+      const int rec_nn = srec[(unsigned)(SL_REC * (n2 < scount ? (int)slo + n2 : lastc) + l31)];
+      unsigned tn = 0;
+      if (lane == 0) tn = draw_ticket(shead);
+      slice_body(rec);
+      rec = rec_n;
+      rec_n = rec_nn;
+      c = n1; n1 = n2; n2 = rlane((int)tn, 0);
+    }
+  } else {
+  int ds_ = (woff - (int)(slo - sbase) - (hand.rung && !tiles ? (int)((uhi - ulo) % wstr) : 0)) % wstr;
+  ds_ = ds_ < 0 ? ds_ + wstr : ds_;
+  const i64 first = slo + ds_, wstride = wstr, hi = shi;
+  const i64 lastc = hi - 1;
+  int rec = first < hi ? srec[(unsigned)(SL_REC * (int)first + l31)] : 0;
+  int rec_n = srec[(unsigned)(SL_REC * (int)(first + wstride < hi ? first + wstride : (first < hi ? lastc : 0)) + l31)];
+  for (i64 chunk = first; chunk < hi; chunk += wstride) {
+    const i64 cnn = chunk + 2 * wstride;
+    const int rec_nn = srec[(unsigned)(SL_REC * (int)(cnn < hi ? cnn : lastc) + l31)];
+    slice_body(rec);
     rec = rec_n;
     rec_n = rec_nn;
   }
+  }
   };
   if (DIAG && (dbg & 4096)) { run_slices(); run_units(); }
-  else { run_units(); run_slices(); }
+  else {
+    run_units();
+    if (DIAG) stamp1 = __builtin_amdgcn_s_memtime();
+    run_slices();
+  }
+  }
+  if (DIAG && (dbg & 8192) && hand.stamps) {
+    asm volatile("s_waitcnt vmcnt(0)" ::: "memory");
+    stamp2 = __builtin_amdgcn_s_memtime();
+    if (lane == 0) {
+      unsigned long long* o = hand.stamps + 4 * ((size_t)blockIdx.x * (BLOCK / 64) + wave);
+      o[0] = stamp0; o[1] = stamp1; o[2] = stamp2;
+      o[3] = (unsigned long long)cnt_u5 | ((unsigned long long)cnt_u7 << 16) | ((unsigned long long)cnt_sg << 32) | ((unsigned long long)cnt_sup << 48);
+    }
   }
   if (DOTS) {
     const double t0 = block_sum(acc0, s_red);
@@ -862,6 +948,26 @@
   hipLaunchKernelGGL(HIP_KERNEL_NAME(KERNEL), dim3(grid), dim3(BLOCK), 0, st, A.n, A.nchunks, A.chunk_desc.p, \
                      A.rowptr.p, A.col.p, A.val.p, x, y, aux, partials, sc)
 
+int g_handout_force = -1;
+int handout_mode() { return g_handout_force >= 0 ? g_handout_force : config().spmv_handout; }
+
+HandArgs hand_args(const CsrMatrix& A, int mode, bool eligible, hipStream_t st) {
+  HandArgs h{nullptr, 0, 0, nullptr};
+  const int ho = handout_mode();
+  if (!eligible || ho == 0 || (mode != 0 && mode != 8)) return h;
+  if (ho == 2) { h.rung = 1; return h; }
+  if (ctx().nranks != 1 || st != ctx().stream || !A.handout.p) return h;
+  h.heads = A.handout.p;
+  h.set = (int)(const_cast<CsrMatrix&>(A).handout_k++ & 1u);
+  return h;
+}
+
+void alloc_handout(CsrMatrix& A) {
+  A.handout.alloc(HANDOUT_WORDS);
+  A.handout.zero();
+  A.handout_k = 0;
+}
+
 template <int MODE>
 bool launch_slices(int v, const CsrMatrix& A, i64 s0, i64 ns, const double* x, double* y, const double* aux, double* partials,
                    const double* sc, int grid, int pstride, int accum, hipStream_t st, const FinArgs* fin, bool units = true) {
@@ -872,18 +978,25 @@
   const bool tiled = units && A.tiles_per_xcd > 0 && s0 == 0 && ns == A.tile_ns && (xcd_map() & 1) && grid >= 8;
   const int* tiles = tiled ? (const int*)A.tiles.p : nullptr;
   const int tpx = tiled ? A.tiles_per_xcd : 0;
-  if (xcd_map() >= 256)
+  const bool diag = xcd_map() >= 256, whole = units && s0 == 0 && ns == A.nslices && !accum;
+  const HandArgs hand = hand_args(A, MODE, whole && !tiled && !diag && (v & 4), st);
+  if (diag)
     hipLaunchKernelGGL(HIP_KERNEL_NAME(k_spmv_s<MODE, true, true>), dim3(grid), dim3(BLOCK), 0, st, ns, rec, A.pval.p,
                        A.g_rowid.p, A.g_rowptr.p, A.g_col.p, A.g_val.p, x, y, aux, partials, sc, xcd_map(), fa, pstride, accum,
-                       (const int*)A.mrec.p, nu, tiles, tpx, (const double*)A.e_val.p);
-  else if (v & 4)
+                       (const int*)A.mrec.p, nu, tiles, tpx, (const double*)A.e_val.p, hand);
+  else if (hand.heads) {
+    if constexpr (MODE == 0 || MODE == 8)
+      hipLaunchKernelGGL(HIP_KERNEL_NAME(k_spmv_s<MODE, true, false, VecF64, true>), dim3(grid), dim3(BLOCK), 0, st, ns, rec, A.pval.p,
+                         A.g_rowid.p, A.g_rowptr.p, A.g_col.p, A.g_val.p, x, y, aux, partials, sc, xcd_map(), fa, pstride, accum,
+                         (const int*)A.mrec.p, nu, tiles, tpx, (const double*)A.e_val.p, hand);
+  } else if (v & 4)
     hipLaunchKernelGGL(HIP_KERNEL_NAME(k_spmv_s<MODE, true, false>), dim3(grid), dim3(BLOCK), 0, st, ns, rec, A.pval.p,
                        A.g_rowid.p, A.g_rowptr.p, A.g_col.p, A.g_val.p, x, y, aux, partials, sc, xcd_map(), fa, pstride, accum,
-                       (const int*)A.mrec.p, nu, tiles, tpx, (const double*)A.e_val.p);
+                       (const int*)A.mrec.p, nu, tiles, tpx, (const double*)A.e_val.p, hand);
   else
     hipLaunchKernelGGL(HIP_KERNEL_NAME(k_spmv_s<MODE, false, false>), dim3(grid), dim3(BLOCK), 0, st, ns, rec, A.pval.p,
                        A.g_rowid.p, A.g_rowptr.p, A.g_col.p, A.g_val.p, x, y, aux, partials, sc, xcd_map(), fa, pstride, accum,
-                       (const int*)A.mrec.p, nu, tiles, tpx, (const double*)A.e_val.p);
+                       (const int*)A.mrec.p, nu, tiles, tpx, (const double*)A.e_val.p, hand);
   return fa.ticket != nullptr;
 }
 
@@ -906,13 +1019,52 @@
 template <class VT>
 void launch_typed(const CsrMatrix& A, const void* x, void* y, const double* sc, int grid, hipStream_t st, const FinArgs& fin) {
   const bool tiled = A.tiles_per_xcd > 0 && A.nslices == A.tile_ns && (xcd_map() & 1) && grid >= 8;
-  hipLaunchKernelGGL(HIP_KERNEL_NAME(k_spmv_s<8, true, false, VT>), dim3(grid), dim3(BLOCK), 0, st, A.nslices, (const int*)A.srec.p,
-                     (const double*)A.pval.p, (const int*)A.g_rowid.p, (const int*)A.g_rowptr.p, (const int*)A.g_col.p,
-                     (const double*)A.g_val.p, static_cast<const typename VT::TX*>(x), static_cast<typename VT::TY*>(y),
-                     (const double*)nullptr, (double*)nullptr, sc, xcd_map(), fin, grid, 0, (const int*)A.mrec.p, A.nunits,
-                     tiled ? (const int*)A.tiles.p : (const int*)nullptr, tiled ? A.tiles_per_xcd : 0, (const double*)A.e_val.p);
-}
-
+  const HandArgs hand = hand_args(A, 8, !tiled, st);
+  if (hand.heads)
+    hipLaunchKernelGGL(HIP_KERNEL_NAME(k_spmv_s<8, true, false, VT, true>), dim3(grid), dim3(BLOCK), 0, st, A.nslices, (const int*)A.srec.p,
+                       (const double*)A.pval.p, (const int*)A.g_rowid.p, (const int*)A.g_rowptr.p, (const int*)A.g_col.p,
+                       (const double*)A.g_val.p, static_cast<const typename VT::TX*>(x), static_cast<typename VT::TY*>(y),
+                       (const double*)nullptr, (double*)nullptr, sc, xcd_map(), fin, grid, 0, (const int*)A.mrec.p, A.nunits,
+                       (const int*)nullptr, 0, (const double*)A.e_val.p, hand);
+  else
+    hipLaunchKernelGGL(HIP_KERNEL_NAME(k_spmv_s<8, true, false, VT>), dim3(grid), dim3(BLOCK), 0, st, A.nslices, (const int*)A.srec.p,
+                       (const double*)A.pval.p, (const int*)A.g_rowid.p, (const int*)A.g_rowptr.p, (const int*)A.g_col.p,
+                       (const double*)A.g_val.p, static_cast<const typename VT::TX*>(x), static_cast<typename VT::TY*>(y),
+                       (const double*)nullptr, (double*)nullptr, sc, xcd_map(), fin, grid, 0, (const int*)A.mrec.p, A.nunits,
+                       tiled ? (const int*)A.tiles.p : (const int*)nullptr, tiled ? A.tiles_per_xcd : 0, (const double*)A.e_val.p, hand);
+}
+
+}
+
+void spmv_force_handout(int handout) { g_handout_force = handout; }
+
+void spmv_stamped_launches(const CsrMatrix& A, int handout, const float* x, float* y, const float* base, double pc0, double pc1,
+                           double pc2, int grid, int reps, hipStream_t st, unsigned long long* stamps) {
+  PG_REQUIRE(A.n > 0 && A.srec.p && A.handout.p && st == ctx().stream, "stamped launches: a slice image, on the library stream");
+  using VT = VecTypes<float, float, float, false>;
+  FinArgs fin{nullptr, nullptr, PH_NONE, 0, 0, nullptr};
+  fin.pc0 = pc0; fin.pc1 = pc1; fin.pc2 = pc2;
+  const int xcd = (xcd_map() & 255) | (8192 << 8);
+  for (int r = 0; r < reps; ++r) {
+    const float* xin = (r & 1) ? y : x;
+    float* yout = (r & 1) ? const_cast<float*>(x) : y;
+    fin.base = reinterpret_cast<const double*>(base);
+    HandArgs hand{nullptr, 0, handout == 2 ? 1 : 0, stamps};
+    if (handout == 1) {
+      hand.heads = A.handout.p;
+      hand.set = (int)(const_cast<CsrMatrix&>(A).handout_k++ & 1u);
+      hipLaunchKernelGGL(HIP_KERNEL_NAME(k_spmv_s<8, true, true, VT, true>), dim3(grid), dim3(BLOCK), 0, st, A.nslices, (const int*)A.srec.p,
+                         (const double*)A.pval.p, (const int*)A.g_rowid.p, (const int*)A.g_rowptr.p, (const int*)A.g_col.p,
+                         (const double*)A.g_val.p, xin, yout, (const double*)nullptr, (double*)nullptr, (const double*)nullptr, xcd, fin, grid, 0,
+                         (const int*)A.mrec.p, A.nunits, (const int*)nullptr, 0, (const double*)A.e_val.p, hand);
+    } else {
+      hipLaunchKernelGGL(HIP_KERNEL_NAME(k_spmv_s<8, true, true, VT, false>), dim3(grid), dim3(BLOCK), 0, st, A.nslices, (const int*)A.srec.p,
+                         (const double*)A.pval.p, (const int*)A.g_rowid.p, (const int*)A.g_rowptr.p, (const int*)A.g_col.p,
+                         (const double*)A.g_val.p, xin, yout, (const double*)nullptr, (double*)nullptr, (const double*)nullptr, xcd, fin, grid, 0,
+                         (const int*)A.mrec.p, A.nunits, (const int*)nullptr, 0, (const double*)A.e_val.p, hand);
+    }
+  }
+  PG_HIP(hipGetLastError());
 }
 
 bool spmv_supports_typed_chain() { return (variant() & 64) != 0 && (variant() & 4) != 0 && xcd_map() < 256; }
@@ -1337,6 +1489,7 @@
   }
   A.srec.alloc((i64)sd.size());
   A.srec.upload(sd.data(), (i64)sd.size());
+  alloc_handout(A);
   if (A.nslices > 0) {
     hipLaunchKernelGGL(k_fill_records, dim3(grid_for(A.nslices, 256)), dim3(256), 0, st, A.nslices, A.srec.p, A.rowptr.p, A.col.p,
                        A.val.p);
@@ -1455,6 +1608,7 @@
     hipLaunchKernelGGL(k_fill_edges, dim3(grid_for(A.rows_e, 256)), dim3(256), 0, st, A.rows_e, (const int*)A.e_meta.p, A.rowptr.p,
                        A.val.p, A.e_val.p);
   clone_buf(A.srec, T.srec, st);
+  alloc_handout(A);
   clone_buf(A.g_rowid, T.g_rowid, st);
   clone_buf(A.g_rowptr, T.g_rowptr, st);
   A.pval.alloc(A.nnz_p + 8);
diff --git a/penguin/jl_amd/csrc/pg_system.h b/penguin/jl_amd/csrc/pg_system.h
--- a/penguin/jl_amd/csrc/pg_system.h
+++ b/penguin/jl_amd/csrc/pg_system.h
@@ -54,6 +54,8 @@
   DevBuf<int> tiles;
   int tiles_per_xcd = 0;
   i64 tile_ns = 0;
+  DevBuf<unsigned> handout;
+  unsigned handout_k = 0;
   const int* geo_cell = nullptr;
   const int* geo_map = nullptr;
   i64 geo_ext0 = 0, geo_lines = 0;
```

After: 1363. -1.0%, worse.
